# mlee03/FRE-NCtools

Hardware: AMD Instinct MI355X
Metric: exchange-cells/s (higher is better)
Workload: dtype f64; 1 GPU; C384 cubed sphere (6 tiles) -> 1440x720 lat-lon, conservative_order2: exchange-grid search + centroid pass + CSR build per step; nxgrid=4160000, parallelism=1 latitude band(s) of the target, one per GPU, world_size=1

## Files before the change

fre-nctools_amd/csrc/apply_kernels.hip:

```cpp
#include "xgrid_device.h"
#include <type_traits>

static inline int nblk(long n, int t) { return (int)((n + t - 1) / t); }

__global__ __launch_bounds__(256) void k_csr_count(long nx, const int *x_dst, int *row_cnt)
{
  long n = (long)blockIdx.x * blockDim.x + threadIdx.x;
  if (n < nx) atomicAdd(&row_cnt[x_dst[n]], 1);
}

__global__ __launch_bounds__(256) void k_csr_fill(long nx, const int *x_src, const int *x_dst, const int *row_ptr, int *row_fill, FgRowEnt *perm)
{
  const long n = (long)blockIdx.x * blockDim.x + threadIdx.x;
  const int lane = threadIdx.x & 63;
  const int d = (n < nx) ? x_dst[n] : -1;
  const int s = (n < nx) ? x_src[n] : 0;
  const int prev = __shfl_up(d, 1);
  const bool head = (lane == 0) || (d != prev);
  const unsigned long long heads = __ballot(head);
  const int start = 63 - __clzll((long long)(heads & ((2ull << lane) - 1ull)));
  const unsigned long long above = (start == 63) ? 0ull : (heads & ~((2ull << start) - 1ull));
  const int end = above ? (__ffsll((long long)above) - 1) : 64;
  int base = 0;
  if (lane == start && d >= 0) base = atomicAdd(&row_fill[d], end - start);
  base = __shfl(base, start);
  if (d >= 0) perm[row_ptr[d] + base + (lane - start)] = FgRowEnt{(int)n, s};
}

__global__ __launch_bounds__(256) void k_csr_fill_pos(long nx, const unsigned long long *nx_dev, const int *x_src, const int *x_dst,
                                                       const int *row_ptr, const int *x_rowpos, FgRowEnt *perm)
{
  if (nx_dev) { const unsigned long long nd = *nx_dev; if (nd < (unsigned long long)nx) nx = (long)nd; }
  const long n = (long)blockIdx.x * blockDim.x + threadIdx.x;
  if (n < nx) { const int s = x_src[n]; perm[row_ptr[x_dst[n]] + x_rowpos[n]] = FgRowEnt{(int)n, s}; }
}

template <int N>
__device__ __forceinline__ void d_rank_count(const int *keys, int n, const int (&v)[N], int (&rank)[N])
{
  int j = 0;
  for (; j + 4 <= n; j += 4) {
    const int x0 = keys[j], x1 = keys[j + 1], x2 = keys[j + 2], x3 = keys[j + 3];
#pragma unroll
    for (int k = 0; k < N; k++) rank[k] += ((x0 < v[k]) ? 1 : 0) + ((x1 < v[k]) ? 1 : 0) + ((x2 < v[k]) ? 1 : 0) + ((x3 < v[k]) ? 1 : 0);
  }
  for (; j < n; j++) {
    const int x = keys[j];
#pragma unroll
    for (int k = 0; k < N; k++) rank[k] += (x < v[k]) ? 1 : 0;
  }
}

template <typename E>
__device__ __forceinline__ void d_store_stream(E *dst, const E &e)
{
  typedef int v4i __attribute__((ext_vector_type(4)));
  static_assert(sizeof(E) % 16 == 0 && alignof(E) >= 8, "records are whole 16-byte words");
  v4i w[sizeof(E) / 16];
  __builtin_memcpy(w, &e, sizeof(E));
#pragma unroll
  for (unsigned k = 0; k < sizeof(E) / 16; k++) __builtin_nontemporal_store(w[k], (v4i *)dst + k);
}

template <int ORDER, bool DIST, int BT, int G, bool STAGED>
__device__ __forceinline__ void d_csr_records(const int *sh, const int *shs, const FgRowEnt *perm, int q0, int nq, const double *x_area,
                                              const double *x_c1, const double *x_c2, const int *src_idx_f, const FgSrcRec *cen,
                                              const FgCsr &csr)
{
  for (int i0 = threadIdx.x; i0 < nq; i0 += BT * G) {
    int n[G], s[G], idx[G];
    double ar[G], c1[G], c2[G], cl[G], ct[G];
#pragma unroll
    for (int g = 0; g < G; g++) {
      const int i = i0 + BT * g, ic = (i < nq) ? i : i0;
      if (STAGED) { n[g] = sh[ic]; s[g] = shs[ic]; }
      else { const FgRowEnt p = perm[q0 + ic]; n[g] = p.n; s[g] = p.s; }
    }
#pragma unroll
    for (int g = 0; g < G; g++) {
      ar[g] = x_area[n[g]];
      if (ORDER == 2) { c1[g] = x_c1[n[g]]; c2[g] = x_c2[n[g]]; }
      idx[g] = src_idx_f[s[g]];
      if (ORDER == 2 && DIST) { const FgSrcRec r = cen[s[g]]; cl[g] = r.cen_lon; ct[g] = r.cen_lat; }
    }
#pragma unroll
    for (int g = 0; g < G; g++) {
      const int i = i0 + BT * g;
      if (ORDER == 2) {
        FgCsrEntry2 E;
        E.idx_f = idx[g]; E.idx_g = s[g]; E.area = ar[g];
        if (DIST) {
          double di = c1[g] / E.area, dj = c2[g] / E.area;
          di -= cl[g]; dj -= ct[g];
          E.di = di; E.dj = dj;
        } else { E.di = c1[g]; E.dj = c2[g]; }
        if (i < nq) d_store_stream(&csr.e2[q0 + i], E);
      } else {
        FgCsrEntry1 E;
        E.idx_f = idx[g]; E.pad = 0; E.area = ar[g];
        if (i < nq) d_store_stream(&csr.e1[q0 + i], E);
      }
    }
  }
}

__device__ __forceinline__ void d_row_insertion(FgRowEnt *perm, int b, int e)
{
  for (int i = b + 1; i < e; i++) {
    const FgRowEnt v = perm[i];
    int j = i - 1;
    while (j >= b && perm[j].n > v.n) { perm[j + 1] = perm[j]; j--; }
    perm[j + 1] = v;
  }
}

#define SG_GROUP 2
template <int ORDER, int RPW, bool DIST, int BT, int G>
__global__ __launch_bounds__(BT) void k_csr_sortgather(int ndst, FgRowEnt *perm, const double *x_area, const double *x_c1, const double *x_c2,
                                                        const int *src_idx_f, const FgSrcRec *cen, FgCsr csr, int *tmp, long ntmp)
{
  constexpr int SHORT = 12, CAP = (RPW >= 64) ? 512 : 2048;
  __shared__ int sh[CAP], shs[CAP];
  __shared__ int long_b[RPW], long_n[RPW];
  __shared__ int nlong;
  if (threadIdx.x == 0) nlong = 0;
  __syncthreads();
  const int d0 = blockIdx.x * RPW, d1 = min(d0 + RPW, ndst);
  const int q0 = csr.row_ptr[d0], q1 = csr.row_ptr[d1], nq = q1 - q0;
  const bool staged = nq <= CAP;
  const int d = d0 + threadIdx.x;
  int b = 0, e = 0;
  if ((int)threadIdx.x < RPW && d < ndst) { b = csr.row_ptr[d]; e = csr.row_ptr[d + 1]; }
  if (staged) {
    for (int i = threadIdx.x; i < nq; i += BT) { const FgRowEnt p = perm[q0 + i]; sh[i] = p.n; shs[i] = p.s; }
    __syncthreads();
    if (e - b > SHORT) { const int q = atomicAdd(&nlong, 1); long_b[q] = b - q0; long_n[q] = e - b; }
    else
      for (int i = b - q0 + 1; i < e - q0; i++) {
        const int v = sh[i], w = shs[i];
        int j = i - 1;
        while (j >= b - q0 && sh[j] > v) { sh[j + 1] = sh[j]; shs[j + 1] = shs[j]; j--; }
        sh[j + 1] = v; shs[j + 1] = w;
      }
    __syncthreads();
    const int nl = nlong;
    for (int q = 0; q < nl; q++) {
      const int rb = long_b[q], n = long_n[q];
      constexpr int OWN = CAP / BT;
      if (n <= BT) {
        const bool own = (int)threadIdx.x < n;
        int v = 0, w = 0, rank = 0;
        if (own) {
          v = sh[rb + threadIdx.x]; w = shs[rb + threadIdx.x];
          for (int j = 0; j < n; j++) rank += (sh[rb + j] < v) ? 1 : 0;
        }
        __syncthreads();
        if (own) { sh[rb + rank] = v; shs[rb + rank] = w; }
      } else {
        int v[OWN], w[OWN], rank[OWN];
#pragma unroll
        for (int k = 0; k < OWN; k++) {
          const int i = threadIdx.x + BT * k;
          v[k] = (i < n) ? sh[rb + i] : 0x7fffffff; w[k] = (i < n) ? shs[rb + i] : 0; rank[k] = 0;
        }
        d_rank_count<OWN>(sh + rb, n, v, rank);
        __syncthreads();
#pragma unroll
        for (int k = 0; k < OWN; k++) if ((int)threadIdx.x + BT * k < n) { sh[rb + rank[k]] = v[k]; shs[rb + rank[k]] = w[k]; }
      }
      __syncthreads();
    }
  } else {
    if (e - b > SHORT) { const int q = atomicAdd(&nlong, 1); long_b[q] = b; long_n[q] = e - b; }
    else d_row_insertion(perm, b, e);
    __syncthreads();
    const int nl = nlong;
    for (int q = 0; q < nl; q++) {
      const int rb = long_b[q], n = long_n[q];
      if (n <= CAP) {
        for (int i = threadIdx.x; i < n; i += BT) { const FgRowEnt p = perm[rb + i]; sh[i] = p.n; shs[i] = p.s; }
        __syncthreads();
        for (int i = threadIdx.x; i < n; i += BT) {
          const int v = sh[i];
          int rank = 0;
          for (int j = 0; j < n; j++) rank += (sh[j] < v) ? 1 : 0;
          perm[rb + rank] = FgRowEnt{v, shs[i]};
        }
        __syncthreads();
      } else if (tmp) {
        FgRowEnt *srt = (FgRowEnt *)tmp + rb;
        int *rk = tmp + 2 * ntmp + rb;
        for (int t0 = 0; t0 < n; t0 += CAP) {
          const int m = min(CAP, n - t0);
          for (int j = threadIdx.x; j < m; j += BT) sh[j] = perm[rb + t0 + j].n;
          __syncthreads();
          for (int i0 = threadIdx.x; i0 < n; i0 += 8 * BT) {
            int v[8], r[8];
#pragma unroll
            for (int k = 0; k < 8; k++) { const int i = i0 + BT * k; v[k] = (i < n) ? perm[rb + i].n : 0x7fffffff; r[k] = (i < n && t0) ? rk[i] : 0; }
            d_rank_count<8>(sh, m, v, r);
#pragma unroll
            for (int k = 0; k < 8; k++) { const int i = i0 + BT * k; if (i < n) rk[i] = r[k]; }
          }
          __syncthreads();
        }
        for (int i = threadIdx.x; i < n; i += BT) srt[rk[i]] = perm[rb + i];
        __syncthreads();
        for (int i = threadIdx.x; i < n; i += BT) perm[rb + i] = srt[i];
        __syncthreads();
      } else if (threadIdx.x == 0) d_row_insertion(perm, rb, rb + n);
    }
    __syncthreads();
  }
  if (staged) d_csr_records<ORDER, DIST, BT, G, true>(sh, shs, perm, q0, nq, x_area, x_c1, x_c2, src_idx_f, cen, csr);
  else        d_csr_records<ORDER, DIST, BT, G, false>(sh, shs, perm, q0, nq, x_area, x_c1, x_c2, src_idx_f, cen, csr);
}

__global__ __launch_bounds__(256) void k_src_field_index(int order, const FgTile *tiles, int ntiles, int nsrc, int *src_idx_f)
{
  int s = blockIdx.x * blockDim.x + threadIdx.x;
  if (s >= nsrc) return;
  if (order != 2) { src_idx_f[s] = s; return; }
  int t = 0, foff = 0;
  while (t + 1 < ntiles && s >= tiles[t + 1].cell_off) { foff += (tiles[t].nx + 2) * (tiles[t].ny + 2); t++; }
  int loc = s - tiles[t].cell_off;
  int i = loc % tiles[t].nx, j = loc / tiles[t].nx;
  src_idx_f[s] = foff + (j + 1) * (tiles[t].nx + 2) + i + 1;
}

__device__ __forceinline__ int d_xcd_block(int b, int nb, int band)
{
  if (!band) return b;
  if (band == 1) {
    const int x = b & 7, k = b >> 3, q = nb >> 3, r = nb & 7;
    return x * q + min(x, r) + k;
  }
  const int C = band, per = 8 * C, full = nb / per * per;
  if (b >= full) return b;
  const int x = b & 7, k = b >> 3;
  return ((k / C) * 8 + x) * C + (k % C);
}

template <int ORDER> using CsrEntry = typename std::conditional<ORDER == 2, FgCsrEntry2, FgCsrEntry1>::type;
template <int ORDER> __device__ __forceinline__ const CsrEntry<ORDER> *csr_entries(const FgCsr &csr)
{
  if constexpr (ORDER == 2) return csr.e2; else return csr.e1;
}
typedef unsigned int u4v __attribute__((ext_vector_type(4)));

struct EpTile { int q0, q1, d, lev, b, e; bool lane; };
template <int ROWS, int LPR>
__device__ __forceinline__ EpTile ep_tile(const FgCsr &csr, int ndst, int tile)
{
  EpTile T;
  const int t = threadIdx.x;
  const int d0 = tile * ROWS, dl = min(d0 + ROWS, ndst);
  T.q0 = csr.row_ptr[d0]; T.q1 = csr.row_ptr[dl];
  T.lane = t < ROWS * LPR;
  T.d = d0 + t / LPR; T.lev = t % LPR;
  const int dc = min(T.d, ndst - 1);
  T.b = 0; T.e = 0;
  if (T.lane) { T.b = csr.row_ptr[dc]; T.e = csr.row_ptr[dc + 1]; }
  return T;
}

template <int TPB, int CAP, typename Entry>
__device__ __forceinline__ void ep_stage_unrolled(Entry *sh_e, const Entry *src, int n)
{
  constexpr int W = sizeof(Entry) / 16, WPL = CAP * W / TPB;
  const int t = threadIdx.x, nw = n * W;
  const u4v *g = reinterpret_cast<const u4v *>(src);
  u4v *l = reinterpret_cast<u4v *>(sh_e);
  u4v w[WPL];
#pragma unroll
  for (int j = 0; j < WPL; j++) w[j] = __builtin_nontemporal_load(g + min(t + TPB * j, nw - 1));
#pragma unroll
  for (int j = 0; j < WPL; j++) if (t + TPB * j < nw) l[t + TPB * j] = w[j];
}
template <int TPB, typename Entry>
__device__ __forceinline__ void ep_stage_loop(Entry *sh_e, const Entry *src, int n)
{
  constexpr int W = sizeof(Entry) / 16;
  const u4v *g = reinterpret_cast<const u4v *>(src);
  u4v *l = reinterpret_cast<u4v *>(sh_e);
  for (int i = threadIdx.x; i < n * W; i += TPB) l[i] = __builtin_nontemporal_load(g + i);
}

struct EpTerm { double p, a; unsigned ok; };
template <typename F>
__device__ __forceinline__ void ep_row_add(int b, int e, int c0, int n, double &acc, double &asum, unsigned &touched, F term)
{
  const int qa = max(b, c0) - c0, qb = min(e, c0 + n) - c0;
  int q = qa;
  for (; q + 8 <= qb; q += 8) {
    EpTerm c[8];
#pragma unroll
    for (int k = 0; k < 8; k++) c[k] = term(q + k);
#pragma unroll
    for (int k = 0; k < 8; k++) { acc += c[k].p; asum += c[k].a; touched |= c[k].ok; }
  }
  for (; q < qb; q++) { const EpTerm c = term(q); acc += c.p; asum += c.a; touched |= c.ok; }
}

__device__ __forceinline__ double apply_finish(double acc, double asum, bool touched, double missing, double &rs)
{
  rs = (asum > 0) ? acc : 0.0;
  if (asum > 0) return acc / asum;
  return touched ? 0.0 : missing;
}
__device__ __forceinline__ double apply_finish_ex(const FgApplyEx &o, int d, double acc, double asum, double asum_t, bool touched, double &rs)
{
  if (o.sum) {
    rs = (asum > 0) ? acc : 0.0;
    return (asum == 0) ? (touched ? 0.0 : o.missing) : acc;
  }
  double r = apply_finish(acc, asum, touched, o.missing, rs);
  if (o.cell_area_out && r != o.missing) r *= (asum_t / o.cell_area_out[d]);
  return r;
}

template <int ORDER, bool MISSING>
__global__ __launch_bounds__(256) void k_apply1(int ndst, FgCsr csr, const double *f, const double *px, const double *py,
                                                 const int *gmask, double missing, double *out, double *row_sum)
{
  int d = blockIdx.x * 256 + threadIdx.x;
  if (d >= ndst) return;
  int b = csr.row_ptr[d], e = csr.row_ptr[d + 1];
  double acc = 0.0, asum = 0.0;
  int touched = 0;
  for (int q = b; q < e; q++) {
    double a, v;
    if (ORDER == 2) {
      const FgCsrEntry2 E = csr.e2[q];
      a = E.area; v = f[E.idx_f];
      if (MISSING) { if (v == missing) continue; }
      bool flatgrad = false;
      if (MISSING) flatgrad = gmask[E.idx_g] != 0;
      if (!flatgrad) v = (v + px[E.idx_g] * E.di + py[E.idx_g] * E.dj);
    } else {
      const FgCsrEntry1 E = csr.e1[q];
      a = E.area; v = f[E.idx_f];
      if (MISSING) { if (v == missing) continue; }
    }
    acc += v * a;
    asum += a;
    touched = 1;
  }
  double rs;
  const double r = apply_finish(acc, asum, touched != 0, missing, rs);
  if (row_sum) row_sum[d] = rs;
  out[d] = r;
}

template <int ORDER, bool MISSING, int TPB, int CAP, int ROWS>
__global__ __launch_bounds__(TPB) void k_apply_ep1(int ndst, FgCsr csr, const double *f, const double *px, const double *py, const int *gmask,
                                                    double missing, double *out, double *row_sum, int xcd_band)
{
  typedef CsrEntry<ORDER> Entry;
  constexpr int PASS = CAP / TPB;
  static_assert(ROWS <= TPB && CAP % TPB == 0, "tile shape");
  __shared__ __attribute__((aligned(16))) Entry sh_e[CAP];
  double *sh_p = reinterpret_cast<double *>(sh_e), *sh_a = sh_p + CAP;
  __shared__ unsigned char sh_fl[CAP];
  const int t = threadIdx.x;
  const EpTile T = ep_tile<ROWS, 1>(csr, ndst, d_xcd_block(blockIdx.x, gridDim.x, xcd_band));
  double acc = 0.0, asum = 0.0;
  unsigned touched = 0;
  for (int c0 = T.q0; c0 < T.q1; c0 += CAP) {
// ... 469 lines not shown
  if (!T.lane || T.d >= ndst || (MASKED && lev >= nb_valid)) return;
  double rs;
  const double r = apply_finish(acc, asum, MASKED ? touched != 0 : T.e > T.b, missing, rs);
  if (row_sum) row_sum[MASKED ? (size_t)lev * out_ld + T.d : (size_t)T.d * NB + lev] = rs;
  if (MASKED || out_ld > 0) { if (lev < nb_valid) out[(size_t)lev * out_ld + T.d] = r; }
  else out[(size_t)T.d * NB + lev] = r;
}

__global__ __launch_bounds__(256) void k_gmask_bits(long n, const int *gmask, long ld, int nb, unsigned char *bits)
{
  const long c = (long)blockIdx.x * blockDim.x + threadIdx.x;
  if (c >= n) return;
  unsigned m = 0;
  for (int k = 0; k < nb; k++) m |= (gmask[(size_t)k * ld + c] != 0 ? 1u : 0u) << k;
  bits[c] = (unsigned char)m;
}

template <int NB>
__global__ __launch_bounds__(256) void k_interleave(long n, const double *in, long ld, int nb, double *out)
{
  long c = (long)blockIdx.x * blockDim.x + threadIdx.x;
  if (c >= n) return;
  double v[NB];
#pragma unroll
  for (int k = 0; k < NB; k++) v[k] = (k < nb) ? in[(size_t)k * ld + c] : 0.0;
#pragma unroll
  for (int k = 0; k < NB; k++) out[(size_t)c * NB + k] = v[k];
}
template <int NB>
__global__ __launch_bounds__(256) void k_deinterleave(long n, const double *in, long ld, int nb, double *out)
{
  long c = (long)blockIdx.x * blockDim.x + threadIdx.x;
  if (c >= n) return;
  double v[NB];
#pragma unroll
  for (int k = 0; k < NB; k++) v[k] = in[(size_t)c * NB + k];
#pragma unroll
  for (int k = 0; k < NB; k++) if (k < nb) out[(size_t)k * ld + c] = v[k];
}

struct FgIl3 { const double *in[3]; double *out[3]; long n[3]; long ld[3]; };
template <int NB>
__global__ __launch_bounds__(256) void k_interleave3(FgIl3 a, int nb)
{
  __shared__ double tile[256 * (NB + 1)];
  const int w = blockIdx.y;
  const long n = a.n[w];
  const long c0 = (long)blockIdx.x * 256;
  if (c0 >= n) return;
  const double *in = a.in[w];
  double *out = a.out[w];
  const long ld = a.ld[w];
  const long c = c0 + threadIdx.x;
#pragma unroll
  for (int k = 0; k < NB; k++) tile[threadIdx.x * (NB + 1) + k] = (k < nb && c < n) ? in[(size_t)k * ld + c] : 0.0;
  __syncthreads();
  const long cnt = ((n - c0) < 256 ? (n - c0) : 256) * NB;
#pragma unroll
  for (int i = 0; i < NB; i++) {
    const long e = (long)i * 256 + threadIdx.x;
    if (e < cnt) out[(size_t)c0 * NB + e] = tile[(e / NB) * (NB + 1) + (e % NB)];
  }
}

template <int NB, int CB>
__global__ __launch_bounds__(256) void k_merge3(long n, const int *src_idx_f, const double *f, long ld_f, const double *gx,
                                                const double *gy, long ld_g, int nb, double *out)
{
  constexpr int R = 3 * NB;
  __shared__ double tile[CB * (R + 1)];
  const long c0 = (long)blockIdx.x * CB;
  const int t = threadIdx.x % CB;
  const long c = c0 + t;
  const long cf = (c < n) ? (long)src_idx_f[c] : 0;
  for (int e = threadIdx.x; e < CB * R; e += 256) {
    const int wk = e / CB, w = wk / NB, k = wk % NB;
    double v = 0.0;
    if (k < nb && c < n) v = (w == 0) ? f[(size_t)k * ld_f + cf] : ((w == 1) ? gx[(size_t)k * ld_g + c] : gy[(size_t)k * ld_g + c]);
    tile[t * (R + 1) + wk] = v;
  }
  __syncthreads();
  const long cnt = ((n - c0) < CB ? (n - c0) : CB) * R;
  for (long e = threadIdx.x; e < cnt; e += 256) out[(size_t)c0 * R + e] = tile[(e / R) * (R + 1) + (e % R)];
}

__global__ __launch_bounds__(256) void k_xgrid_indices(long nx, const int *x_src, const int *x_dst, const FgTile *tiles, int ntiles,
                                                        int nx_out, int *t_in, int *i_in, int *j_in, int *i_out, int *j_out)
{
  const long k = (long)blockIdx.x * blockDim.x + threadIdx.x;
  if (k >= nx) return;
  const int s = x_src[k], d = x_dst[k];
  int m = 0;
  while (m + 1 < ntiles && s >= tiles[m + 1].cell_off) m++;
  const int loc = s - tiles[m].cell_off, nxt = tiles[m].nx;
  t_in[k] = m; i_in[k] = loc % nxt; j_in[k] = loc / nxt;
  i_out[k] = d % nx_out; j_out[k] = d / nx_out;
}
void fgd_xgrid_indices(long nx, const int *x_src, const int *x_dst, const FgTile *tiles_dev, int ntiles, int nx_out,
                       int *t_in, int *i_in, int *j_in, int *i_out, int *j_out, hipStream_t st)
{
  if (nx > 0) k_xgrid_indices<<<nblk(nx, 256), 256, 0, st>>>(nx, x_src, x_dst, tiles_dev, ntiles, nx_out, t_in, i_in, j_in, i_out, j_out);
}

__global__ __launch_bounds__(256) void k_apply_frac(int ndst, FgCsr csr, const double *data, double *out)
{
  int d = blockIdx.x * blockDim.x + threadIdx.x;
  if (d >= ndst) return;
  int b = csr.row_ptr[d], e = csr.row_ptr[d + 1];
  double asum = 0.0, acc = 0.0;
  for (int q = b; q < e; q++) asum += csr.e1[q].area;
  for (int q = b; q < e; q++) {
    double frac = csr.e1[q].area / asum;
    acc += data[csr.e1[q].idx_f] * frac;
  }
  out[d] = acc;
}

__global__ __launch_bounds__(256) void k_reduce_partial(const double *v, long n, double *partial)
{
  __shared__ double sh[256];
  double s = 0;
  for (long i = (long)blockIdx.x * blockDim.x + threadIdx.x; i < n; i += (long)gridDim.x * blockDim.x) s += v[i];
  sh[threadIdx.x] = s;
  __syncthreads();
  for (int w = 128; w > 0; w >>= 1) { if (threadIdx.x < w) sh[threadIdx.x] += sh[threadIdx.x + w]; __syncthreads(); }
  if (threadIdx.x == 0) partial[blockIdx.x] = sh[0];
}
__global__ __launch_bounds__(256) void k_reduce_final(const double *partial, int np, double *result)
{
  __shared__ double sh[256];
  double s = 0;
  for (int i = threadIdx.x; i < np; i += 256) s += partial[i];
  sh[threadIdx.x] = s;
  __syncthreads();
  for (int w = 128; w > 0; w >>= 1) { if (threadIdx.x < w) sh[threadIdx.x] += sh[threadIdx.x + w]; __syncthreads(); }
  if (threadIdx.x == 0) *result = sh[0];
}

#define REDUCE_BLOCKS 512

void fgd_csr_count(long nx, const int *x_dst, int *row_cnt, hipStream_t st)
{
  if (nx > 0) k_csr_count<<<nblk(nx, 256), 256, 0, st>>>(nx, x_dst, row_cnt);
}
void fgd_csr_fill(long nx, const int *x_src, const int *x_dst, const int *row_ptr, int *row_fill, FgRowEnt *perm, hipStream_t st)
{
  if (nx > 0) k_csr_fill<<<nblk(nx, 256), 256, 0, st>>>(nx, x_src, x_dst, row_ptr, row_fill, perm);
}
void fgd_csr_fill_pos(long nx_cap, const unsigned long long *nx_dev, const int *x_src, const int *x_dst, const int *row_ptr, const int *x_rowpos, FgRowEnt *perm,
                      hipStream_t st)
{
  if (nx_cap > 0) k_csr_fill_pos<<<nblk(nx_cap, 256), 256, 0, st>>>(nx_cap, nx_dev, x_src, x_dst, row_ptr, x_rowpos, perm);
}
void fgd_csr_sortgather(int order, int ndst, long nx, const FgRowEnt *perm, const double *x_area, const double *x_c1, const double *x_c2,
                        const int *src_idx_f, const FgSrcRec *cen, FgCsr csr, hipStream_t st, int *tmp, long ntmp,
                        int long_rows)
{
  if (ndst <= 0) return;
  FgRowEnt *pm = const_cast<FgRowEnt *>(perm);
  const int mode = nx > 256 * (long)ndst ? 2 : ((nx > 8 * (long)ndst || long_rows) ? 1 : 0);
#define SG(O_, R_, D_) k_csr_sortgather<O_, R_, D_, (R_ >= 64 ? 64 : 256), SG_GROUP><<<nblk(ndst, R_), (R_ >= 64 ? 64 : 256), 0, st>>>(ndst, pm, x_area, x_c1, x_c2, src_idx_f, cen, csr, tmp, ntmp)
#define SGM(O_, D_) do { if (mode == 2) SG(O_, 1, D_); else if (mode == 1) SG(O_, 16, D_); else SG(O_, 64, D_); } while (0)
  if (order == 2) { if (cen) SGM(2, true); else SGM(2, false); }
  else SGM(1, false);
#undef SGM
#undef SG
}
void fgd_src_field_index(int order, const FgTile *tiles_dev, int ntiles, int nsrc, int *src_idx_f, hipStream_t st)
{
  if (nsrc > 0) k_src_field_index<<<nblk(nsrc, 256), 256, 0, st>>>(order, tiles_dev, ntiles, nsrc, src_idx_f);
}
extern int g_apply_xcd, g_apply_ep;
template <int V> using Int = std::integral_constant<int, V>;
template <int R0, int R1, int R2, int R3, typename F>
static void by_row_length(long m, F launch)
{
  if (m <= 6) launch(Int<R0>()); else if (m <= 24) launch(Int<R1>()); else if (m <= 96) launch(Int<R2>()); else launch(Int<R3>());
}
static int xcd_chunk8() { return g_apply_xcd >= 2 ? 2 * g_apply_xcd : g_apply_xcd; }

void fgd_apply1(int order, int ndst, FgCsr csr, const double *f, const double *gx, const double *gy, const int *gmask,
                int has_missing, double missing, double *out, double *row_sum, hipStream_t st, long nx)
{
  if (ndst <= 0) return;
  if (g_apply_ep && nx >= 0) {
    auto ep1 = [&](auto O, auto M) {
      by_row_length<64, 16, 4, 1>(nx / ndst, [&](auto R) {
        k_apply_ep1<decltype(O)::value, decltype(M)::value, 256, 512, decltype(R)::value><<<nblk(ndst, decltype(R)::value), 256, 0, st>>>(
            ndst, csr, f, gx, gy, gmask, missing, out, row_sum, g_apply_xcd);
      });
    };
    if (order == 2) { if (has_missing) ep1(Int<2>(), std::true_type()); else ep1(Int<2>(), std::false_type()); }
    else            { if (has_missing) ep1(Int<1>(), std::true_type()); else ep1(Int<1>(), std::false_type()); }
    return;
  }
  int grid = nblk(ndst, 256);
  if (order == 2) {
    if (has_missing) k_apply1<2, true><<<grid, 256, 0, st>>>(ndst, csr, f, gx, gy, gmask, missing, out, row_sum);
    else             k_apply1<2, false><<<grid, 256, 0, st>>>(ndst, csr, f, gx, gy, gmask, missing, out, row_sum);
  } else {
    if (has_missing) k_apply1<1, true><<<grid, 256, 0, st>>>(ndst, csr, f, gx, gy, gmask, missing, out, row_sum);
    else             k_apply1<1, false><<<grid, 256, 0, st>>>(ndst, csr, f, gx, gy, gmask, missing, out, row_sum);
  }
}

template <int ORDER, bool MASKED, int CAP, int R0, int R1, int R2, int R3>
static void apply_ep8g(int ndst, long nx, FgCsr csr, const double *rec, const unsigned char *gbits, double missing, double *out,
                       double *row_sum, long out_ld, int nb_valid, int xb, hipStream_t st)
{
  by_row_length<R0, R1, R2, R3>(nx / ndst, [&](auto R) {
    k_apply_ep8g<ORDER, MASKED, 256, CAP, decltype(R)::value><<<nblk(ndst, decltype(R)::value), 256, 0, st>>>(
        ndst, csr, rec, gbits, missing, out, row_sum, out_ld, nb_valid, xb);
  });
}

template <int NB, int V>
static void apply_il_nb(int order, int ndst, FgCsr csr, const double *f, const double *gx, const double *gy, double missing,
                        double *out, double *row_sum, long out_ld, int nb_valid, hipStream_t st)
{
  int grid = nblk(ndst, 256 / (NB / V));
  if (order == 2) k_apply_il<2, NB, V><<<grid, 256, 0, st>>>(ndst, csr, f, gx, gy, missing, out, row_sum, out_ld, nb_valid, g_apply_xcd);
  else            k_apply_il<1, NB, V><<<grid, 256, 0, st>>>(ndst, csr, f, gx, gy, missing, out, row_sum, out_ld, nb_valid, g_apply_xcd);
}
int g_apply_xcd = 64;
int g_apply_ep = 1;
int g_apply_vec = 0;
void fgd_apply_il(int order, int nb, int ndst, FgCsr csr, const double *f, const double *gx, const double *gy, double missing,
                  double *out, double *row_sum, long out_ld, int nb_valid, hipStream_t st, long nx)
{
  if (ndst <= 0) return;
  if (order == 1 && nb == 8 && g_apply_ep && nx > 6L * ndst) {
    apply_ep8g<1, false, 256, 8, 8, 2, 1>(ndst, nx, csr, f, nullptr, missing, out, row_sum, out_ld, nb_valid, xcd_chunk8(), st);
    return;
  }
  const int v = g_apply_vec ? g_apply_vec : (nb >= 8 ? 4 : 2);
#define AP(NB_) do { if (v >= 4 && NB_ >= 4) apply_il_nb<NB_, (NB_ >= 4 ? 4 : 2)>(order, ndst, csr, f, gx, gy, missing, out, row_sum, out_ld, nb_valid, st); \
                     else if (v >= 2) apply_il_nb<NB_, 2>(order, ndst, csr, f, gx, gy, missing, out, row_sum, out_ld, nb_valid, st); \
                     else apply_il_nb<NB_, 1>(order, ndst, csr, f, gx, gy, missing, out, row_sum, out_ld, nb_valid, st); } while (0)
  if (nb == 16) AP(16);
  else if (nb == 8) AP(8);
  else if (nb == 4) AP(4);
  else AP(2);
#undef AP
}
void fgd_apply_il_merged(int nb, int ndst, long nx, FgCsr csr, const double *rec, double missing, double *out, double *row_sum, long out_ld,
                         int nb_valid, hipStream_t st)
{
  if (ndst <= 0) return;
#define APM(NB_, V_) k_apply_il<2, NB_, V_, true><<<nblk(ndst, 256 / (NB_ / V_)), 256, 0, st>>>(ndst, csr, rec, nullptr, nullptr, missing, out, row_sum, out_ld, nb_valid, g_apply_xcd)
  if (nb == 16) APM(16, 4);
  else if (nb == 8 && g_apply_ep && nx <= 6L * ndst)
    k_apply_ep8<256, 256><<<nblk(ndst, EP_ROWS), 256, 0, st>>>(ndst, csr, rec, missing, out, row_sum, out_ld, nb_valid, xcd_chunk8());
  else if (nb == 8 && g_apply_ep)
    apply_ep8g<2, false, 256, 8, 8, 2, 1>(ndst, nx, csr, rec, nullptr, missing, out, row_sum, out_ld, nb_valid, xcd_chunk8(), st);
  else if (nb == 8) { if (g_apply_vec == 2) APM(8, 2); else APM(8, 4); }
  else if (nb == 4) APM(4, 2);
  else APM(2, 2);
#undef APM
}
void fgd_apply_levels8(int order, int ndst, long nx, FgCsr csr, const double *rec, const unsigned char *gbits, double missing, double *out,
                       double *row_sum, long ld, int nb_valid, hipStream_t st)
{
  if (ndst <= 0) return;
  if (order == 2) apply_ep8g<2, true, FG_LEVELS_CAP, 32, 8, 2, 1>(ndst, nx, csr, rec, gbits, missing, out, row_sum, ld, nb_valid, 0, st);
  else            apply_ep8g<1, true, FG_LEVELS_CAP, 32, 8, 2, 1>(ndst, nx, csr, rec, gbits, missing, out, row_sum, ld, nb_valid, 0, st);
}
void fgd_gmask_bits(long n, const int *gmask, long ld, int nb, unsigned char *bits, hipStream_t st)
{
  if (n > 0) k_gmask_bits<<<nblk(n, 256), 256, 0, st>>>(n, gmask, ld, nb, bits);
}
void fgd_merge3(int nb_pad, long n, const int *src_idx_f, const double *f, long ld_f, const double *gx, const double *gy, long ld_g,
                int nb_valid, double *out, hipStream_t st)
{
  if (n <= 0) return;
  if (nb_pad == 16) k_merge3<16, 64><<<nblk(n, 64), 256, 0, st>>>(n, src_idx_f, f, ld_f, gx, gy, ld_g, nb_valid, out);
  else if (nb_pad == 8) k_merge3<8, 64><<<nblk(n, 64), 256, 0, st>>>(n, src_idx_f, f, ld_f, gx, gy, ld_g, nb_valid, out);
  else if (nb_pad == 4) k_merge3<4, 128><<<nblk(n, 128), 256, 0, st>>>(n, src_idx_f, f, ld_f, gx, gy, ld_g, nb_valid, out);
  else k_merge3<2, 128><<<nblk(n, 128), 256, 0, st>>>(n, src_idx_f, f, ld_f, gx, gy, ld_g, nb_valid, out);
}
void fgd_interleave(int nb_pad, long n, const double *in, long ld, int nb_valid, double *out, hipStream_t st)
{
  if (n <= 0) return;
  if (nb_pad == 16) k_interleave<16><<<nblk(n, 256), 256, 0, st>>>(n, in, ld, nb_valid, out);
  else if (nb_pad == 8) k_interleave<8><<<nblk(n, 256), 256, 0, st>>>(n, in, ld, nb_valid, out);
  else if (nb_pad == 4) k_interleave<4><<<nblk(n, 256), 256, 0, st>>>(n, in, ld, nb_valid, out);
  else k_interleave<2><<<nblk(n, 256), 256, 0, st>>>(n, in, ld, nb_valid, out);
}
void fgd_interleave3(int nb_pad, int narr, const double *const *in, const long *ld, const long *n, double *const *out, int nb_valid,
                     hipStream_t st)
{
  FgIl3 a;
  long nmax = 0;
  for (int w = 0; w < 3; w++) {
    a.in[w] = (w < narr) ? in[w] : nullptr; a.out[w] = (w < narr) ? out[w] : nullptr;
    a.n[w] = (w < narr) ? n[w] : 0; a.ld[w] = (w < narr) ? ld[w] : 0;
    if (a.n[w] > nmax) nmax = a.n[w];
  }
  if (nmax <= 0) return;
  dim3 grid(nblk(nmax, 256), narr);
  if (nb_pad == 16) k_interleave3<16><<<grid, 256, 0, st>>>(a, nb_valid);
  else if (nb_pad == 8) k_interleave3<8><<<grid, 256, 0, st>>>(a, nb_valid);
  else if (nb_pad == 4) k_interleave3<4><<<grid, 256, 0, st>>>(a, nb_valid);
  else k_interleave3<2><<<grid, 256, 0, st>>>(a, nb_valid);
}
void fgd_deinterleave(int nb_pad, long n, const double *in, long ld, int nb_valid, double *out, hipStream_t st)
{
  if (n <= 0) return;
  if (nb_pad == 16) k_deinterleave<16><<<nblk(n, 256), 256, 0, st>>>(n, in, ld, nb_valid, out);
  else if (nb_pad == 8) k_deinterleave<8><<<nblk(n, 256), 256, 0, st>>>(n, in, ld, nb_valid, out);
  else if (nb_pad == 4) k_deinterleave<4><<<nblk(n, 256), 256, 0, st>>>(n, in, ld, nb_valid, out);
  else k_deinterleave<2><<<nblk(n, 256), 256, 0, st>>>(n, in, ld, nb_valid, out);
}
void fgd_apply_ex(int order, int ndst, FgCsr csr, const double *f, const double *gx, const double *gy, FgApplyEx o,
                  double *out, double *row_sum, int *err, hipStream_t st, long nx)
// ... 46 lines not shown
```

fre-nctools_amd/csrc/plan.hip:

```cpp
#include <hip/hip_runtime.h>
#include <math.h>
#include <stdarg.h>
#include <stdio.h>
#include <stdlib.h>
#include <string.h>
#include <algorithm>
#include <map>
#include <mutex>
#include <string>
#include <type_traits>
#include <vector>
#include "fregrid_hip.h"
#include "xgrid_device.h"

static thread_local std::string g_err;
static int fail(int code, const char *fmt, ...)
{
  char buf[512];
  va_list ap; va_start(ap, fmt); vsnprintf(buf, sizeof buf, fmt, ap); va_end(ap);
  g_err = buf;
  return code;
}
#define HIPCHK(call) do { hipError_t e_ = (call); if (e_ != hipSuccess) \
  return fail(FG_ERR_HIP, "%s failed: %s (%s:%d)", #call, hipGetErrorString(e_), __FILE__, __LINE__); } while (0)
// ... 196 lines not shown
    for (const XferJob &j : batch) total += j.bytes;
    if (total == 0) return true;
    static const int nthreads = [] {
      const char *e = getenv("FREGRID_HIP_XFER_THREADS");
      int n = e ? atoi(e) : 0;
      if (n <= 0) { const unsigned hc = std::thread::hardware_concurrency(); n = hc >= 16 ? 8 : (hc >= 8 ? 4 : 2); }
      return std::min(n, 16);
    }();
    if (total < 2 * CHUNK) {
      if (hipSetDevice(dev) != hipSuccess) return false;
      for (const XferJob &j : batch)
        if (j.bytes && hipMemcpy(j.d2h ? j.host : j.dev, j.d2h ? j.dev : j.host, j.bytes, j.d2h ? hipMemcpyDeviceToHost : hipMemcpyHostToDevice) != hipSuccess) return false;
      return true;
    }
    std::lock_guard<std::mutex> bl(batch_mu);
    {
      std::lock_guard<std::mutex> lk(mu);
      if (threads.empty())
        for (int t = 0; t < nthreads; t++) { threads.emplace_back([this] { loop(); }); threads.back().detach(); }
      jobs = &batch; chunks.clear();
      for (size_t k = 0; k < batch.size(); k++)
        for (size_t off = 0; off < batch[k].bytes; off += CHUNK) chunks.push_back({(int)k, off});
      next.store(0); failed.store(0); device = dev; active = (int)threads.size(); gen++;
    }
    cv_work.notify_all();
    std::unique_lock<std::mutex> lk(mu);
    cv_done.wait(lk, [&] { return active == 0; });
    jobs = nullptr;
    return failed.load() == 0;
  }
};
XferPool &xfer_pool() { static XferPool *p = new XferPool(); return *p; }
}

static int g_profiling = 0;
extern "C" void fg_set_profiling(int on) { g_profiling = on ? 1 : 0; }
enum { PH_CELL_STRUCT = 0, PH_BINS, PH_CANDIDATES, PH_CLIP_QUAD, PH_CLIP_GENERAL, PH_COMPACT, PH_ROWS,
       PH_SEARCH_TOTAL, PH_FINALIZE, PH_APPLY, PH_COUNT };
struct HandleCache {
  std::mutex mu;
  std::map<int, std::vector<hipStream_t>> streams;
  std::map<int, std::vector<hipEvent_t>> events;
  static int current_device() { int d = 0; (void)hipGetDevice(&d); return d; }
  hipStream_t get_stream(int dev)
  {
    {
      std::lock_guard<std::mutex> lk(mu);
      auto &v = streams[dev];
      if (!v.empty()) { hipStream_t s = v.back(); v.pop_back(); return s; }
    }
    hipStream_t s = nullptr;
    if (hipStreamCreateWithFlags(&s, hipStreamNonBlocking) != hipSuccess) return nullptr;
    return s;
  }
  void put_stream(int dev, hipStream_t s)
  {
    if (!s) return;
    std::lock_guard<std::mutex> lk(mu);
    streams[dev].push_back(s);
  }
  hipEvent_t get_event()
  {
    {
      std::lock_guard<std::mutex> lk(mu);
      auto &v = events[current_device()];
      if (!v.empty()) { hipEvent_t e = v.back(); v.pop_back(); return e; }
    }
    hipEvent_t e = nullptr;
    (void)hipEventCreate(&e);
    return e;
  }
  void put_event(hipEvent_t e)
  {
    if (!e) return;
    std::lock_guard<std::mutex> lk(mu);
    events[current_device()].push_back(e);
  }
  std::map<int, std::vector<hipEvent_t>> sync_events;
  hipEvent_t get_sync_event()
  {
    {
      std::lock_guard<std::mutex> lk(mu);
      auto &v = sync_events[current_device()];
      if (!v.empty()) { hipEvent_t e = v.back(); v.pop_back(); return e; }
    }
    hipEvent_t e = nullptr;
    (void)hipEventCreateWithFlags(&e, hipEventDisableTiming);
    return e;
  }
  void put_sync_event(hipEvent_t e)
  {
    if (!e) return;
    std::lock_guard<std::mutex> lk(mu);
    sync_events[current_device()].push_back(e);
  }
};
static HandleCache g_handles;

struct PhaseTimer {
  bool on = false;
  hipStream_t st = nullptr;
  std::vector<std::pair<int, std::pair<hipEvent_t, hipEvent_t>>> spans;
  hipEvent_t open_ev = nullptr; int open_ph = -1;
  void start(bool enable, hipStream_t s) { on = enable; st = s; }
  void begin(int ph)
  {
    if (!on) return;
    open_ev = g_handles.get_event(); (void)hipEventRecord(open_ev, st); open_ph = ph;
  }
  void end()
  {
    if (!on || open_ph < 0) return;
    hipEvent_t e = g_handles.get_event(); (void)hipEventRecord(e, st);
    spans.push_back({open_ph, {open_ev, e}}); open_ph = -1;
  }
  void collect(float *ms)
  {
    for (auto &sp : spans) {
      float t = 0; (void)hipEventElapsedTime(&t, sp.second.first, sp.second.second);
      ms[sp.first] += t;
      g_handles.put_event(sp.second.first); g_handles.put_event(sp.second.second);
    }
    spans.clear();
  }
};

struct fg_plan {
  float phase_ms[PH_COUNT] = {0};
  PhaseTimer apply_pt;
  int apply_spans = 0;
  int order = 0, device = 0;
  bool great_circle = false;
  hipStream_t stream = nullptr;
  hipStream_t stream_b = nullptr;
  bool own_stream = true;
  int ntiles = 0;
  std::vector<int> nx_in, ny_in, cell_off;
  std::vector<FgTile> tiles_host;
  int nsrc = 0;
  int nx_out = 0, ny_out = 0, ndst = 0;
  long f_stride = 0;
  bool searched = false, finalized = false, have_geom = false;
  bool fused = false;

  std::vector<void *> owned;
  FgTile *tiles_dev = nullptr;
  double *mask_dev = nullptr;
  FgCells S{}, D{};
  bool rect = false;
  FgRect rect_tab{};
  FgPolyList polys{};
  long nx = 0;
  int *x_src = nullptr, *x_dst = nullptr;
  double *x_area = nullptr, *x_c1 = nullptr, *x_c2 = nullptr;
  int *xoff = nullptr;
  FgRowEnt *perm = nullptr;
  bool rows_built = false;
  bool dist_pending = false;
  double *sums = nullptr;
  FgSrcRec *cen = nullptr;
  FgCsr csr{};
  int *src_idx_f = nullptr;
  double *row_sum = nullptr, *red_partial = nullptr, *red_result = nullptr;
  long row_sum_cap = 0;
  double *il_f = nullptr, *il_out = nullptr, *il_rs = nullptr;
  double *il_m = nullptr;
  unsigned char *lv_bits = nullptr;
  long stats[FG_NSTATS] = {0};
  double *mono_x = nullptr, *mono_b = nullptr;
  int *xerr = nullptr;
  bool mono_open = false;
  unsigned *ll_err = nullptr;

  template <typename T> T *alloc(size_t count)
  {
    void *p = g_pool.get(device, count * sizeof(T));
    if (p) owned.push_back(p);
    return (T *)p;
  }
  void release(void *p)
  {
    if (!p) return;
    for (size_t k = 0; k < owned.size(); k++) if (owned[k] == p) { owned.erase(owned.begin() + k); break; }
    g_pool.put(p);
  }
  void drop_search(size_t keep)
  {
    while (owned.size() > keep) { g_pool.put(owned.back()); owned.pop_back(); }
    tiles_dev = nullptr; mask_dev = nullptr; S = FgCells{}; D = FgCells{};
    x_src = x_dst = nullptr; x_area = x_c1 = x_c2 = nullptr; xoff = nullptr;
    perm = nullptr; csr.row_ptr = nullptr; csr.e1 = nullptr; csr.e2 = nullptr; cen = nullptr; src_idx_f = nullptr; sums = nullptr;
    have_geom = false; rect = false; rect_tab = FgRect{};
  }
};

static bool alloc_cells(fg_plan *pl, FgCells *c, size_t n)
{
  c->lat_min = pl->alloc<double>(n); c->lat_max = pl->alloc<double>(n);
  c->lon_min = pl->alloc<double>(n); c->lon_max = pl->alloc<double>(n);
  c->lon_avg = pl->alloc<double>(n); c->area = pl->alloc<double>(n);
  c->nv = pl->alloc<int>(n);
  c->verts = pl->alloc<double>(n * 16);
  return c->lat_min && c->lat_max && c->lon_min && c->lon_max && c->lon_avg && c->area && c->nv && c->verts;
}

static int plan_base(int order, int ntiles_in, const int *nx_in, const int *ny_in, int nx_out, int ny_out,
                     int device, fg_plan **out)
{
  if (order != FG_CONSERVE_ORDER1 && order != FG_CONSERVE_ORDER2) return fail(FG_ERR_ARG, "order must be 1 or 2");
  if (ntiles_in < 1 || !nx_in || !ny_in || nx_out < 1 || ny_out < 1 || !out) return fail(FG_ERR_ARG, "bad grid sizes");
  int ndev = 0;
  HIPCHK(hipGetDeviceCount(&ndev));
  if (ndev < 1) return fail(FG_ERR_HIP, "no HIP device visible: libfregrid_hip needs an MI355X-class GPU");
  if (device < 0 || device >= ndev) return fail(FG_ERR_ARG, "device %d out of range (0..%d)", device, ndev - 1);
  HIPCHK(hipSetDevice(device));
  fg_plan *pl = new fg_plan();
  pl->order = order; pl->device = device; pl->ntiles = ntiles_in;
  long off = 0, foff = 0;
  for (int m = 0; m < ntiles_in; m++) {
    if (nx_in[m] < 1 || ny_in[m] < 1) { delete pl; return fail(FG_ERR_ARG, "bad source tile size"); }
    pl->nx_in.push_back(nx_in[m]); pl->ny_in.push_back(ny_in[m]); pl->cell_off.push_back((int)off);
    off += (long)nx_in[m] * ny_in[m];
    foff += (order == 2) ? (long)(nx_in[m] + 2) * (ny_in[m] + 2) : (long)nx_in[m] * ny_in[m];
  }
  if (off > 2000000000L || (long)nx_out * ny_out > 2000000000L) { delete pl; return fail(FG_ERR_ARG, "grid too large for 32-bit cell indices"); }
  pl->nsrc = (int)off; pl->f_stride = foff;
  pl->nx_out = nx_out; pl->ny_out = ny_out; pl->ndst = nx_out * ny_out;
  pl->stream = g_handles.get_stream(device);
  if (!pl->stream) { delete pl; return fail(FG_ERR_HIP, "hipStreamCreate failed"); }
  *out = pl;
  return 0;
}

extern "C" void fg_plan_destroy(fg_plan *pl)
{
  if (!pl) return;
  (void)hipSetDevice(pl->device);
  if (pl->stream || !pl->own_stream) (void)hipStreamSynchronize(pl->stream);
  if (pl->stream && pl->own_stream) g_handles.put_stream(pl->device, pl->stream);
  if (pl->stream_b) { (void)hipStreamSynchronize(pl->stream_b); g_handles.put_stream(pl->device, pl->stream_b); }
  { float junk[PH_COUNT] = {0}; pl->apply_pt.collect(junk); }
  for (void *p : pl->owned) g_pool.put(p);
  delete pl;
}

static void choose_bins(const fg_plan *pl, double mean_dlat, double mean_dlon, FgBins *b)
{
  const double PI = 3.14159265358979323846;
  double h = 1.25 * mean_dlat, w = 1.25 * mean_dlon;
  int nblat = (h > 0) ? (int)ceil(PI / h) : 1;
  int nblon = (w > 0) ? (int)ceil(2.0 * PI / w) : 1;
  if (nblat < 1) nblat = 1; if (nblat > 8192) nblat = 8192;
  if (nblon < 1) nblon = 1; if (nblon > 16384) nblon = 16384;
  (void)pl;
  b->nblat = nblat; b->nblon = nblon;
  b->inv_wlat = nblat / PI;
  b->inv_wlon = nblon / (2.0 * PI);
}

static FgCounters *pinned_counters()
{
  static thread_local FgCounters *h = nullptr;
  if (!h) { if (hipHostMalloc((void **)&h, sizeof(FgCounters), hipHostMallocDefault) != hipSuccess) h = nullptr; }
  return h;
}

struct GcXyz { const double *x, *y, *z; };
struct BoxMode { FgBox box; const double *mask_quad; int no_adjust; };
struct SearchIn {
  const double *const *lon_in = nullptr, *const *lat_in = nullptr, *const *mask_in = nullptr;
  const double *lon_out = nullptr, *lat_out = nullptr;
  const GcXyz *gc_in = nullptr, *gc_out = nullptr;
  const BoxMode *boxm = nullptr;
  double mean_dlat = 0, mean_dlon = 0;
  int rect_hint = 1;
};
struct SearchOpts { bool exact, cull, finalize, rect, dst_frame; int gc_split; bool profile; };
static const char *gc_clip_error(int code)
{
  switch (code) {
    case 3: return "firstIntersect is not in the grid1List";
    case 4: return " not found the next intersection ";
    case 5: return "not return back to the first intersection";
    case 6: return "After clipping, nintersect should be 0";
    case 7: return "inserAfter: point (x,y,z) is not found in the list";
    case 8: return "Error from create_xgrid.c: temp is not in list1";
    default: return "clip_2dx2d_great_circle: more intersections than two convex quadrilaterals can have (list capacity)";
  }
}

static int g_search_cull = 0;
static int g_search_finalize = 0;
static int g_gc_split = 1;
extern "C" void fg_set_gc_split(int on) { g_gc_split = on < 0 ? 0 : on; }
struct SearchCaps { unsigned long long entries; int regcap, nreg; bool rect; };
static int g_search_rect = 1;
extern "C" void fg_set_search_rect(int on) { g_search_rect = on ? 1 : 0; }
static int g_dst_frame = 0;
extern "C" void fg_set_search_frame(int coupler) { g_dst_frame = coupler ? 1 : 0; }
static bool host_says_not_rect(int nx, int ny, const double *lon, const double *lat)
{
  const long nxp = nx + 1;
  const int js[3] = {ny, ny / 2, 1}, is[3] = {nx, nx / 2, 1};
  for (int a = 0; a < 3; a++)
    for (int b = 0; b < 3; b++) {
      const long e = (long)js[a] * nxp + is[b];
      if (memcmp(&lon[e], &lon[is[b]], sizeof(double)) || memcmp(&lat[e], &lat[(long)js[a] * nxp], sizeof(double))) return true;
    }
  return false;
}
#define FG_RETRY (-1000L)
struct Carve {
  size_t n = 0;
  size_t operator()(size_t size) { const size_t at = n; n += size; return at; }
};
struct SearchBlocks {
  fg_plan *pl;
  bool ok = true;
  std::vector<void *> scratch;
  template <typename T> T *keep(size_t count) { T *p = pl->alloc<T>(count); ok = ok && p; return p; }
  template <typename T> T *get(size_t count) { T *p = keep<T>(count); if (p) scratch.push_back(p); return p; }
  void release() { for (void *p : scratch) pl->release(p); scratch.clear(); }
};
static long plan_search_core(fg_plan *pl, const SearchIn &in, const SearchOpts &opt, SearchCaps *caps)
{
  const bool gc = in.gc_in != nullptr;
  const BoxMode *const boxm = in.boxm;
  pl->great_circle = gc;
  hipStream_t st = pl->stream;
  const int nsrc = pl->nsrc, ndst = pl->ndst, order = pl->order;
  FgCounters *hc = pinned_counters();
  if (!hc) return fail(FG_ERR_HIP, "hipHostMalloc failed");

  std::vector<FgTile> &th = pl->tiles_host;
  th.resize(pl->ntiles + 1);
  for (int m = 0; m < pl->ntiles; m++) th[m] = FgTile{gc ? nullptr : in.lon_in[m], gc ? nullptr : in.lat_in[m], pl->nx_in[m], pl->ny_in[m], pl->cell_off[m]};
  th[pl->ntiles] = FgTile{in.lon_out, in.lat_out, pl->nx_out, pl->ny_out, 0};
  pl->tiles_dev = pl->alloc<FgTile>(pl->ntiles + 1);
  if (!pl->tiles_dev) return fail(FG_ERR_HIP, "out of device memory");
  FgTileSet ts; ts.n = 0;
  const bool by_value = !gc && pl->ntiles + 1 <= FG_TILESET_MAX;
  if (by_value) { ts.n = pl->ntiles + 1; for (int m = 0; m <= pl->ntiles; m++) ts.t[m] = th[m]; }
  else HIPCHK(hipMemcpyAsync(pl->tiles_dev, th.data(), sizeof(FgTile) * th.size(), hipMemcpyHostToDevice, st));
  FgTileXyz *gct_dev = nullptr;
  std::vector<FgTileXyz> gct;
  if (gc) {
    gct.resize(pl->ntiles + 1);
    for (int m = 0; m < pl->ntiles; m++) gct[m] = FgTileXyz{in.gc_in[m].x, in.gc_in[m].y, in.gc_in[m].z, pl->nx_in[m], pl->ny_in[m], pl->cell_off[m]};
    gct[pl->ntiles] = FgTileXyz{in.gc_out->x, in.gc_out->y, in.gc_out->z, pl->nx_out, pl->ny_out, 0};
    gct_dev = pl->alloc<FgTileXyz>(pl->ntiles + 1);
    if (!gct_dev) return fail(FG_ERR_HIP, "out of device memory");
    HIPCHK(hipMemcpyAsync(gct_dev, gct.data(), sizeof(FgTileXyz) * gct.size(), hipMemcpyHostToDevice, st));
  }

  bool any_mask = false;
  if (in.mask_in) for (int m = 0; m < pl->ntiles; m++) if (in.mask_in[m]) any_mask = true;
  if (any_mask) {
    pl->mask_dev = pl->alloc<double>(nsrc);
    if (!pl->mask_dev) return fail(FG_ERR_HIP, "out of device memory");
    std::vector<double> ones;
    for (int m = 0; m < pl->ntiles; m++) {
      size_t nc = (size_t)pl->nx_in[m] * pl->ny_in[m];
      if (in.mask_in[m]) HIPCHK(hipMemcpyAsync(pl->mask_dev + pl->cell_off[m], in.mask_in[m], nc * sizeof(double), hipMemcpyDeviceToDevice, st));
      else {
        ones.assign(nc, 1.0);
        HIPCHK(hipMemcpyAsync(pl->mask_dev + pl->cell_off[m], ones.data(), nc * sizeof(double), hipMemcpyHostToDevice, st));
        HIPCHK(hipStreamSynchronize(st));
      }
    }
  }

  const bool rect = caps->rect && !gc && !boxm;
  pl->rect = rect;
  const double dst_tlon = opt.dst_frame ? (double)NAN : 3.14159265358979323846;
  FgBins bins;
  choose_bins(pl, in.mean_dlat, in.mean_dlon, &bins);
  if (rect) { bins.nblat = 0; bins.nblon = 0; }
  const long nbins = (long)bins.nblat * bins.nblon;
  const long nslots = nbins + bins.nblat;
  const unsigned long long nentries = rect ? 0ull : caps->entries;
  const int ecap = (int)std::min<unsigned long long>(nentries, 2147483647ull);
  FgPairSpace ps{};
  ps.nreg = caps->nreg; ps.regcap = caps->regcap;
  const long npairs = fgd_pairs_total(ps);
  const long nx_alloc = npairs;

  if (!alloc_cells(pl, &pl->S, nsrc)) return fail(FG_ERR_HIP, "out of device memory");
  SearchBlocks blk{pl};
  struct { double *hdr, *lat_ax, *lon_ax, *col, *row, *col_min, *col_max, *col_avg; } rt{};
  if (rect) {
    pl->D = FgCells{};
    pl->D.area = blk.keep<double>(ndst);
    Carve at;
    const size_t o_hdr = at(8), o_lat = at((size_t)pl->ny_out + 1), o_lon = at((size_t)pl->nx_out + 1), o_col = at(8 * (size_t)pl->nx_out),
                 o_row = at(4 * ((size_t)pl->ny_out + 1)), o_cmin = at((size_t)pl->nx_out), o_cmax = at((size_t)pl->nx_out), o_cavg = at((size_t)pl->nx_out);
    double *rect_blk = blk.keep<double>(at.n);
    if (!blk.ok) return fail(FG_ERR_HIP, "out of device memory");
    rt = {rect_blk + o_hdr, rect_blk + o_lat, rect_blk + o_lon, rect_blk + o_col, rect_blk + o_row, rect_blk + o_cmin, rect_blk + o_cmax, rect_blk + o_cavg};
  } else if (!alloc_cells(pl, &pl->D, ndst)) return fail(FG_ERR_HIP, "out of device memory");
  const long t_bins = fgd_scan_tiles(nslots), t_rows = fgd_scan_tiles(ndst), t_comp = fgd_scan_tiles(nsrc);
  const size_t zreg = (size_t)FG_NREG * FG_FILL_STRIDE * sizeof(unsigned);
  Carve z;
  const size_t z_dc = z((sizeof(FgCounters) + 127) / 128 * 128), z_fill = z(zreg), z_tick = z(128);
  const size_t z_lb_bins = z(t_bins * sizeof(unsigned long long)), z_lb_rows = z(t_rows * sizeof(unsigned long long)),
               z_lb_comp = z(t_comp * sizeof(unsigned long long));
  const size_t z_bin_cnt = z((size_t)(nslots + 1) * sizeof(int)), z_bin_fill = z((size_t)(nslots + 1) * sizeof(int)),
               z_row_cnt = z((size_t)(ndst + 1) * sizeof(int)), z_nacc = z((size_t)(nsrc + 1) * sizeof(int));
  z((16 - (z.n - z_bin_cnt) % 16) % 16);
  const size_t z_gc_ntask = z(gc ? zreg : 0), z_gc_ocnt = z(gc ? zreg : 0);
  const size_t zbytes = z.n;
  char *zero_blk = blk.get<char>(zbytes);
  int *bin_start = blk.get<int>(nslots + 1);
  int *heavy_list = blk.get<int>(nsrc + 1);
  int *big_list = blk.get<int>(nsrc + 1);
  int *pair_beg = blk.get<int>(nsrc + 1), *pair_cnt = blk.get<int>(nsrc + 1);
  FgBinEntry *bin_entries = blk.get<FgBinEntry>(nentries ? nentries : 1);
  ps.src = blk.get<int>(npairs + 1); ps.dst = blk.get<int>(npairs + 1);
  double *tmp_area = blk.get<double>(npairs + 1);
  double *tmp_clon = (order == 2) ? blk.get<double>(npairs + 1) : nullptr;
  double *tmp_clat = (order == 2) ? blk.get<double>(npairs + 1) : nullptr;
  int *defer_list = blk.get<int>(npairs + 1);
  const bool early_rows = !gc && !boxm;
  int *tmp_rowpos = early_rows ? blk.get<int>(npairs + 1) : nullptr;
  const bool gc_split = gc && opt.gc_split && npairs < (1L << 28);
  const long tcap_want = (opt.gc_split == 2) ? npairs / 64 : 3 * npairs;
  const long tcap_reg = gc_split ? std::min<long>((tcap_want / FG_NREG + 255) / 256 * 256, 0x7ffffff0L / FG_NREG) : 0;
  const long tcap_all = tcap_reg * FG_NREG;
  unsigned *gc_meta = gc_split ? blk.get<unsigned>(npairs + 1) : nullptr;
  int *gc_tbase = gc_split ? blk.get<int>(npairs + 1) : nullptr;
  int *gc_order = gc_split ? blk.get<int>(npairs + 1) : nullptr;
  unsigned *gc_task = gc_split ? blk.get<unsigned>(tcap_all + 1) : nullptr;
  double *gc_res = gc_split ? blk.get<double>(2 * (size_t)tcap_all + 2) : nullptr;
  pl->xoff = blk.keep<int>(nsrc + 1);
  pl->x_src = blk.keep<int>(nx_alloc + 1); pl->x_dst = blk.keep<int>(nx_alloc + 1);
  pl->x_area = blk.keep<double>(nx_alloc + 1);
  if (order == 2) { pl->x_c1 = blk.keep<double>(nx_alloc + 1); pl->x_c2 = blk.keep<double>(nx_alloc + 1); pl->sums = blk.keep<double>(3 * (size_t)nsrc); }
  int *x_rowpos = blk.get<int>(nx_alloc + 1);
  pl->perm = blk.keep<FgRowEnt>(nx_alloc + 1);
  pl->csr.row_ptr = blk.keep<int>(ndst + 1);
  if (!pl->src_idx_f) pl->src_idx_f = blk.keep<int>(nsrc + 1);
  if (!blk.ok) return fail(FG_ERR_HIP, "out of device memory");
  FgCounters *dc = (FgCounters *)(zero_blk + z_dc);
  ps.fill = (unsigned *)(zero_blk + z_fill);
  unsigned *tickets = (unsigned *)(zero_blk + z_tick);
  unsigned long long *lb_bins = (unsigned long long *)(zero_blk + z_lb_bins), *lb_rows = (unsigned long long *)(zero_blk + z_lb_rows),
                     *lb_comp = (unsigned long long *)(zero_blk + z_lb_comp);
  int *bin_cnt = (int *)(zero_blk + z_bin_cnt), *bin_fill = (int *)(zero_blk + z_bin_fill), *row_cnt = (int *)(zero_blk + z_row_cnt);
  int *nacc = (int *)(zero_blk + z_nacc);
  HIPCHK(hipMemsetAsync(zero_blk, 0, zbytes, st));
  if (pl->ll_err) HIPCHK(hipMemcpyAsync(&dc->err[2], pl->ll_err, sizeof(unsigned), hipMemcpyDeviceToDevice, st));

  PhaseTimer pt, ptot;
  pt.start(opt.profile, st); ptot.start(opt.profile, st);
  for (int k = 0; k < PH_COUNT; k++) pl->phase_ms[k] = 0;
  ptot.begin(PH_SEARCH_TOTAL);
  pt.begin(PH_CELL_STRUCT);
  if (gc) {
    fgd_gc_cell_struct(gct_dev + pl->ntiles, 1, ndst, pl->D, st, opt.cull ? dc->band_keys : nullptr, 1);
    fgd_gc_cell_struct(gct_dev, pl->ntiles, nsrc, pl->S, st, opt.cull ? dc->band_keys : nullptr, 2);
    fgd_src_field_index(order, pl->tiles_dev, pl->ntiles, nsrc, pl->src_idx_f, st);
  } else if (rect) {
    FgRect &R = pl->rect_tab;
    R.hdr = rt.hdr; R.lat_ax = rt.lat_ax; R.lon_ax = rt.lon_ax; R.col = rt.col; R.row = rt.row;
    R.col_min = rt.col_min; R.col_max = rt.col_max; R.col_avg = rt.col_avg;
    R.bad = &dc->rect_bad; R.nx = pl->nx_out; R.ny = pl->ny_out;
    fgd_rect_tables(in.lon_out, in.lat_out, pl->nx_out, pl->ny_out, rt.hdr, rt.lat_ax, rt.lon_ax, rt.col, rt.col_min, rt.col_max, rt.col_avg, rt.row,
                    &dc->rect_bad, dc->err, st, dst_tlon);
    if (pl->polys.npoly) fgd_polylist_records(pl->polys, pl->S, pl->src_idx_f, pl->sums, &R, heavy_list, &dc->heavy_cnt, dc->err, st);
    fgd_cell_struct2r(ts, pl->tiles_dev, pl->tiles_dev, pl->ntiles, pl->polys.npoly ? 0 : nsrc, ndst, pl->S, pl->D.area, R, pl->mask_dev, order,
                      pl->src_idx_f, pl->sums, dc->err, st, dc->band_keys, (opt.cull && !pl->polys.npoly) ? 2 : 0, heavy_list, &dc->heavy_cnt,
                      ps, pair_beg, pair_cnt, big_list, &dc->big_cnt);
  } else if (opt.cull && !boxm && !pl->polys.npoly) {
    fgd_band_keys(in.lat_out, (long)(pl->nx_out + 1) * (pl->ny_out + 1), dc->band_keys, st);
    fgd_cell_struct2(ts, pl->tiles_dev, pl->tiles_dev, pl->ntiles, nsrc, ndst, pl->S, pl->D, bins, bin_cnt, order, pl->src_idx_f, pl->sums, dc->err, st, dc->band_keys, 2, dst_tlon);
  } else if (pl->polys.npoly) {
    fgd_polylist_records(pl->polys, pl->S, pl->src_idx_f, pl->sums, nullptr, nullptr, nullptr, dc->err, st);
    fgd_cell_struct2(ts, pl->tiles_dev, pl->tiles_dev, pl->ntiles, 0, ndst, pl->S, pl->D, bins, bin_cnt, order, pl->src_idx_f, pl->sums, dc->err, st, nullptr, 0, dst_tlon);
  } else
    fgd_cell_struct2(ts, pl->tiles_dev, pl->tiles_dev, pl->ntiles, nsrc, ndst, pl->S, pl->D, bins, bin_cnt, order, pl->src_idx_f, pl->sums, dc->err, st, nullptr, 0, dst_tlon);
  if (boxm) fgd_box_cell_boxes(boxm->box, pl->S, st);
  if (boxm && boxm->no_adjust) fgd_box_area_no_adjust(boxm->box, pl->S.area, st);
  pt.end();
  pl->have_geom = true;

  if (!rect) {
    pt.begin(PH_BINS);
    if (gc) fgd_bin_count(ndst, pl->D, bins, bin_cnt, st);
    fgd_exclusive_scan1(bin_cnt, nslots, bin_start, lb_bins, &tickets[0], &dc->total[0], dc->err, st);
    fgd_bin_fill(ndst, pl->D, bins, bin_fill, bin_start, bin_entries, ecap, nsrc, pl->S, pl->mask_dev, heavy_list, &dc->heavy_cnt, st);
    pt.end();
  }

  pt.begin(PH_CANDIDATES);
  if (rect)
    fgd_candidates_rect(nsrc, pl->S, pl->mask_dev, pl->rect_tab, ps, pair_beg, pair_cnt, heavy_list, &dc->heavy_cnt, big_list, &dc->big_cnt, st,
                        pl->polys.npoly ? 0 : 1);
  else
    fgd_candidates1(nsrc, pl->S, pl->mask_dev, bins, bin_start, bin_entries, ecap, ps, pair_beg, pair_cnt, heavy_list, &dc->heavy_cnt, big_list,
                    &dc->big_cnt, st);
  pt.end();
  hipEvent_t gc_e1 = nullptr, gc_e2 = nullptr;
  struct EvReturn {
    hipEvent_t &a, &b;
    ~EvReturn() { g_handles.put_sync_event(a); g_handles.put_sync_event(b); a = b = nullptr; }
  } ev_return{gc_e1, gc_e2};
  if (boxm) {
    pt.begin(PH_CLIP_GENERAL);
    fgd_clip_box(order, ps, boxm->box, th[pl->ntiles], pl->S, pl->D, pl->mask_dev, boxm->mask_quad, tmp_area, tmp_clon, tmp_clat, nacc, dc->stats, dc->err, st);
    pt.end();
  } else if (gc) {
    pt.begin(PH_CLIP_GENERAL);
    if (gc_split) {
      if (!pl->stream_b) pl->stream_b = g_handles.get_stream(pl->device);
      gc_e1 = g_handles.get_sync_event(); gc_e2 = g_handles.get_sync_event();
      GcSplit g{gc_meta, gc_tbase, gc_task, gc_res, (unsigned)tcap_reg, (unsigned *)(zero_blk + z_gc_ntask), defer_list, &dc->defer_cnt,
                &dc->gc_list2_cnt, npairs, gc_order, (unsigned *)(zero_blk + z_gc_ocnt)};
      fgd_gc_clip_split(ps, pl->S, pl->mask_dev, pl->D, tmp_area, nacc, g, dc->stats, dc->err, st, pl->stream_b, gc_e1, gc_e2);
    } else
      fgd_gc_clip(ps, pl->S, pl->mask_dev, pl->D, tmp_area, nacc, defer_list, &dc->defer_cnt, dc->stats, dc->err, st);
    pt.end();
  } else {
    pt.begin(PH_CLIP_QUAD);
    fgd_clip_quad(order, ps, pl->S, pl->mask_dev, pl->D, tmp_area, tmp_clon, tmp_clat, nacc, defer_list, &dc->defer_cnt, dc->stats, dc->err, st,
                  rect ? &pl->rect_tab : nullptr, row_cnt, tmp_rowpos);
    pt.end();
    pt.begin(PH_CLIP_GENERAL);
    fgd_clip_general(order, ps, pl->S, pl->mask_dev, pl->D, tmp_area, tmp_clon, tmp_clat, nacc, defer_list, &dc->defer_cnt, dc->stats, dc->err, st,
                     rect ? &pl->rect_tab : nullptr, row_cnt, tmp_rowpos);
    pt.end();
  }
  pt.begin(PH_COMPACT);
  FgCompactIo io{};
  io.pair_beg = pair_beg; io.pair_cnt = pair_cnt;
  io.tmp_area = tmp_area; io.tmp_clon = tmp_clon; io.tmp_clat = tmp_clat;
  io.xoff = pl->xoff; io.x_src = pl->x_src; io.x_dst = pl->x_dst; io.x_area = pl->x_area; io.x_c1 = pl->x_c1; io.x_c2 = pl->x_c2;
  io.row_cnt = row_cnt; io.x_rowpos = x_rowpos; io.sums = pl->sums; io.big_list = big_list; io.big_cnt = &dc->big_cnt;
  io.tmp_rowpos = tmp_rowpos; io.row_ptr = pl->csr.row_ptr; io.perm = pl->perm;
  io.dc = dc; io.xcap = nx_alloc;
  if (early_rows)
    fgd_exclusive_scan2(nacc, nsrc, pl->xoff, lb_comp, &tickets[2], &dc->xtot, row_cnt, ndst, pl->csr.row_ptr, lb_rows, &tickets[1], &dc->rows_total, dc->err, st);
  else
    fgd_exclusive_scan1(nacc, nsrc, pl->xoff, lb_comp, &tickets[2], &dc->xtot, dc->err, st);
  fgd_compact(order, nsrc, ps, io, st);
  pt.end();
  if (!early_rows) {
    pt.begin(PH_ROWS);
    fgd_exclusive_scan1(row_cnt, ndst, pl->csr.row_ptr, lb_rows, &tickets[1], &dc->rows_total, dc->err, st);
    fgd_csr_fill_pos(nx_alloc, &dc->xtot, pl->x_src, pl->x_dst, pl->csr.row_ptr, x_rowpos, pl->perm, st);
    pt.end();
  }
  ptot.end();
  const bool fuse = opt.finalize && early_rows && !pl->polys.npoly;
  int *fused_tmp = nullptr;
  if (fuse) {
    pt.begin(PH_FINALIZE);
    if (order == 2) {
      pl->cen = pl->alloc<FgSrcRec>((size_t)nsrc + 1);
      if (!pl->cen) return fail(FG_ERR_HIP, "out of device memory");
      fgd_centroids(nsrc, pl->S, pl->sums, pl->cen, st);
      pl->csr.e2 = pl->alloc<FgCsrEntry2>(nx_alloc + 1);
    } else pl->csr.e1 = pl->alloc<FgCsrEntry1>(nx_alloc + 1);
    if (!pl->csr.e1 && !pl->csr.e2) return fail(FG_ERR_HIP, "out of device memory");
    int *sg_tmp = pl->alloc<int>(3 * (size_t)(nx_alloc + 1));
    fgd_csr_sortgather(order, ndst, (long)nsrc + ndst, pl->perm, pl->x_area, pl->x_c1, pl->x_c2, pl->src_idx_f,
                       order == 2 ? pl->cen : nullptr, pl->csr, st, sg_tmp, nx_alloc + 1);
    fused_tmp = sg_tmp;
    pt.end();
  }
  HIPCHK(hipMemcpyAsync(hc, dc, sizeof(FgCounters), hipMemcpyDeviceToHost, st));
  HIPCHK(hipStreamSynchronize(st));
  pt.collect(pl->phase_ms); ptot.collect(pl->phase_ms);
  HIPCHK(hipGetLastError());
  if (rect && hc->rect_bad) { caps->rect = false; return FG_RETRY; }
  if (hc->total[0] > nentries) { caps->entries = hc->total[0]; return FG_RETRY; }
  if (hc->total[0] > 2000000000ull) return fail(FG_ERR_ARG, "bin table too large");
  if (hc->total[3] > (unsigned long long)ps.regcap) {
    if (hc->total[3] > 2000000000ull / (unsigned long long)ps.nreg) return fail(FG_ERR_CAPACITY, "candidate pair list exceeds 2^31 entries");
    caps->regcap = (int)((hc->total[3] + FG_REG_ALIGN - 1) / FG_REG_ALIGN * FG_REG_ALIGN);
    return FG_RETRY;
  }
  if (hc->err[2] & G_ERRBIT_LL2X) return fail(FG_ERR_ARG, "latlon2xyz: a grid corner is not finite, or its latitude (|lat| >= 2.4262) or longitude "
                                                          "(|lon| > 1024) lies outside the range of the device trig (radians expected)");
  if (hc->err[0] & 8u) return fail(FG_ERR_ARG, "a grid corner latitude lies outside [-pi/2, pi/2] (radians expected)");
  if (hc->err[0] & 1u) return fail(FG_ERR_MAXV, "create_xgrid.c: n2_in is greater than MAX_V");
  if (hc->err[0] & 2u) return fail(FG_ERR_PARALLEL, "the line between <x1_0,y1_0> and  <x1_1,y1_1> should not parallel to "
                                                    "the line between <x2_0,y2_0> and  <x2_1,y2_1>");
  if (hc->err[0] & 4u) return fail(FG_ERR_MAXV, "clipped polygon exceeds 16 vertices");
  if (hc->err[0] & G_ERRBIT_GC_CONVEX1) return fail(FG_ERR_GEOM, "create_xgrid.c(clip_2dx2d_great_circle): grid box 1 is not convex");
  if (hc->err[0] & G_ERRBIT_GC_CONVEX2) return fail(FG_ERR_GEOM, "create_xgrid.c(clip_2dx2d_great_circle): grid box 2 is not convex");
  if (hc->err[0] & G_ERRBIT_GC_CLIP) return fail(FG_ERR_GEOM, "%s", gc_clip_error((int)hc->err[1]));
  if (hc->err[0] & G_ERRBIT_LOOKBACK) return fail(FG_ERR_HIP, "single-pass scan: a tile waited too long for its predecessor");
  pl->nx = (long)hc->xtot;
  pl->stats[FG_STAT_PAIRS] = (long)hc->total[1];
  pl->stats[FG_STAT_NONEMPTY] = (long)(hc->xtot + hc->stats[FG_STAT_BELOW]);
  pl->stats[FG_STAT_NXGRID] = pl->nx;
  pl->stats[FG_STAT_BORDERLINE] = (long)hc->stats[FG_STAT_BORDERLINE];
  pl->stats[FG_STAT_BINS] = nbins;
  pl->stats[FG_STAT_BIN_ENTRIES] = (long)hc->total[0];
  pl->stats[FG_STAT_DEFERRED] = hc->defer_cnt + hc->gc_list2_cnt;
  pl->stats[FG_STAT_HEAVY] = hc->heavy_cnt;
  pl->stats[FG_STAT_BELOW] = (long)hc->stats[FG_STAT_BELOW];

  pl->rect_tab.bad = nullptr;
  blk.release();
  pl->rows_built = true;
  pl->searched = true;
  if (fuse) {
    pl->release(pl->perm); pl->perm = nullptr; pl->release(fused_tmp);
    if (!pl->red_partial) { pl->red_partial = pl->alloc<double>(1024); pl->red_result = pl->alloc<double>(260); }
    if (!pl->red_partial || !pl->red_result) return fail(FG_ERR_HIP, "out of device memory");
    pl->dist_pending = (order == 2);
    pl->finalized = true; pl->fused = true;
  }
  return pl->nx;
}

static int g_search_exact = 0;
extern "C" void fg_set_search_mode(int exact) { g_search_exact = exact; }
extern "C" void fg_set_search_cull(int on) { g_search_cull = on ? 1 : 0; }
extern "C" void fg_set_search_finalize(int on) { g_search_finalize = on ? 1 : 0; }
static long plan_search(fg_plan *pl, const SearchIn &in)
{
  static const bool env_exact = getenv("FREGRID_HIP_EXACT_SEARCH") && atoi(getenv("FREGRID_HIP_EXACT_SEARCH")) != 0;
  const SearchOpts opt{.exact = g_search_exact || env_exact, .cull = g_search_cull != 0, .finalize = g_search_finalize != 0,
                       .rect = g_search_rect != 0, .dst_frame = g_dst_frame != 0, .gc_split = g_gc_split, .profile = g_profiling != 0};
  const long big = std::max((long)pl->nsrc, (long)pl->ndst);
  if (big > (1L << 28)) return fail(FG_ERR_CAPACITY, "grid of %ld cells: more than 2^28 cells per search are not supported", big);
  SearchCaps caps;
  caps.entries = opt.exact ? 0ull : 3ull * (unsigned long long)pl->ndst + 4096ull;
  const unsigned long long cap_pairs = std::min<unsigned long long>(8ull * (unsigned long long)big + 65536ull, 2000000000ull);
  caps.nreg = (int)std::max(1L, std::min((long)FG_NREG, ((long)pl->nsrc + 1023) / 1024));
  caps.regcap = opt.exact ? 0 : (int)((cap_pairs / caps.nreg + FG_REG_ALIGN - 1) / FG_REG_ALIGN * FG_REG_ALIGN);
  caps.rect = opt.rect && in.rect_hint && !in.gc_in && !in.boxm && pl->nx_out <= 8192 && pl->nx_out >= 2;
  const size_t keep = pl->owned.size();
  long rc = FG_RETRY;
  int attempts = 0;
  for (; attempts < 4 && rc == FG_RETRY; attempts++) {
    if (attempts) {
      (void)hipStreamSynchronize(pl->stream);
      pl->drop_search(keep);
    }
    rc = plan_search_core(pl, in, opt, &caps);
  }
  if (rc == FG_RETRY) return fail(FG_ERR_CAPACITY, "exchange-grid search: capacities did not settle");
  if (rc >= 0) pl->stats[FG_STAT_EXACT] = (attempts > 1) ? 1 : 0;
  return rc;
}

struct CornerSample {
  int nsamp = 0;
  std::vector<double> q;
  const double *corners(int a, int k) const { return &q[((size_t)a * nsamp + k) * 4]; }
};
static long sample_step(int nx, int ny, int *nsamp)
{
  const long ncell = (long)nx * ny;
  long step = ncell / 4096; if (step < 1) step = 1;
  *nsamp = (int)((ncell + step - 1) / step);
  return step;
}
__host__ __device__ static inline void sample_nodes(int nx, long step, int k, long n[4])
{
  const long c = (long)k * step;
  const int i = (int)(c % nx), j = (int)(c / nx);
  n[0] = (long)j * (nx + 1) + i; n[1] = n[0] + 1; n[3] = n[0] + nx + 1; n[2] = n[3] + 1;
}
static CornerSample sample_corners_host(int nx, int ny, int narr, const double *const *arr)
{
  CornerSample s;
  const long step = sample_step(nx, ny, &s.nsamp);
  s.q.resize((size_t)s.nsamp * narr * 4);
  for (int k = 0; k < s.nsamp; k++) {
    long n[4];
    sample_nodes(nx, step, k, n);
    for (int a = 0; a < narr; a++)
      for (int v = 0; v < 4; v++) s.q[((size_t)a * s.nsamp + k) * 4 + v] = arr[a][n[v]];
  }
  return s;
}
__global__ void k_sample_corners(int nx, long step, int nsamp, int narr, const double *a0, const double *a1, const double *a2, double *out)
{
  const int k = blockIdx.x * blockDim.x + threadIdx.x;
  if (k >= nsamp) return;
  long n[4];
  sample_nodes(nx, step, k, n);
  const double *arr[3] = {a0, a1, a2};
  for (int a = 0; a < narr; a++) {
    double *o = out + ((size_t)a * nsamp + k) * 4;
    o[0] = arr[a][n[0]]; o[1] = arr[a][n[1]]; o[2] = arr[a][n[2]]; o[3] = arr[a][n[3]];
  }
}
static int sample_corners_dev(fg_plan *pl, int nx, int ny, int narr, const double *d_a0, const double *d_a1, const double *d_a2, CornerSample *s)
{
  const long step = sample_step(nx, ny, &s->nsamp);
  s->q.resize((size_t)s->nsamp * narr * 4);
  double *d_q = (double *)g_pool.get(pl->device, s->q.size() * sizeof(double));
  if (!d_q) return fail(FG_ERR_HIP, "out of device memory");
  k_sample_corners<<<(s->nsamp + 255) / 256, 256, 0, pl->stream>>>(nx, step, s->nsamp, narr, d_a0, d_a1, d_a2, d_q);
  hipError_t e = hipMemcpyAsync(s->q.data(), d_q, s->q.size() * sizeof(double), hipMemcpyDeviceToHost, pl->stream);
  if (e == hipSuccess) e = hipStreamSynchronize(pl->stream);
  g_pool.put(d_q);
  if (e != hipSuccess) return fail(FG_ERR_HIP, "sampling the destination corners failed: %s", hipGetErrorString(e));
  return 0;
}
static void mean_extents(double sl, double sw, long cnt, double *mdlat, double *mdlon)
{
  const double PI = 3.14159265358979323846;
  if (cnt == 0) { *mdlat = PI / 180; *mdlon = PI / 180; return; }
  *mdlat = sl / cnt; *mdlon = sw / cnt;
  if (*mdlat < 1e-7) *mdlat = 1e-7;
  if (*mdlon < 1e-7) *mdlon = 1e-7;
}
static void extents_lonlat(const CornerSample &s, double *mdlat, double *mdlon, int *curvilinear)
{
  const double PI = 3.14159265358979323846;
  *curvilinear = 0;
  double sl = 0, sw = 0; long cnt = 0;
// ... 205 lines not shown


extern "C" int fg_dev_latlon2xyz(long n, const double *d_lon, const double *d_lat, double *d_x, double *d_y, double *d_z, int device, void *stream)
{
  if (n < 0 || (n > 0 && (!d_lon || !d_lat || !d_x || !d_y || !d_z))) return fail(FG_ERR_ARG, "fg_dev_latlon2xyz: bad size or null pointer");
  if (n == 0) return 0;
  HIPCHK(hipSetDevice(device));
  const FgLl2xGrid g{d_lon, d_lat, d_x, d_y, d_z, n};
  fgd_latlon2xyz(&g, 1, nullptr, (hipStream_t)stream);
  HIPCHK(hipGetLastError());
  return 0;
}

static long gc_lonlat_search(fg_plan *pl, const double *const *d_lon_in, const double *const *d_lat_in, const double *const *d_mask_in,
                             const double *d_lon_out, const double *d_lat_out, DstExtents x)
{
  const int nt = pl->ntiles;
  std::vector<FgLl2xGrid> jobs(nt + 1);
  std::vector<GcXyz> gxyz(nt + 1);
  std::vector<void *> blocks;
  for (int m = 0; m <= nt; m++) {
    const size_t np = m < nt ? (size_t)(pl->nx_in[m] + 1) * (pl->ny_in[m] + 1) : (size_t)(pl->nx_out + 1) * (pl->ny_out + 1);
    double *d = pl->alloc<double>(3 * np);
    if (!d) return fail(FG_ERR_HIP, "out of device memory");
    blocks.push_back(d);
    jobs[m] = FgLl2xGrid{m < nt ? d_lon_in[m] : d_lon_out, m < nt ? d_lat_in[m] : d_lat_out, d, d + np, d + 2 * np, (long)np};
    gxyz[m] = GcXyz{d, d + np, d + 2 * np};
  }
  pl->ll_err = pl->alloc<unsigned>(1);
  if (!pl->ll_err) return fail(FG_ERR_HIP, "out of device memory");
  blocks.push_back(pl->ll_err);
  hipError_t e = hipSetDevice(pl->device);
  if (e == hipSuccess) e = hipMemsetAsync(pl->ll_err, 0, sizeof(unsigned), pl->stream);
  if (e == hipSuccess) { fgd_latlon2xyz(jobs.data(), nt + 1, pl->ll_err, pl->stream); e = hipGetLastError(); }
  if (e != hipSuccess) return fail(FG_ERR_HIP, "latlon2xyz: %s", hipGetErrorString(e));
  const long nx = gc_search(pl, gxyz.data(), d_mask_in, x);
  if (nx < 0) return nx;
  for (void *p : blocks) pl->release(p);
  pl->ll_err = nullptr;
  return nx;
}

extern "C" long fg_plan_create_great_circle_lonlat_dev(int ntiles_in, const int *nx_in, const int *ny_in,
                                                       const double *const *d_lon_in, const double *const *d_lat_in,
                                                       const double *const *d_mask_in, int nx_out, int ny_out,
                                                       const double *d_lon_out, const double *d_lat_out,
                                                       double mean_dlat, double mean_dlon, int device, void *stream, int use_caller_stream,
                                                       fg_plan **plan_out)
{
  PlanGuard g;
  if (int rc = plan_base(FG_CONSERVE_ORDER1, ntiles_in, nx_in, ny_in, nx_out, ny_out, device, &g.pl)) return rc;
  if (int rc = check_grid_ptrs(ntiles_in, {d_lon_in, d_lat_in}, {d_lon_out, d_lat_out})) return rc;
  if (use_caller_stream) adopt_stream(g.pl, stream);
  const long nx = gc_lonlat_search(g.pl, d_lon_in, d_lat_in, d_mask_in, d_lon_out, d_lat_out, DstExtents{mean_dlat, mean_dlon});
  return g.hand_over(nx, plan_out);
}

extern "C" long fg_plan_create_great_circle_lonlat(int ntiles_in, const int *nx_in, const int *ny_in,
                                                   const double *const *lon_in, const double *const *lat_in, const double *const *mask_in,
                                                   int nx_out, int ny_out, const double *lon_out, const double *lat_out,
                                                   int device, fg_plan **plan_out)
{
  PlanGuard g;
  if (int rc = plan_base(FG_CONSERVE_ORDER1, ntiles_in, nx_in, ny_in, nx_out, ny_out, device, &g.pl)) return rc;
  StagedGrids s(g.pl);
  if (int rc = stage_host_grids(g.pl, lon_in, lat_in, mask_in, lon_out, lat_out, &s)) return rc;
  const long nx = gc_lonlat_search(g.pl, s.lon.data(), s.lat.data(), s.masks(), s.lon_out, s.lat_out,
                                   dst_extents_host(nx_out, ny_out, lon_out, lat_out));
  if (nx >= 0) s.up.done();
  return g.hand_over(nx, plan_out);
}

extern "C" long fg_plan_create_polylist(int order, int npoly, const int *n, const double *lon, const double *lat, const double *lon_avg,
                                        const double *area_ref, int nx_out, int ny_out, const double *lon_out, const double *lat_out,
                                        int device, fg_plan **plan_out)
{
  if (npoly < 1 || !n || !lon || !lat || !lon_avg || !area_ref || !lon_out || !lat_out) return fail(FG_ERR_ARG, "null argument");
  PlanGuard g;
  const int one = 1;
  if (int rc = plan_base(order, 1, &npoly, &one, nx_out, ny_out, device, &g.pl)) return rc;
  fg_plan *pl = g.pl;
  if (order == 2) pl->f_stride = npoly;
  const size_t npo = (size_t)(nx_out + 1) * (ny_out + 1);
  HostUpload up{pl};
  pl->polys = FgPolyList{up.put(n, npoly), up.put(lon, (size_t)npoly * 8), up.put(lat, (size_t)npoly * 8), up.put(lon_avg, npoly),
                         up.put(area_ref, npoly), npoly};
  double *d_lo = up.put(lon_out, npo), *d_la = up.put(lat_out, npo);
  if (!up.run()) return fail(FG_ERR_HIP, "polygon upload failed (out of device memory?)");
  const DstExtents x = dst_extents_host(nx_out, ny_out, lon_out, lat_out);
  const double *none[1] = {nullptr};
  const long nx = plan_search(pl, SearchIn{.lon_in = none, .lat_in = none, .lon_out = d_lo, .lat_out = d_la, .mean_dlat = x.dlat,
                                           .mean_dlon = x.dlon, .rect_hint = x.rect_hint});
  if (nx >= 0) { pl->release(d_lo); pl->release(d_la); }
  return g.hand_over(nx, plan_out);
}

extern "C" int fg_plan_set_stream(fg_plan *pl, void *stream)
{
  if (!pl) return fail(FG_ERR_ARG, "null plan");
  HIPCHK(hipSetDevice(pl->device));
  HIPCHK(hipStreamSynchronize(pl->stream));
  adopt_stream(pl, stream);
  return 0;
}

int fg_plan_borrow_stream(fg_plan *pl, void *stream, void **saved, int *saved_own)
{
  if (!pl) return fail(FG_ERR_ARG, "null plan");
  HIPCHK(hipSetDevice(pl->device));
  HIPCHK(hipStreamSynchronize(pl->stream));
  *saved = (void *)pl->stream; *saved_own = pl->own_stream ? 1 : 0;
  pl->stream = (hipStream_t)stream; pl->own_stream = false;
  return 0;
}
void fg_plan_return_stream(fg_plan *pl, void *saved, int saved_own)
{
  if (!pl) return;
  pl->stream = (hipStream_t)saved; pl->own_stream = saved_own != 0;
}

extern "C" int fg_plan_create_empty(int order, int ntiles_in, const int *nx_in, const int *ny_in,
                                    int nx_out, int ny_out, int device, fg_plan **plan_out)
{
  PlanGuard g;
  if (int rc = plan_base(order, ntiles_in, nx_in, ny_in, nx_out, ny_out, device, &g.pl)) return rc;
  fg_plan *pl = g.pl;
  std::vector<FgTile> th(pl->ntiles);
  for (int m = 0; m < pl->ntiles; m++) th[m] = FgTile{nullptr, nullptr, pl->nx_in[m], pl->ny_in[m], pl->cell_off[m]};
  pl->tiles_dev = pl->alloc<FgTile>(pl->ntiles + 1);
  if (!pl->tiles_dev || hipMemcpy(pl->tiles_dev, th.data(), sizeof(FgTile) * th.size(), hipMemcpyHostToDevice) != hipSuccess)
    return fail(FG_ERR_HIP, "out of device memory");
  return (int)g.hand_over(0, plan_out);
}

extern "C" int fg_plan_trim(fg_plan *pl)
{
  if (!pl) return fail(FG_ERR_ARG, "null plan");
  if (!pl->searched) return fail(FG_ERR_STATE, "fg_plan_trim: plan holds no exchange cells");
  HIPCHK(hipSetDevice(pl->device));
  HIPCHK(hipStreamSynchronize(pl->stream));
  const size_t n = (size_t)pl->nx + 1;
  auto shrink = [&](auto *&ptr) -> int {
    if (!ptr) return 0;
    typedef typename std::remove_reference<decltype(*ptr)>::type T;
    T *q = pl->alloc<T>(n);
    if (!q) return fail(FG_ERR_HIP, "out of device memory");
    if (hipMemcpyAsync(q, ptr, n * sizeof(T), hipMemcpyDeviceToDevice, pl->stream) != hipSuccess) return fail(FG_ERR_HIP, "device copy failed");
    void *old = ptr; ptr = q;
    HIPCHK(hipStreamSynchronize(pl->stream));
    pl->release(old);
    return 0;
  };
  int rc = 0;
  if ((rc = shrink(pl->x_src)) || (rc = shrink(pl->x_dst)) || (rc = shrink(pl->x_area)) || (rc = shrink(pl->x_c1)) || (rc = shrink(pl->x_c2))) return rc;
  if (pl->perm && (rc = shrink(pl->perm))) return rc;
  return 0;
}

extern "C" long fg_plan_nxgrid(const fg_plan *pl) { return pl ? pl->nx : FG_ERR_ARG; }
extern "C" long fg_plan_ncells_in(const fg_plan *pl) { return pl ? pl->nsrc : FG_ERR_ARG; }
extern "C" long fg_plan_ncells_out(const fg_plan *pl) { return pl ? pl->ndst : FG_ERR_ARG; }
extern "C" int fg_plan_order(const fg_plan *pl) { return pl ? pl->order : FG_ERR_ARG; }
extern "C" int fg_plan_device(const fg_plan *pl) { return pl ? pl->device : FG_ERR_ARG; }
extern "C" double *fg_plan_cell_sums_dev(fg_plan *pl) { return (pl && pl->order == 2) ? pl->sums : nullptr; }
extern "C" int fg_plan_copy_cell_sums(fg_plan *pl, double *dst_dev)
{
  if (!pl || !dst_dev) return fail(FG_ERR_ARG, "null argument");
  if (pl->order != 2 || !pl->sums) return fail(FG_ERR_STATE, "plan holds no order-2 cell sums");
  HIPCHK(hipSetDevice(pl->device));
  HIPCHK(hipMemcpyAsync(dst_dev, pl->sums, 3 * (size_t)pl->nsrc * sizeof(double), hipMemcpyDeviceToDevice, pl->stream));
  HIPCHK(hipStreamSynchronize(pl->stream));
  return 0;
}
static int accumulate_cell_sums(fg_plan *pl, double *total_dev, const int *cells_dev, int ncells, bool sync)
{
  if (!pl || !total_dev) return fail(FG_ERR_ARG, "null argument");
  if (pl->order != 2 || !pl->searched || pl->finalized || !pl->xoff)
    return fail(FG_ERR_STATE, "fg_plan_accumulate_cell_sums: needs a searched, not yet finalized order-2 plan");
  HIPCHK(hipSetDevice(pl->device));
  if (pl->nx > 0)
    fgd_accumulate_cell_sums(cells_dev ? ncells : pl->nsrc, cells_dev, pl->nsrc, pl->xoff, pl->x_area, pl->x_c1, pl->x_c2, total_dev, pl->stream);
  if (sync) HIPCHK(hipStreamSynchronize(pl->stream));
  HIPCHK(hipGetLastError());
  return 0;
}
extern "C" int fg_plan_accumulate_cell_sums(fg_plan *pl, double *total_dev, const int *cells_dev, int ncells)
{
  return accumulate_cell_sums(pl, total_dev, cells_dev, ncells, true);
}
extern "C" int fg_plan_accumulate_cell_sums_async(fg_plan *pl, double *total_dev, const int *cells_dev, int ncells)
{
  return accumulate_cell_sums(pl, total_dev, cells_dev, ncells, false);
}
extern "C" void *fg_plan_stream(fg_plan *pl) { return pl ? (void *)pl->stream : nullptr; }
extern "C" int fg_plan_sync(fg_plan *pl)
{
  if (!pl) return fail(FG_ERR_ARG, "null plan");
  HIPCHK(hipStreamSynchronize(pl->stream));
  return 0;
}
extern "C" int fg_plan_stats(const fg_plan *pl, long *stats, int n)
{
  if (!pl || !stats) return fail(FG_ERR_ARG, "null argument");
  for (int k = 0; k < n && k < FG_NSTATS; k++) stats[k] = pl->stats[k];
  return 0;
}

static int build_csr(fg_plan *pl, const FgSrcRec *cen)
{
  hipStream_t st = pl->stream;
  const int ndst = pl->ndst;
  const long nx = pl->nx;
  HIPCHK(hipSetDevice(pl->device));
  if (!pl->src_idx_f) {
    pl->src_idx_f = pl->alloc<int>(pl->nsrc + 1);
    if (!pl->src_idx_f) return fail(FG_ERR_HIP, "out of device memory");
    fgd_src_field_index(pl->order, pl->tiles_dev, pl->ntiles, pl->nsrc, pl->src_idx_f, st);
  }
  void *scratch = nullptr;
  if (!pl->rows_built) {
    const long t_rows = fgd_scan_tiles(ndst);
    const size_t zb = 256 + (size_t)t_rows * sizeof(unsigned long long) + 2 * ((size_t)ndst + 1) * sizeof(int);
    char *z = pl->alloc<char>(zb);
    pl->perm = pl->alloc<FgRowEnt>(nx + 1);
    pl->csr.row_ptr = pl->alloc<int>(ndst + 1);
    if (!z || !pl->perm || !pl->csr.row_ptr) return fail(FG_ERR_HIP, "out of device memory");
    HIPCHK(hipMemsetAsync(z, 0, zb, st));
    unsigned long long *lb = (unsigned long long *)(z + 256);
    int *row_cnt = (int *)(z + 256 + (size_t)t_rows * sizeof(unsigned long long));
    fgd_csr_count(nx, pl->x_dst, row_cnt, st);
    fgd_exclusive_scan1(row_cnt, ndst, pl->csr.row_ptr, lb, (unsigned *)z, (unsigned long long *)(z + 8), (unsigned *)(z + 16), st);
    fgd_csr_fill(nx, pl->x_src, pl->x_dst, pl->csr.row_ptr, row_cnt + ndst + 1, pl->perm, st);
    scratch = z;
  }
  if (pl->order == 2) pl->csr.e2 = pl->alloc<FgCsrEntry2>(nx + 1);
  else pl->csr.e1 = pl->alloc<FgCsrEntry1>(nx + 1);
  if (!pl->csr.e1 && !pl->csr.e2) return fail(FG_ERR_HIP, "out of device memory");
  int *sg_tmp = pl->alloc<int>(3 * (size_t)(nx + 1));
  const int long_rows = !pl->rect && !pl->great_circle && pl->stats[FG_STAT_DEFERRED] > 0 && nx > 4 * (long)ndst;
  fgd_csr_sortgather(pl->order, ndst, nx, pl->perm, pl->x_area, pl->x_c1, pl->x_c2, pl->src_idx_f, cen, pl->csr, st, sg_tmp, nx + 1,
                     long_rows);
  HIPCHK(hipStreamSynchronize(st));
  HIPCHK(hipGetLastError());
  pl->release(scratch); pl->release(pl->perm); pl->perm = nullptr; pl->release(sg_tmp);
  if (!pl->red_partial) { pl->red_partial = pl->alloc<double>(1024); pl->red_result = pl->alloc<double>(260); }
  if (!pl->red_partial || !pl->red_result) return fail(FG_ERR_HIP, "out of device memory");
  return 0;
}

extern "C" int fg_plan_finalize(fg_plan *pl, const double *total_cell_sums_dev)
{
  if (!pl) return fail(FG_ERR_ARG, "null plan");
  if (!pl->searched) return fail(FG_ERR_STATE, "fg_plan_finalize: plan holds no search result");
  if (pl->finalized && pl->fused && !total_cell_sums_dev) return 0;
  if (pl->finalized) return fail(FG_ERR_STATE, pl->fused ? "fg_plan_finalize: the plan was finalized by its search (fg_set_search_finalize) from its own "
                                                          "per-cell sums; totals over several plans need the two-step sequence"
                                                         : "fg_plan_finalize: already finalized");
  HIPCHK(hipSetDevice(pl->device));
  PhaseTimer pt; pt.start(g_profiling != 0, pl->stream);
  pt.begin(PH_FINALIZE);
  if (pl->order == 2) {
    pl->cen = pl->alloc<FgSrcRec>((size_t)pl->nsrc + 1);
    if (!pl->cen) return fail(FG_ERR_HIP, "out of device memory");
    const double *tot = total_cell_sums_dev ? total_cell_sums_dev : pl->sums;
    fgd_centroids(pl->nsrc, pl->S, tot, pl->cen, pl->stream);
    pl->dist_pending = true;
  }
  int rc = build_csr(pl, pl->order == 2 ? pl->cen : nullptr);
  if (rc) return rc;
  pt.end();
  HIPCHK(hipStreamSynchronize(pl->stream));
  pl->phase_ms[PH_FINALIZE] = 0; pt.collect(pl->phase_ms);
  pl->finalized = true;
  return 0;
}

extern "C" int fg_plan_phase_ms(fg_plan *pl, float *ms, int n)
{
  if (!pl || !ms) return fail(FG_ERR_ARG, "null argument");
  if (pl->apply_spans > 0) {
    HIPCHK(hipSetDevice(pl->device));
    HIPCHK(hipStreamSynchronize(pl->stream));
    float acc[PH_COUNT] = {0};
    pl->apply_pt.collect(acc);
    pl->phase_ms[PH_APPLY] = acc[PH_APPLY] / pl->apply_spans;
    pl->apply_spans = 0;
  }
  for (int k = 0; k < n && k < PH_COUNT; k++) ms[k] = pl->phase_ms[k];
  return 0;
}

extern "C" int fg_plan_get_xgrid(const fg_plan *pl, int *t_in, int *i_in, int *j_in, int *i_out, int *j_out,
                                 double *area, double *c1, double *c2)
{
  if (!pl) return fail(FG_ERR_ARG, "null plan");
  if (!pl->searched) return fail(FG_ERR_STATE, "plan holds no exchange cells");
  HIPCHK(hipSetDevice(pl->device));
  HIPCHK(hipStreamSynchronize(pl->stream));
  const long nx = pl->nx;
  if (nx == 0) return 0;
  if (pl->dist_pending) {
    fg_plan *m = const_cast<fg_plan *>(pl);
    fgd_distances(nx, pl->x_src, pl->x_area, pl->cen, m->x_c1, m->x_c2, pl->stream);
    HIPCHK(hipStreamSynchronize(pl->stream));
    m->dist_pending = false;
  }
  std::vector<XferJob> jobs;
  int *idx = nullptr;
  struct PutBack { int *&p; ~PutBack() { g_pool.put(p); } } put_back{idx};
  if (t_in || i_in || j_in || i_out || j_out) {
    idx = (int *)g_pool.get(pl->device, 5 * (size_t)nx * sizeof(int));
    if (!idx) return fail(FG_ERR_HIP, "out of device memory");
    fgd_xgrid_indices(nx, pl->x_src, pl->x_dst, pl->tiles_dev, pl->ntiles, pl->nx_out, idx, idx + nx, idx + 2 * nx, idx + 3 * nx,
                      idx + 4 * nx, pl->stream);
    HIPCHK(hipStreamSynchronize(pl->stream));
    int *dst[5] = {t_in, i_in, j_in, i_out, j_out};
    for (int q = 0; q < 5; q++) if (dst[q]) jobs.push_back(XferJob{dst[q], idx + (size_t)q * nx, (size_t)nx * sizeof(int), true});
  }
  if (area) jobs.push_back(XferJob{area, pl->x_area, (size_t)nx * sizeof(double), true});
  if (pl->order == 2) {
    if (c1) jobs.push_back(XferJob{c1, pl->x_c1, (size_t)nx * sizeof(double), true});
    if (c2) jobs.push_back(XferJob{c2, pl->x_c2, (size_t)nx * sizeof(double), true});
  }
  if (!xfer_pool().run(pl->device, jobs)) return fail(FG_ERR_HIP, "fg_plan_get_xgrid: device -> host copy failed");
  return 0;
}

extern "C" int fg_plan_get_polygons(const fg_plan *pl, int maxv, int *n_out, double *v0, double *v1, double *v2)
{
  if (!pl || !n_out || !v0 || !v1) return fail(FG_ERR_ARG, "null argument");
  if (!pl->searched || !pl->have_geom || !pl->x_src) return fail(FG_ERR_STATE, "fg_plan_get_polygons: needs a plan from a search (cell records)");
  if (pl->great_circle && !v2) return fail(FG_ERR_ARG, "fg_plan_get_polygons: a great-circle plan returns x, y, z");
  if (maxv < 3 || maxv > 64) return fail(FG_ERR_ARG, "fg_plan_get_polygons: maxv must be 3..64");
  HIPCHK(hipSetDevice(pl->device));
  HIPCHK(hipStreamSynchronize(pl->stream));
  const long nx = pl->nx, CH = 1L << 20;
  const int dev = pl->device;
  for (long k0 = 0; k0 < nx; k0 += CH) {
    const long n = std::min(CH, nx - k0);
    const size_t nv = (size_t)n * maxv;
    int *d_n = (int *)g_pool.get(dev, n * sizeof(int));
    double *d_v = (double *)g_pool.get(dev, 3 * nv * sizeof(double));
    struct Put { void *a, *b; ~Put() { g_pool.put(a); g_pool.put(b); } } put{d_n, d_v};
    if (!d_n || !d_v) return fail(FG_ERR_HIP, "out of device memory");
    std::vector<XferJob> jobs;
    if (pl->great_circle) {
      double *a = (double *)g_pool.get(dev, (size_t)n * 12 * 8), *b = (double *)g_pool.get(dev, (size_t)n * 12 * 8);
      double *o = (double *)g_pool.get(dev, (size_t)n * FG_GC_POLY_CAP * 3 * 8), *ar = (double *)g_pool.get(dev, (size_t)n * 8);
      struct Put4 { void *p[4]; ~Put4() { for (void *q : p) g_pool.put(q); } } put4{{a, b, o, ar}};
      if (!a || !b || !o || !ar) return fail(FG_ERR_HIP, "out of device memory");
      fgd_xgrid_gather_gc(n, pl->x_src + k0, pl->x_dst + k0, pl->S, pl->D, a, b, pl->stream);
      fgd_gc_clip_batch((int)n, a, b, o, d_n, ar, pl->stream);
      fgd_split_xyz(n, maxv, o, d_v, d_v + nv, d_v + 2 * nv, pl->stream);
      HIPCHK(hipStreamSynchronize(pl->stream));
      jobs.push_back(XferJob{v2 + (size_t)k0 * maxv, d_v + 2 * nv, nv * sizeof(double), true});
    } else {
      fgd_xgrid_polygons(n, pl->x_src + k0, pl->x_dst + k0, pl->S, pl->D, pl->rect ? &pl->rect_tab : nullptr, maxv, d_n, d_v, d_v + nv, pl->stream);
      HIPCHK(hipStreamSynchronize(pl->stream));
    }
    HIPCHK(hipGetLastError());
    jobs.push_back(XferJob{n_out + k0, d_n, (size_t)n * sizeof(int), true});
    jobs.push_back(XferJob{v0 + (size_t)k0 * maxv, d_v, nv * sizeof(double), true});
    jobs.push_back(XferJob{v1 + (size_t)k0 * maxv, d_v + nv, nv * sizeof(double), true});
    if (!xfer_pool().run(dev, jobs)) return fail(FG_ERR_HIP, "fg_plan_get_polygons: device -> host copy failed");
  }
  return 0;
}

extern "C" int fg_plan_get_cell_area(const fg_plan *pl, double *area_in, double *area_out)
{
  if (!pl) return fail(FG_ERR_ARG, "null plan");
  if (!pl->have_geom) return fail(FG_ERR_STATE, "plan holds no cell records");
  HIPCHK(hipSetDevice(pl->device));
  HIPCHK(hipStreamSynchronize(pl->stream));
  if (area_in) HIPCHK(hipMemcpy(area_in, pl->S.area, (size_t)pl->nsrc * sizeof(double), hipMemcpyDeviceToHost));
  if (area_out) HIPCHK(hipMemcpy(area_out, pl->D.area, (size_t)pl->ndst * sizeof(double), hipMemcpyDeviceToHost));
  return 0;
}

extern "C" int fg_plan_get_cell_struct(const fg_plan *pl, int which, double *lat_min, double *lat_max, double *lon_min,
                                       double *lon_max, double *lon_avg, int *nvert, double *vlon, double *vlat)
{
  if (!pl) return fail(FG_ERR_ARG, "null plan");
  if (!pl->have_geom) return fail(FG_ERR_STATE, "plan holds no cell records");
  HIPCHK(hipSetDevice(pl->device));
  HIPCHK(hipStreamSynchronize(pl->stream));
  FgCells tmp{};
  std::vector<void *> tmp_blocks;
  struct Free { std::vector<void *> &v; ~Free() { for (void *p : v) g_pool.put(p); } } free_tmp{tmp_blocks};
  if (which && pl->rect) {
    const size_t nd = (size_t)pl->ndst;
    auto get = [&](size_t bytes) { void *p = g_pool.get(pl->device, bytes); if (p) tmp_blocks.push_back(p); return p; };
    tmp.lat_min = (double *)get(nd * 8); tmp.lat_max = (double *)get(nd * 8); tmp.lon_min = (double *)get(nd * 8);
    tmp.lon_max = (double *)get(nd * 8); tmp.lon_avg = (double *)get(nd * 8); tmp.nv = (int *)get(nd * 4); tmp.verts = (double *)get(nd * 128);
    tmp.area = pl->D.area;
    if (tmp_blocks.size() != 7) return fail(FG_ERR_HIP, "out of device memory");
    FgRect R = pl->rect_tab;
    fgd_rect_materialize(pl->ndst, R, tmp, pl->stream);
    HIPCHK(hipStreamSynchronize(pl->stream));
  }
  const FgCells &c = which ? (pl->rect ? tmp : pl->D) : pl->S;
  size_t n = which ? pl->ndst : pl->nsrc;
  if (lat_min) HIPCHK(hipMemcpy(lat_min, c.lat_min, n * sizeof(double), hipMemcpyDeviceToHost));
  if (lat_max) HIPCHK(hipMemcpy(lat_max, c.lat_max, n * sizeof(double), hipMemcpyDeviceToHost));
  if (lon_min) HIPCHK(hipMemcpy(lon_min, c.lon_min, n * sizeof(double), hipMemcpyDeviceToHost));
  if (lon_max) HIPCHK(hipMemcpy(lon_max, c.lon_max, n * sizeof(double), hipMemcpyDeviceToHost));
  if (lon_avg) HIPCHK(hipMemcpy(lon_avg, c.lon_avg, n * sizeof(double), hipMemcpyDeviceToHost));
  if (nvert) HIPCHK(hipMemcpy(nvert, c.nv, n * sizeof(int), hipMemcpyDeviceToHost));
  if (vlon || vlat) {
    std::vector<double> v(n * 16);
    HIPCHK(hipMemcpy(v.data(), c.verts, n * 16 * sizeof(double), hipMemcpyDeviceToHost));
    for (size_t k = 0; k < n; k++)
      for (int l = 0; l < 8; l++) {
        if (vlon) vlon[k * 8 + l] = v[k * 16 + l];
        if (vlat) vlat[k * 8 + l] = v[k * 16 + 8 + l];
      }
  }
  return 0;
}

extern "C" int fg_plan_set_xgrid(fg_plan *pl, long nxgrid, const int *t_in, const int *i_in, const int *j_in,
                                 const int *i_out, const int *j_out, const double *area,
                                 const double *di_in, const double *dj_in)
{
  if (!pl) return fail(FG_ERR_ARG, "null plan");
  if (nxgrid < 0 || (nxgrid > 0 && (!t_in || !i_in || !j_in || !i_out || !j_out || !area))) return fail(FG_ERR_ARG, "null exchange-cell array");
  if (pl->order == 2 && nxgrid > 0 && (!di_in || !dj_in)) return fail(FG_ERR_ARG, "order 2 needs di_in/dj_in");
  if (pl->finalized || pl->searched) return fail(FG_ERR_STATE, "fg_plan_set_xgrid needs a plan from fg_plan_create_empty");
  HIPCHK(hipSetDevice(pl->device));
  std::vector<int> s(nxgrid), d(nxgrid);
  for (long k = 0; k < nxgrid; k++) {
    int m = t_in[k];
    if (m < 0 || m >= pl->ntiles || i_in[k] < 0 || i_in[k] >= pl->nx_in[m] || j_in[k] < 0 || j_in[k] >= pl->ny_in[m] ||
        i_out[k] < 0 || i_out[k] >= pl->nx_out || j_out[k] < 0 || j_out[k] >= pl->ny_out)
      return fail(FG_ERR_ARG, "exchange cell %ld has an index outside its grid", k);
    s[k] = pl->cell_off[m] + j_in[k] * pl->nx_in[m] + i_in[k];
    d[k] = j_out[k] * pl->nx_out + i_out[k];
  }
  pl->nx = nxgrid;
  pl->x_src = pl->alloc<int>(nxgrid + 1); pl->x_dst = pl->alloc<int>(nxgrid + 1);
  pl->x_area = pl->alloc<double>(nxgrid + 1);
  if (pl->order == 2) { pl->x_c1 = pl->alloc<double>(nxgrid + 1); pl->x_c2 = pl->alloc<double>(nxgrid + 1); }
  if (!pl->x_src || !pl->x_dst || !pl->x_area || (pl->order == 2 && (!pl->x_c1 || !pl->x_c2))) return fail(FG_ERR_HIP, "out of device memory");
  if (nxgrid > 0) {
    HIPCHK(hipMemcpy(pl->x_src, s.data(), nxgrid * sizeof(int), hipMemcpyHostToDevice));
    HIPCHK(hipMemcpy(pl->x_dst, d.data(), nxgrid * sizeof(int), hipMemcpyHostToDevice));
    HIPCHK(hipMemcpy(pl->x_area, area, nxgrid * sizeof(double), hipMemcpyHostToDevice));
    if (pl->order == 2) {
      HIPCHK(hipMemcpy(pl->x_c1, di_in, nxgrid * sizeof(double), hipMemcpyHostToDevice));
      HIPCHK(hipMemcpy(pl->x_c2, dj_in, nxgrid * sizeof(double), hipMemcpyHostToDevice));
    }
  }
  pl->searched = true;
  int rc = build_csr(pl, nullptr);
  if (rc) return rc;
  pl->finalized = true;
  return 0;
}

extern int g_apply_vec, g_apply_ep;
extern "C" void fg_set_apply_ep(int on) { g_apply_ep = on ? 1 : 0; }

extern int g_apply_xcd;
extern "C" void fg_set_apply_xcd(int on) { g_apply_xcd = on < 0 ? 0 : on; }
extern "C" void fg_set_apply_vec(int v) { g_apply_vec = (v >= 4) ? 4 : (v >= 2 ? 2 : (v == 1 ? 1 : 0)); }

static void apply_span_begin(fg_plan *pl, hipStream_t st)
{
  pl->apply_pt.start(g_profiling != 0 && pl->apply_spans < 256, st);
  pl->apply_pt.begin(PH_APPLY);
}
static void apply_span_end(fg_plan *pl)
{
  pl->apply_pt.end();
  if (pl->apply_pt.on) pl->apply_spans++;
}

static int levels_pad(int nz) { return nz > 4 ? 8 : (nz > 2 ? 4 : 2); }

static int ensure_il_rs(fg_plan *pl)
{
  if (!pl->il_rs) {
    pl->il_rs = pl->alloc<double>((size_t)pl->ndst * 16);
    if (!pl->il_rs) return fail(FG_ERR_HIP, "out of device memory");
  }
  return 0;
}

static int ensure_il_scratch(fg_plan *pl, bool want_rs)
{
  if (!pl->il_out) {
    pl->il_out = pl->alloc<double>((size_t)pl->ndst * 8);
    if (pl->order == 2) pl->il_m = pl->alloc<double>((size_t)pl->nsrc * 24);
    else pl->il_f = pl->alloc<double>((size_t)pl->f_stride * 8);
    if (!pl->il_out || (pl->order == 2 ? !pl->il_m : !pl->il_f)) return fail(FG_ERR_HIP, "out of device memory");
  }
  return want_rs ? ensure_il_rs(pl) : 0;
}

static void interleave_field(fg_plan *pl, const double *f, int nbp, int nbv, hipStream_t st)
{
  const double *ins[3] = {f, nullptr, nullptr};
  double *outs[3] = {pl->il_f, nullptr, nullptr};
  const long lds[3] = {pl->f_stride, 0, 0}, ns[3] = {pl->f_stride, 0, 0};
  fgd_interleave3(nbp, 1, ins, lds, ns, outs, nbv, st);
}

extern "C" int fg_plan_apply(fg_plan *pl, const double *data, const double *grad_x, const double *grad_y,
                             const int *grad_mask, int has_missing, double missing, int nz,
                             double *out, double *gsum_out)
{
  if (!pl || !data || !out) return fail(FG_ERR_ARG, "null argument");
  if (!pl->finalized) return fail(FG_ERR_STATE, "fg_plan_apply: call fg_plan_finalize first");
  if (nz < 1) return fail(FG_ERR_ARG, "nz must be >= 1");
  if (nz > 1 && has_missing) return fail(FG_ERR_ARG, "conserve_interp: has_missing should be false when nz > 1");
  if (pl->order == 2 && (!grad_x || !grad_y)) return fail(FG_ERR_ARG, "order 2 needs grad_x and grad_y");
  if (pl->order == 2 && has_missing && !grad_mask) return fail(FG_ERR_ARG, "order 2 with missing values needs grad_mask");
  HIPCHK(hipSetDevice(pl->device));
  hipStream_t st = pl->stream;
  const double miss = has_missing ? missing : -1.e20;
  const int ndst = pl->ndst;
  const int nchunk = (nz + 7) / 8;
  if (nchunk > 256) return fail(FG_ERR_ARG, "nz too large for one call (max 2048 levels)");
  if (gsum_out && pl->row_sum_cap < ndst) {
    pl->release(pl->row_sum);
    pl->row_sum = pl->alloc<double>(ndst);
    if (!pl->row_sum) { pl->row_sum_cap = 0; return fail(FG_ERR_HIP, "out of device memory"); }
    pl->row_sum_cap = ndst;
  }
  if (nz > 1) { int rc = ensure_il_scratch(pl, gsum_out != nullptr); if (rc) return rc; }
  apply_span_begin(pl, st);
  int nred = 0;
  for (int k0 = 0; k0 < nz; k0 += 8) {
    const int nbv = (nz - k0 < 8) ? nz - k0 : 8;
    const double *f = data + (size_t)k0 * pl->f_stride;
    const double *gx = grad_x ? grad_x + (size_t)k0 * pl->nsrc : nullptr;
    const double *gy = grad_y ? grad_y + (size_t)k0 * pl->nsrc : nullptr;
    double *o = out + (size_t)k0 * ndst;
    if (nbv == 1) {
      fgd_apply1(pl->order, ndst, pl->csr, f, gx, gy, grad_mask, has_missing, miss, o, gsum_out ? pl->row_sum : nullptr, st, pl->nx);
      if (gsum_out) fgd_reduce_sum(pl->row_sum, ndst, pl->red_partial, pl->red_result + nred++, st);
    } else {
      const int nbp = levels_pad(nbv);
      double *rs = gsum_out ? pl->il_rs : nullptr;
      if (pl->order == 2) {
        fgd_merge3(nbp, pl->nsrc, pl->src_idx_f, f, pl->f_stride, gx, gy, pl->nsrc, nbv, pl->il_m, st);
        fgd_apply_il_merged(nbp, ndst, pl->nx, pl->csr, pl->il_m, miss, o, rs, (long)ndst, nbv, st);
      } else {
        interleave_field(pl, f, nbp, nbv, st);
        fgd_apply_il(1, nbp, ndst, pl->csr, pl->il_f, nullptr, nullptr, miss, o, rs, (long)ndst, nbv, st, pl->nx);
      }
      if (gsum_out) fgd_reduce_sum(pl->il_rs, (long)ndst * nbp, pl->red_partial, pl->red_result + nred++, st);
    }
  }
  apply_span_end(pl);
  if (gsum_out) {
    double parts[256];
    HIPCHK(hipMemcpyAsync(parts, pl->red_result, nred * sizeof(double), hipMemcpyDeviceToHost, st));
    HIPCHK(hipStreamSynchronize(st));
    double g = 0;
    for (int k = 0; k < nred; k++) g += parts[k];
    *gsum_out = g;
  }
  HIPCHK(hipGetLastError());
  return 0;
}

extern "C" int fg_plan_apply_records(fg_plan *pl, int nz, const double *rec, double *out, double *gsum_out)
{
  if (!pl || !rec || !out) return fail(FG_ERR_ARG, "null argument");
  if (!pl->finalized) return fail(FG_ERR_STATE, "fg_plan_apply_records: call fg_plan_finalize first");
  if (pl->order != 2) return fail(FG_ERR_ARG, "fg_plan_apply_records: records carry gradients, the plan is first order");
  if (nz < 1 || nz > 8) return fail(FG_ERR_ARG, "fg_plan_apply_records: 1 to 8 levels per call");
  HIPCHK(hipSetDevice(pl->device));
  hipStream_t st = pl->stream;
  const int ndst = pl->ndst, nbp = levels_pad(nz);
  if (gsum_out) { int rc = ensure_il_rs(pl); if (rc) return rc; }
  apply_span_begin(pl, st);
  fgd_apply_il_merged(nbp, ndst, pl->nx, pl->csr, rec, -1.e20, out, gsum_out ? pl->il_rs : nullptr, (long)ndst, nz, st);
  if (gsum_out) fgd_reduce_sum(pl->il_rs, (long)ndst * nbp, pl->red_partial, pl->red_result, st);
  apply_span_end(pl);
  if (gsum_out) {
    HIPCHK(hipMemcpyAsync(gsum_out, pl->red_result, sizeof(double), hipMemcpyDeviceToHost, st));
    HIPCHK(hipStreamSynchronize(st));
  }
  HIPCHK(hipGetLastError());
  return 0;
}

extern "C" int fg_plan_levels_capacity(void) { return FG_LEVELS_CAP; }
int fg_plan_is_finalized(const fg_plan *pl) { return pl && pl->finalized; }

static int levels_scratch(fg_plan *pl, bool want_rs, bool want_il)
{
  if (want_il) { int rc = ensure_il_scratch(pl, false); if (rc) return rc; }
  if (want_il && pl->order == 2 && !pl->lv_bits) {
    pl->lv_bits = pl->alloc<unsigned char>(pl->nsrc > 0 ? pl->nsrc : 1);
    if (!pl->lv_bits) return fail(FG_ERR_HIP, "out of device memory");
  }
  return want_rs ? ensure_il_rs(pl) : 0;
}

static int levels_gsum(fg_plan *pl, int nbv, int *nred, double **gsum_out, bool last)
{
// ... 930 lines not shown
```

fre-nctools_amd/csrc/xgrid_device.h:

```cpp
#pragma once
#include <hip/hip_runtime.h>

struct FgTile {
  const double *lon;
  const double *lat;
  int nx, ny;
  int cell_off;
};

struct FgTileXyz {
  const double *x, *y, *z;
  int nx, ny;
  int cell_off;
};
#define G_ERRBIT_GC_CONVEX1 16u
#define G_ERRBIT_GC_CONVEX2 32u
#define G_ERRBIT_GC_CLIP    64u

struct FgCells {
  double *lat_min, *lat_max, *lon_min, *lon_max, *lon_avg, *area;
  int *nv;
  double *verts;
};

struct FgBins {
  int nblat, nblon;
  double inv_wlat, inv_wlon;
};

struct FgBinEntry {
  double lat_min, lat_max, lon_min, lon_max, lon_avg;
  int d;
  int row0;
};

enum {
  FG_STAT_PAIRS = 0,
  FG_STAT_NONEMPTY = 1,
  FG_STAT_NXGRID = 2,
  FG_STAT_BORDERLINE = 3,
  FG_STAT_BINS = 4,
  FG_STAT_BIN_ENTRIES = 5,
  FG_STAT_DEFERRED = 6,
  FG_STAT_HEAVY = 7,
  FG_STAT_BELOW = 8,
  FG_STAT_EXACT = 9,
  FG_NSTATS = 10
};

#define FG_REG_ALIGN 512
#define FG_NREG 64
#define FG_FILL_STRIDE 32
struct FgPairSpace {
  int *src, *dst;
  unsigned *fill;
  int regcap, nreg;
};
#ifdef __HIPCC__
__device__ __forceinline__ bool d_pair_live(const FgPairSpace &ps, int p)
{
  const unsigned first = blockIdx.x * blockDim.x;
  const unsigned r = first / (unsigned)ps.regcap;
  const unsigned f = ps.fill[r * FG_FILL_STRIDE];
  return (unsigned)p - r * (unsigned)ps.regcap < (f < (unsigned)ps.regcap ? f : (unsigned)ps.regcap);
}
#endif
static inline long fgd_pairs_total(const FgPairSpace &ps) { return (long)ps.regcap * ps.nreg; }
#ifdef __HIPCC__
__device__ __forceinline__ unsigned long long d_ord_key(double v)
{
  const unsigned long long b = (unsigned long long)__double_as_longlong(v);
  return (b >> 63) ? ~b : (b | 0x8000000000000000ull);
}
__device__ __forceinline__ double d_ord_val(unsigned long long k)
{
  const unsigned long long b = (k >> 63) ? (k & 0x7fffffffffffffffull) : ~k;
  return __longlong_as_double((long long)b);
}
#endif

#define FG_TILESET_MAX 8
struct FgTileSet { FgTile t[FG_TILESET_MAX]; int n; };

struct FgLl2xGrid { const double *lon, *lat; double *x, *y, *z; long n; };
struct FgLl2xSet { FgLl2xGrid g[FG_TILESET_MAX]; int n; };
#define G_ERRBIT_LL2X 256u
void fgd_latlon2xyz(const FgLl2xGrid *grids, int ngrids, unsigned *err, hipStream_t st);

struct FgCounters {
  unsigned long long total[4];
  unsigned long long rows_total;
  unsigned long long band_keys[2];
  unsigned long long xtot;
  unsigned err[4];
  int heavy_cnt;
  unsigned rect_bad;
  int defer_cnt, big_cnt;
  int gc_list2_cnt;
  unsigned long long stats[FG_NSTATS];
};
#define G_ERRBIT_LOOKBACK 128u

long fgd_scan_tiles(long n);
void fgd_exclusive_scan1(const int *in, long n, int *out, unsigned long long *status, unsigned *ticket,
                         unsigned long long *total_dev, unsigned *err, hipStream_t st);

void fgd_exclusive_scan2(const int *in_a, long n_a, int *out_a, unsigned long long *status_a, unsigned *ticket_a, unsigned long long *total_a,
                         const int *in_b, long n_b, int *out_b, unsigned long long *status_b, unsigned *ticket_b, unsigned long long *total_b,
                         unsigned *err, hipStream_t st);

void fgd_cell_struct2(const FgTileSet &ts, const FgTile *tiles_in, FgTile *tiles_out, int ntiles, int nsrc, int ndst, FgCells S, FgCells D,
                      FgBins b, int *slot_cnt, int order, int *src_idx_f, double *sums, unsigned *err, hipStream_t st,
                      unsigned long long *band_keys = nullptr, int cull = 0, double dst_tlon = 3.14159265358979323846);
void fgd_cell_struct(const FgTile *tiles_dev, int ntiles, int ncells, FgCells c, unsigned *err, hipStream_t st);
void fgd_band_keys(const double *lat, long n, unsigned long long *band_keys, hipStream_t st);
void fgd_bin_count(int ncells, FgCells c, FgBins b, int *slot_cnt, hipStream_t st);
void fgd_bin_fill(int ndst, FgCells D, FgBins b, int *slot_fill, const int *slot_start, FgBinEntry *entries, int cap,
                  int nsrc, FgCells S, const double *mask, int *heavy_list, int *heavy_cnt, hipStream_t st);
void fgd_candidates1(int nsrc, FgCells S, const double *mask, FgBins b, const int *slot_start, const FgBinEntry *entries, int ecap,
                     FgPairSpace ps, int *pair_beg, int *pair_cnt, const int *heavy_list, const int *heavy_cnt, int *big_list, int *big_cnt,
                     hipStream_t st);
#define RECT_COLW 8
struct FgRect {
  const double *lon_ax;
  const double *lat_ax;
  const double *col;
  const double *col_min, *col_max, *col_avg;
  const double *hdr;
  const double *row;
  const unsigned *bad;
  int nx, ny;
};
void fgd_rect_tables(const double *lon, const double *lat, int nx, int ny, double *hdr, double *lat_ax, double *lon_ax, double *col,
                     double *col_min, double *col_max, double *col_avg, double *row, unsigned *bad, unsigned *err, hipStream_t st,
                     double dst_tlon = 3.14159265358979323846);
void fgd_cell_struct2r(const FgTileSet &ts, const FgTile *tiles_in, FgTile *tiles_out, int ntiles, int nsrc, int ndst, FgCells S, double *area_out,
                       FgRect R, const double *mask, int order, int *src_idx_f, double *sums, unsigned *err, hipStream_t st,
                       unsigned long long *band_keys, int cull, int *heavy_list, int *heavy_cnt, FgPairSpace ps, int *pair_beg, int *pair_cnt,
                       int *big_list, int *big_cnt);
void fgd_rect_materialize(int ndst, FgRect R, FgCells D, hipStream_t st);
struct FgPolyList { const int *n; const double *lon, *lat; const double *lon_avg, *area; int npoly; };
void fgd_polylist_records(FgPolyList P, FgCells S, int *src_idx_f, double *sums, const FgRect *rect, int *heavy_list, int *heavy_cnt,
                          unsigned *err, hipStream_t st);
void fgd_candidates_rect(int nsrc, FgCells S, const double *mask, FgRect R, FgPairSpace ps, int *pair_beg, int *pair_cnt,
                         const int *heavy_list, const int *heavy_cnt, int *big_list, int *big_cnt, hipStream_t st, int listed_only);
void fgd_clip_general(int order, FgPairSpace ps, FgCells S, const double *mask, FgCells D,
              double *tmp_area, double *tmp_clon, double *tmp_clat, int *nacc, int *defer_list, int *defer_cnt,
              unsigned long long *stats, unsigned *err, hipStream_t st, const FgRect *rect = nullptr, int *row_cnt = nullptr,
              int *tmp_rowpos = nullptr);
void fgd_clip_quad(int order, FgPairSpace ps, FgCells S, const double *mask, FgCells D,
              double *tmp_area, double *tmp_clon, double *tmp_clat, int *nacc, int *defer_list, int *defer_cnt,
              unsigned long long *stats, unsigned *err, hipStream_t st, const FgRect *rect = nullptr, int *row_cnt = nullptr,
              int *tmp_rowpos = nullptr);
struct alignas(8) FgRowEnt { int n, s; };
struct alignas(16) FgSrcRec { double cen_lon, cen_lat; };
struct FgCompactIo {
  const int *pair_beg, *pair_cnt;
  const double *tmp_area, *tmp_clon, *tmp_clat;
  const int *xoff;
  int *x_src, *x_dst;
  double *x_area, *x_c1, *x_c2;
  int *row_cnt, *x_rowpos;
  const int *tmp_rowpos;
  const int *row_ptr; FgRowEnt *perm;
  double *sums;
  const int *big_list;
  const int *big_cnt;
  FgCounters *dc;
  long xcap;
};
void fgd_compact(int order, int nsrc, FgPairSpace ps, const FgCompactIo &io, hipStream_t st);
void fgd_centroids(int nsrc, FgCells S, const double *sums, FgSrcRec *cen, hipStream_t st);
void fgd_distances(long nx, const int *x_src, const double *x_area, const FgSrcRec *cen, double *x_c1, double *x_c2, hipStream_t st);

struct FgCsrEntry1 { int idx_f; int pad; double area; };
struct FgCsrEntry2 { int idx_f; int idx_g; double area, di, dj; };
struct FgCsr {
  int *row_ptr;
  FgCsrEntry1 *e1;
  FgCsrEntry2 *e2;
};
void fgd_csr_count(long nx, const int *x_dst, int *row_cnt, hipStream_t st);
void fgd_csr_fill(long nx, const int *x_src, const int *x_dst, const int *row_ptr, int *row_fill, FgRowEnt *perm, hipStream_t st);
void fgd_csr_fill_pos(long nx_cap, const unsigned long long *nx_dev, const int *x_src, const int *x_dst, const int *row_ptr, const int *x_rowpos,
                      FgRowEnt *perm, hipStream_t st);
void fgd_csr_sortgather(int order, int ndst, long nx, const FgRowEnt *perm, const double *x_area, const double *x_c1, const double *x_c2,
                        const int *src_idx_f, const FgSrcRec *cen, FgCsr csr, hipStream_t st, int *tmp = nullptr, long ntmp = 0,
                        int long_rows = 0);
void fgd_src_field_index(int order, const FgTile *tiles_dev, int ntiles, int nsrc, int *src_idx_f, hipStream_t st);
void fgd_apply1(int order, int ndst, FgCsr csr, const double *f, const double *gx, const double *gy, const int *gmask,
                int has_missing, double missing, double *out, double *row_sum, hipStream_t st, long nx = -1);
void fgd_apply_il(int order, int nb, int ndst, FgCsr csr, const double *f, const double *gx, const double *gy, double missing,
                  double *out, double *row_sum, long out_ld, int nb_valid, hipStream_t st, long nx = -1);
void fgd_interleave(int nb_pad, long n, const double *in, long ld, int nb_valid, double *out, hipStream_t st);
void fgd_apply_il_merged(int nb, int ndst, long nx, FgCsr csr, const double *rec, double missing, double *out, double *row_sum, long out_ld,
                         int nb_valid, hipStream_t st);
void fgd_merge3(int nb_pad, long n, const int *src_idx_f, const double *f, long ld_f, const double *gx, const double *gy, long ld_g,
                int nb_valid, double *out, hipStream_t st);
void fgd_interleave3(int nb_pad, int narr, const double *const *in, const long *ld, const long *n, double *const *out, int nb_valid,
                     hipStream_t st);
void fgd_deinterleave(int nb_pad, long n, const double *in, long ld, int nb_valid, double *out, hipStream_t st);
#define FG_LEVELS_CAP 256
void fgd_apply_levels8(int order, int ndst, long nx, FgCsr csr, const double *rec, const unsigned char *gbits, double missing, double *out,
                       double *row_sum, long ld, int nb_valid, hipStream_t st);
void fgd_gmask_bits(long n, const int *gmask, long ld, int nb, unsigned char *bits, hipStream_t st);
void fgd_apply_frac(int ndst, FgCsr csr, const double *data, double *out, hipStream_t st);
void fgd_reduce_sum(const double *v, long n, double *partial, double *result, hipStream_t st);
void fgd_xgrid_indices(long nx, const int *x_src, const int *x_dst, const FgTile *tiles_dev, int ntiles, int nx_out,
                       int *t_in, int *i_in, int *j_in, int *i_out, int *j_out, hipStream_t st);

struct FgApplyEx {
  const double *weight;
  const double *cell_area;
  const double *field_area;
  const double *cell_area_out;
  const int *gmask;
  const double *xdata;
  double area_missing, missing;
  int has_missing, sum;
};
#define FG_XERR_AREA_MISSING 1
#define FG_XERR_ABOVE 2
#define FG_XERR_BELOW 4
void fgd_apply_ex(int order, int ndst, FgCsr csr, const double *f, const double *gx, const double *gy, FgApplyEx o,
                  double *out, double *row_sum, int *err, hipStream_t st, long nx = -1);
void fgd_mono_bounds(const FgTile *tiles_dev, int ntiles, int nsrc, const int *src_idx_f, const double *f, double missing,
                     double *fbmax, double *fbmin, double *fmax, double *fmin, hipStream_t st);
void fgd_mono_xdata(long nx, FgCsr csr, const double *f, const double *gx, const double *gy, const int *gmask, double missing,
                    double *xdata, double *fmax, double *fmin, hipStream_t st);
void fgd_mono_limit(long nx, FgCsr csr, const double *f, double missing, const double *fbmax, const double *fbmin,
                    const double *fmax, const double *fmin, double *xdata, int *err, hipStream_t st);

struct FgBox { const double *lon, *lat; int nx, ny; };
void fgd_clip_box(int order, FgPairSpace ps, FgBox box, FgTile quad, FgCells S, FgCells D,
                  const double *mask_box, const double *mask_quad, double *tmp_area, double *tmp_clon, double *tmp_clat, int *nacc,
                  unsigned long long *stats, unsigned *err, hipStream_t st);
void fgd_box_area_no_adjust(FgBox box, double *area, hipStream_t st);
void fgd_box_cell_boxes(FgBox box, FgCells c, hipStream_t st);
void fgd_clip_single(const double *lon_in, const double *lat_in, int n_in, double ll_lon, double ll_lat, double ur_lon, double ur_lat,
                     double *lon_out, double *lat_out, int *n_out, hipStream_t st);
void fgd_box_ctr(double ll_lon, double ll_lat, double ur_lon, double ur_lat, double clon, double *out, hipStream_t st);
void fgd_grid_area_no_adjust(int nx, int ny, const double *lon, const double *lat, double *area, hipStream_t st);

void fgd_accumulate_cell_sums(int n, const int *cells, int nsrc, const int *xoff, const double *xa, const double *c1, const double *c2,
                              double *total, hipStream_t st);

void fgd_gc_cell_struct(const FgTileXyz *tiles_dev, int ntiles, int ncells, FgCells c, hipStream_t st,
                        unsigned long long *band_keys = nullptr, int band_mode = 0);
void fgd_gc_clip(FgPairSpace ps, FgCells S, const double *mask, FgCells D,
                 double *tmp_area, int *nacc, int *defer_list, int *defer_cnt, unsigned long long *stats, unsigned *err, hipStream_t st);
struct GcSplit {
  unsigned *meta;
  int *tbase;
  unsigned *task;
  double *res;
  unsigned tcap;
  unsigned *ntask;
  int *list, *list_cnt;
  int *list2_cnt;
  long list_cap;
  int *order;
  unsigned *ocnt;
};
void fgd_gc_clip_split(FgPairSpace ps, FgCells S, const double *mask, FgCells D, double *tmp_area, int *nacc, GcSplit g,
                       unsigned long long *stats, unsigned *err, hipStream_t st, hipStream_t st2, hipEvent_t e1, hipEvent_t e2);
#define FG_GC_POLY_CAP 16
void fgd_gc_clip_batch(int n, const double *a, const double *b, double *out, int *n_out, double *area, hipStream_t st);
void fgd_gc_area_batch(int npoly, int stride_pts, const double *xyz, const int *n, double *area, hipStream_t st);

#define FG_POLY_STRIDE 24
void fgd_poly_clip(int npoly, const double *lon1, const double *lat1, const int *n1, const double *lon2, const double *lat2,
                   const int *n2, double *lon_out, double *lat_out, int *n_out, hipStream_t st);
void fgd_poly_op(int op, int npoly, double *lon, double *lat, int *n, const double *clon, double *result, hipStream_t st);
void fgd_xgrid_polygons(long n, const int *x_src, const int *x_dst, FgCells S, FgCells D, const FgRect *rect, int maxv,
                        int *n_out, double *lon_out, double *lat_out, hipStream_t st);
void fgd_xgrid_gather_gc(long n, const int *x_src, const int *x_dst, FgCells S, FgCells D, double *a, double *b, hipStream_t st);
void fgd_split_xyz(long n, int maxv, const double *xyz, double *x, double *y, double *z, hipStream_t st);
void fgd_sincos_probe(long n, const double *x, double *s, double *c, hipStream_t st);

void fgd_pack_interior(const void *tiles, int ntiles, long ncells, long F, int nz, const double *src, double *dst, hipStream_t st);
void fgd_halo_gather(long F, int nz, const int *map, double *data, hipStream_t st);
void fgd_grad_c2l(const void *tiles, int ntiles, long ncells, long F, int nz, const double *data, const double *const *geom,
                  double *grad_x, double *grad_y, hipStream_t st);
void fgd_grad_c2l_rec(const void *tiles, int ntiles, long ncells, long F, int nz, int nb_pad, const double *data,
                      const double *const *geom, double *rec, hipStream_t st);
void fgd_c2l_records(const void *tiles, int ntiles, long ncells, int nz, int nb_pad, const double *src, const int *cell_of,
                     const double *const *geom, double *rec, hipStream_t st);
void fgd_c2l_records_levels(const void *tiles, int ntiles, long ncells, int nz, const double *src, const int *cell_of,
                            const double *const *geom, double missing, double *rec, unsigned char *gbits, hipStream_t st);
void fgd_grad_mask(const void *tiles, int ntiles, long ncells, long F, int nz, const double *data, double missing, int *mask, hipStream_t st);
size_t fgd_c2l_tile_size(void);
void fgd_c2l_tile_fill(void *dst, int idx, int nx, int ny, long cell_off, long f_off, long dx_off, long dy_off, long ew_off, long es_off);
```

fre-nctools_amd/csrc/xgrid_kernels.hip:

```cpp
#include <algorithm>
#include "xgrid_device.h"
#ifndef FG_EXP
#define FG_EXP 0
#endif
static __shared__ double fgs_lds_tab[112 * 4];
#define FGS_TAB(k, j) fgs_lds_tab[(k) * 4 + (j)]
#include "geom.hip.h"
__device__ __forceinline__ void d_load_trig_table()
{
  for (int i = threadIdx.x; i < 112 * 4; i += blockDim.x) fgs_lds_tab[i] = FG_SINCOS_TAB[i >> 2][i & 3];
  __syncthreads();
}

#define SCAN_THREADS 256
#define SCAN_ITEMS   8
#define SCAN_CHUNK   (SCAN_THREADS * SCAN_ITEMS)
#define LB_AGG   (1ull << 62)
#define LB_INC   (2ull << 62)
#define LB_MASK  ((1ull << 62) - 1ull)
#define LB_SPIN_LIMIT (1u << 22)

__device__ __forceinline__ unsigned wave_incl_scan(unsigned v, int lane)
{
#pragma unroll
// ... 1402 lines not shown
    }
    double shift = 0.0;
    {
      double dx = lon_out_avg - lon_in_avg;
      if (dx < -G_PI) shift = G_TPI; else if (dx > G_PI) shift = -G_TPI;
    }
    bool wrap = false;
    for (int k = 0; k < n1; k++) { double xv = sv[k]; if (xv > G_TPI || xv < 0.0) wrap = true; }
    for (int k = 0; k < n1; k++) {
      double xv = sv[k]; if (wrap) xv = d_pimod1(xv);
      sh_a[k][tid] = make_double2(xv, sv[8 + k]);
    }
#pragma unroll
    for (int k = 0; k < G_MAXV; k++)
      if (k < n2) {
        double xv = dvx[k]; if (shift != 0.0) xv += shift; if (wrap) xv = d_pimod1(xv);
        sh_cut[k][tid] = make_double2(xv, dvy[k]);
      }
    double2 (*cur)[GEN_THREADS] = sh_a;
    double2 (*nxt)[GEN_THREADS] = sh_b;
    int n_cur = n1;
    bool overflow = false, parallel = false;
    double2 e0 = sh_cut[n2 - 1][tid];
    for (int e = 0; e < n2 && n_cur > 0 && !overflow; e++) {
      double2 e1 = sh_cut[e][tid];
      const double x2_0 = e0.x, y2_0 = e0.y, x2_1 = e1.x, y2_1 = e1.y;
      double2 lastv = cur[n_cur - 1][tid];
      double x1_0 = lastv.x, y1_0 = lastv.y;
      int inside_last = d_inside_edge(x2_0, y2_0, x2_1, y2_1, x1_0, y1_0);
      int n_new = 0;
      for (int k = 0; k < n_cur; k++) {
        double2 cv = cur[k][tid];
        double x1_1 = cv.x, y1_1 = cv.y;
        int inside = d_inside_edge(x2_0, y2_0, x2_1, y2_1, x1_1, y1_1);
        if (inside != inside_last) {
          double dy1 = y1_1 - y1_0;
          double dy2 = y2_1 - y2_0;
          double dx1 = x1_1 - x1_0;
          double dx2 = x2_1 - x2_0;
          double ds1 = y1_0 * x1_1 - y1_1 * x1_0;
          double ds2 = y2_0 * x2_1 - y2_1 * x2_0;
          double determ = dy2 * dx1 - dy1 * dx2;
          if (fabs(determ) < 1.0e-30) parallel = true;
          if (n_new < GEN_CAP) nxt[n_new][tid] = make_double2((dx2 * ds1 - dx1 * ds2) / determ,
                                                              (dy2 * ds1 - dy1 * ds2) / determ);
          else overflow = true;
          n_new++;
        }
        if (inside) {
          if (n_new < GEN_CAP) nxt[n_new][tid] = make_double2(x1_1, y1_1);
          else overflow = true;
          n_new++;
        }
        x1_0 = x1_1; y1_0 = y1_1; inside_last = inside;
      }
      n_cur = n_new;
      double2 (*t)[GEN_THREADS] = cur; cur = nxt; nxt = t;
      e0 = e1;
    }
    if (overflow) { atomicOr(err, G_ERRBIT_OVERFLOW); pair_dst[p] = -1; continue; }
    if (parallel) atomicOr(err, G_ERRBIT_PARALLEL);
    ClipOut o; o.area = -1.0; o.clon = 0; o.clat = 0;
    if (n_cur > 0) {
      const double *px = (const double *)&cur[0][tid];
      d_finish_pair<ORDER, 2 * GEN_THREADS>(px, px + 1, n_cur, mask ? mask[s] : 1.0, S.area[s], D.area[d],
                                            lon_in_avg, &o, stats);
    }
    if (o.area >= 0) {
      tmp_area[p] = o.area;
      if (ORDER == 2) { tmp_clon[p] = o.clon; tmp_clat[p] = o.clat; }
      atomicAdd(&nacc[s], 1);
      if (row_cnt) tmp_rowpos[p] = atomicAdd(&row_cnt[d], 1);
    } else {
      pair_dst[p] = -1;
      if (o.area == -2.0) atomicAdd(&stats[FG_STAT_BELOW], 1ull);
    }
  }
}

#define CP_SPAN (256 + CP_SMALL)
static_assert(CP_SMALL % 64 == 0 && CP_SMALL <= 256, "the halo lanes of k_compact are whole waves of its 256-lane block");

struct CpPair { int s, d, beg, cnt, row; long x0; int na; double a, l, t; bool mine; };

__device__ __forceinline__ int d_row_slot(int *row_cnt, bool take, int d, int lane)
{
  const int key = take ? d : -1 - lane;
  const int prev = __shfl_up(key, 1, 64);
  const bool head = (lane == 0) || (key != prev);
  const unsigned long long hm = __ballot(head), am = __ballot(take);
  int slot = 0;
  if (!am) return 0;
  if (4 * __popcll(hm & am) > 3 * __popcll(am)) {
    if (take) slot = atomicAdd(&row_cnt[d], 1);
    return slot;
  }
  unsigned long long rem = am;
  for (int it = 0; rem && it < 8; it++) {
    const int lead = __ffsll((long long)rem) - 1;
    const int d0 = __shfl(d, lead);
    const unsigned long long grp = __ballot(take && d == d0) & rem;
    int base = 0;
    if (lane == lead) base = atomicAdd(&row_cnt[d0], __popcll(grp));
    base = __shfl(base, lead);
    if ((grp >> lane) & 1ull) slot = base + __popcll(grp & ((1ull << lane) - 1ull));
    rem &= ~grp;
  }
  if ((rem >> lane) & 1ull) slot = atomicAdd(&row_cnt[d], 1);
  return slot;
}

template <int ORDER, bool HALO>
__device__ __forceinline__ void d_cp_load(const FgPairSpace &ps, const FgCompactIo &io, int p0, int tid, unsigned live_end, CpPair &c, CpPair &h)
{
  constexpr int N = HALO ? 2 : 1;
  const int *const rowpos = io.tmp_rowpos ? io.tmp_rowpos : ps.dst;
  int p[N], pc[N], s[N], d[N], rp[N], beg[N], cnt[N], rb[N], x0[N], x1[N];
  bool ok[N];
  double a[N], l[N], t[N];
#pragma unroll
  for (int k = 0; k < N; k++) { p[k] = p0 + 256 * k + tid; ok[k] = (unsigned)p[k] < live_end; pc[k] = ok[k] ? p[k] : p0; }
#pragma unroll
  for (int k = 0; k < N; k++) {
    s[k] = ps.src[pc[k]]; d[k] = ps.dst[pc[k]]; rp[k] = rowpos[pc[k]];
    if (k == 0) { a[k] = io.tmp_area[pc[k]]; if (ORDER == 2) { l[k] = io.tmp_clon[pc[k]]; t[k] = io.tmp_clat[pc[k]]; } }
  }
#pragma unroll
  for (int k = 0; k < N; k++) {
    beg[k] = io.pair_beg[s[k]]; cnt[k] = io.pair_cnt[s[k]]; rb[k] = io.row_ptr[max(d[k], 0)];
    x0[k] = io.xoff[s[k]]; x1[k] = io.xoff[s[k] + 1];
  }
#pragma unroll
  for (int k = 0; k < N; k++) {
    const bool mine = ok[k] && cnt[k] <= CP_SMALL && beg[k] >= p0 && beg[k] < p0 + 256;
    if (k == 1) {
      a[k] = 0; l[k] = 0; t[k] = 0;
      if (mine && d[k] >= 0) { a[k] = io.tmp_area[p[k]]; if (ORDER == 2) { l[k] = io.tmp_clon[p[k]]; t[k] = io.tmp_clat[p[k]]; } }
    }
    CpPair &o = k ? h : c;
    o.s = ok[k] ? s[k] : 0; o.d = ok[k] ? d[k] : -1; o.beg = ok[k] ? beg[k] : 0; o.cnt = ok[k] ? cnt[k] : 0;
    o.mine = mine; o.x0 = mine ? x0[k] : 0; o.na = mine ? x1[k] - x0[k] : 0; o.row = (int)((unsigned)rb[k] + (unsigned)rp[k]);
    o.a = a[k]; o.l = (ORDER == 2) ? l[k] : 0.0; o.t = (ORDER == 2) ? t[k] : 0.0;
  }
}

template <int ORDER>
__device__ __forceinline__ long d_cp_place(const FgCompactIo &io, const CpPair &c, int p0, const int *sh_d, double (*sh_v)[CP_SPAN])
{
  if (!c.mine || c.d < 0 || c.x0 + c.na > io.xcap) return -1;
  int rank = 0;
  const int lb = c.beg - p0;
  for (int j = 0; j < c.cnt; j++) rank += ((unsigned)sh_d[lb + j] < (unsigned)c.d) ? 1 : 0;
  const long pos = c.x0 + rank;
  io.x_src[pos] = c.s; io.x_dst[pos] = c.d; io.x_area[pos] = c.a;
  if (ORDER == 2) { io.x_c1[pos] = c.l; io.x_c2[pos] = c.t; sh_v[0][lb + rank] = c.a; sh_v[1][lb + rank] = c.l; sh_v[2][lb + rank] = c.t; }
  if (io.tmp_rowpos) io.perm[c.row] = FgRowEnt{(int)pos, c.s};
  else return pos;
  return -1;
}

#define RANK_WORDS 1024
#define BIG_STAGE 512
#define BIG_BLOCKS 512
#define CP_LDS_DOUBLES (RANK_WORDS + RANK_WORDS / 2 + 3 * BIG_STAGE)

template <int ORDER>
__device__ __forceinline__ void d_compact_big(int nsrc, const FgPairSpace &ps, const FgCompactIo &io, double *lds)
{
  unsigned long long *bits = (unsigned long long *)lds;
  int *pref = (int *)(lds + RANK_WORDS);
  double (*sval)[BIG_STAGE] = (double (*)[BIG_STAGE])(lds + RANK_WORDS + RANK_WORDS / 2);
  __shared__ int smin, smax;
  if (blockIdx.x == 0 && threadIdx.x < 64) {
    unsigned long long f = 0; unsigned mx = 0;
    for (int r = threadIdx.x; r < ps.nreg; r += 64) { const unsigned v = ps.fill[r * FG_FILL_STRIDE]; f += v; mx = max(mx, v); }
#pragma unroll
    for (int o = 32; o; o >>= 1) { f += __shfl_xor(f, o); mx = max(mx, (unsigned)__shfl_xor((int)mx, o)); }
    if (threadIdx.x == 0) { io.dc->total[1] = f; io.dc->total[3] = mx; }
  }
  const int nb = *io.big_cnt;
  for (int h = blockIdx.x; h < nb; h += BIG_BLOCKS) {
    const int s = io.big_list[h];
    const int o = io.pair_beg[s], c = io.pair_cnt[s];
    const long x0 = io.xoff[s];
    const int na = io.xoff[s + 1] - (int)x0;
    if (threadIdx.x == 0) { smin = 0x7fffffff; smax = -1; }
    __syncthreads();
    int lmin = 0x7fffffff, lmax = -1;
    for (int k = threadIdx.x; k < c; k += 256) { const int d = ps.dst[o + k]; if (d >= 0) { lmin = min(lmin, d); lmax = max(lmax, d); } }
    if (lmax >= 0) { atomicMin(&smin, lmin); atomicMax(&smax, lmax); }
    __syncthreads();
    const int dmin = smin, dmax = smax;
    const long span = (long)dmax - dmin + 1;
    const bool bitmap = dmax >= 0 && span <= (long)RANK_WORDS * 64;
    if (bitmap) {
      const int nw = (int)((span + 63) >> 6);
      for (int w = threadIdx.x; w < nw; w += 256) bits[w] = 0ull;
      __syncthreads();
      for (int k = threadIdx.x; k < c; k += 256) {
        const int d = ps.dst[o + k];
        if (d >= 0) atomicOr(&bits[(d - dmin) >> 6], 1ull << ((d - dmin) & 63));
      }
      __syncthreads();
      const int per = (nw + 255) / 256, w0 = threadIdx.x * per, w1 = min(nw, w0 + per);
      int mine = 0;
      for (int w = w0; w < w1; w++) mine += __popcll(bits[w]);
      unsigned tot;
      const int before = (int)block_incl_scan((unsigned)mine, &tot) - mine;
      int run = before;
      for (int w = w0; w < w1; w++) { pref[w] = run; run += __popcll(bits[w]); }
      __syncthreads();
    }
    const bool ahead = na <= BIG_STAGE;
    const int *const rowpos = io.tmp_rowpos ? io.tmp_rowpos : ps.dst;
    double acc = 0;
    for (int c0 = 0; c0 < max(na, 1); c0 += BIG_STAGE) {
      for (int k = threadIdx.x; k < c; k += 256) {
        const int p = o + k;
        const int d = ps.dst[p];
        double a = 0, l = 0, t = 0;
        int row = 0;
        if (ahead) {
          a = io.tmp_area[p]; if (ORDER == 2) { l = io.tmp_clon[p]; t = io.tmp_clat[p]; }
          row = (int)((unsigned)rowpos[p] + (unsigned)io.row_ptr[max(d, 0)]);
        }
        if (d < 0) continue;
        int rank;
        if (bitmap) { const int w = (d - dmin) >> 6, b = (d - dmin) & 63; rank = pref[w] + __popcll(bits[w] & ((1ull << b) - 1ull)); }
        else { rank = 0; for (int j = 0; j < c; j++) rank += ((unsigned)ps.dst[o + j] < (unsigned)d) ? 1 : 0; }
        if (rank < c0 || rank >= c0 + BIG_STAGE) continue;
        const long pos = x0 + rank;
        if (pos >= io.xcap) continue;
        if (!ahead) {
          a = io.tmp_area[p]; if (ORDER == 2) { l = io.tmp_clon[p]; t = io.tmp_clat[p]; }
          if (io.tmp_rowpos) row = io.row_ptr[d] + io.tmp_rowpos[p];
        }
        io.x_src[pos] = s; io.x_dst[pos] = d; io.x_area[pos] = a;
        if (ORDER == 2) {
          io.x_c1[pos] = l; io.x_c2[pos] = t;
          sval[0][rank - c0] = a; sval[1][rank - c0] = l; sval[2][rank - c0] = t;
        }
        if (io.tmp_rowpos) io.perm[row] = FgRowEnt{(int)pos, s};
        else io.x_rowpos[pos] = atomicAdd(&io.row_cnt[d], 1);
      }
      __syncthreads();
      if (ORDER == 2 && threadIdx.x < 3 && x0 + na <= io.xcap) {
        const double *v = sval[threadIdx.x];
        const int n = min(BIG_STAGE, na - c0);
        int k = 0;
        for (; k + 8 <= n; k += 8) {
          double t[8];
#pragma unroll
          for (int u = 0; u < 8; u++) t[u] = v[k + u];
#pragma unroll
          for (int u = 0; u < 8; u++) acc += t[u];
        }
        for (; k < n; k++) acc += v[k];
      }
      __syncthreads();
    }
    if (ORDER == 2 && io.sums && threadIdx.x < 3) io.sums[(size_t)threadIdx.x * nsrc + s] = acc;
  }
}

template <int ORDER>
__global__ __launch_bounds__(256) void k_compact(int nsrc, FgPairSpace ps, FgCompactIo io)
{
  __shared__ double lds[CP_LDS_DOUBLES];
  if ((int)blockIdx.x < BIG_BLOCKS) { d_compact_big<ORDER>(nsrc, ps, io, lds); return; }
  int *sh_d = (int *)lds;
  double (*sh_v)[CP_SPAN] = (double (*)[CP_SPAN])(lds + CP_SPAN / 2 + 8);
  const int tid = threadIdx.x;
  const int p0 = ((int)blockIdx.x - BIG_BLOCKS) * 256;
  const unsigned r = (unsigned)p0 / (unsigned)ps.regcap;
  const unsigned rfill = ps.fill[r * FG_FILL_STRIDE];
  const unsigned live_end = r * (unsigned)ps.regcap + (rfill < (unsigned)ps.regcap ? rfill : (unsigned)ps.regcap);
  if ((unsigned)p0 >= live_end) return;
  CpPair c, h; h.mine = false; h.d = -1;
  if (tid < CP_SMALL) { d_cp_load<ORDER, true>(ps, io, p0, tid, live_end, c, h); sh_d[256 + tid] = h.d; }
  else d_cp_load<ORDER, false>(ps, io, p0, tid, live_end, c, h);
  sh_d[tid] = c.d;
  __syncthreads();
  const bool first = (unsigned)(p0 + tid) < live_end && p0 + tid == c.beg;
  {
    const long pos = d_cp_place<ORDER>(io, c, p0, sh_d, sh_v);
    if (!io.tmp_rowpos) { const int slot = d_row_slot(io.row_cnt, pos >= 0, c.d, tid & 63); if (pos >= 0) io.x_rowpos[pos] = slot; }
  }
  if (tid < CP_SMALL) {
    const long pos = d_cp_place<ORDER>(io, h, p0, sh_d, sh_v);
    if (!io.tmp_rowpos) { const int slot = d_row_slot(io.row_cnt, pos >= 0, h.d, tid & 63); if (pos >= 0) io.x_rowpos[pos] = slot; }
  }
  if (ORDER != 2 || !io.sums) return;
  __syncthreads();
  if (!first || !c.mine || c.x0 + c.na > io.xcap) return;
  double sa = 0, sl = 0, st = 0;
  const int lb = c.beg - p0;
  for (int k = 0; k < c.na; k++) { sa += sh_v[0][lb + k]; sl += sh_v[1][lb + k]; st += sh_v[2][lb + k]; }
  io.sums[c.s] = sa; io.sums[nsrc + c.s] = sl; io.sums[2 * (size_t)nsrc + c.s] = st;
}

__global__ __launch_bounds__(256) void k_centroids(int nsrc, FgCells S, const double *sums, FgSrcRec *cen)
{
  const int s = blockIdx.x * blockDim.x + threadIdx.x;
  double a = 0, ca = 1, cl = 0, ct = 0;
  int nv = 0;
  bool whole = false;
  if (s < nsrc && (a = sums[s]) > 0) {
    const double sl = sums[nsrc + s], st = sums[2 * (size_t)nsrc + s], sa = S.area[s];
    nv = S.nv[s];
    if (nv > 0) {
      ca = sa;
      if (fabs(a - ca) / ca < 1.e-3) {
        cl = sl / a;
        ct = st / a;
      } else whole = true;
    }
  }
  if (__syncthreads_or(whole)) {
    d_load_trig_table();
    if (whole) {
      double x[G_MAXV], y[G_MAXV];
      int n = nv;
      const double *vp = S.verts + (size_t)s * 16;
      for (int k = 0; k < G_MAXV; k++) { x[k] = vp[k]; y[k] = vp[8 + k]; }
      cl = d_poly_ctrlon<1>(x, y, n, S.lon_avg[s]) / ca;
      ct = d_poly_ctrlat<1>(x, y, n) / ca;
    }
  }
  if (s < nsrc) cen[s] = FgSrcRec{cl, ct};
}

__global__ __launch_bounds__(256) void k_distances(long nx, const int *x_src, const double *x_area, const FgSrcRec *cen, double *x_c1,
                                                    double *x_c2)
{
  long n = (long)blockIdx.x * blockDim.x + threadIdx.x;
  if (n >= nx) return;
  int s = x_src[n];
  double a = x_area[n];
  double di = x_c1[n] / a, dj = x_c2[n] / a;
  di -= cen[s].cen_lon; dj -= cen[s].cen_lat;
  x_c1[n] = di; x_c2[n] = dj;
}

static inline int nblk(long n, int t) { return (int)((n + t - 1) / t); }

void fgd_cell_struct(const FgTile *tiles_dev, int ntiles, int ncells, FgCells c, unsigned *err, hipStream_t st)
{
  if (ncells > 0) k_cell_struct<<<nblk(ncells, 256), 256, 0, st>>>(tiles_dev, ntiles, ncells, c, err);
}

void fgd_cell_struct2(const FgTileSet &ts, const FgTile *tiles_in, FgTile *tiles_out, int ntiles, int nsrc, int ndst, FgCells S, FgCells D,
                      FgBins b, int *slot_cnt, int order, int *src_idx_f, double *sums, unsigned *err, hipStream_t st,
                      unsigned long long *band_keys, int cull, double dst_tlon)
{
  const int nbS = nblk(nsrc, 256), nbD = nblk(ndst, 256);
  if (nbS + nbD > 0)
    k_cell_struct2<<<nbS + nbD, 256, 0, st>>>(ts, tiles_in, tiles_out, ntiles, nsrc, ndst, nbS, S, D, b, slot_cnt, order, src_idx_f, sums, err,
                                              band_keys, cull, dst_tlon);
}

void fgd_bin_count(int ncells, FgCells c, FgBins b, int *slot_cnt, hipStream_t st)
{
  if (ncells > 0) k_bin_count<<<nblk(ncells, 256), 256, 0, st>>>(ncells, c, b, slot_cnt);
}

void fgd_bin_fill(int ndst, FgCells D, FgBins b, int *slot_fill, const int *slot_start, FgBinEntry *entries, int cap,
                  int nsrc, FgCells S, const double *mask, int *heavy_list, int *heavy_cnt, hipStream_t st)
{
  const int nbD = nblk(ndst, 256), nbS = nblk(nsrc, 256);
  if (nbD + nbS > 0)
    k_bin_fill<<<nbD + nbS, 256, 0, st>>>(ndst, nbD, D, b, slot_fill, slot_start, entries, cap, nsrc, S, mask, heavy_list, heavy_cnt);
}

void fgd_candidates1(int nsrc, FgCells S, const double *mask, FgBins b, const int *slot_start, const FgBinEntry *entries, int ecap,
                     FgPairSpace ps, int *pair_beg, int *pair_cnt, const int *heavy_list, const int *heavy_cnt, int *big_list, int *big_cnt,
                     hipStream_t st)
{
  if (nsrc <= 0) return;
  const int nbR = nblk((long)nsrc * CAND_G, 64);
  const int H = min(8 * HEAVY_BLOCKS, max(64, nblk(nsrc, 8)));
  k_candidates1<<<nbR + H, 64, 0, st>>>(nsrc, H, S, mask, b, slot_start, entries, ecap, ps, pair_beg, pair_cnt, heavy_list, heavy_cnt, big_list, big_cnt);
}

void fgd_clip_quad(int order, FgPairSpace ps, FgCells S, const double *mask, FgCells D,
                   double *tmp_area, double *tmp_clon, double *tmp_clat, int *nacc, int *defer_list, int *defer_cnt,
                   unsigned long long *stats, unsigned *err, hipStream_t st, const FgRect *rect, int *row_cnt, int *tmp_rowpos)
{
  const long np = fgd_pairs_total(ps);
  if (np <= 0) return;
  const FgRect R = rect ? *rect : FgRect{};
  const int g = nblk(np, CLIP_THREADS);
#define FG_LAUNCH_QUAD(O, RC) k_clip_quad<O, RC><<<g, CLIP_THREADS, 0, st>>>(ps, S, mask, D, R, tmp_area, tmp_clon, tmp_clat, nacc, defer_list, defer_cnt, stats, err, row_cnt, tmp_rowpos)
  if (order == 2) { if (rect) FG_LAUNCH_QUAD(2, true); else FG_LAUNCH_QUAD(2, false); }
  else            { if (rect) FG_LAUNCH_QUAD(1, true); else FG_LAUNCH_QUAD(1, false); }
#undef FG_LAUNCH_QUAD
}

void fgd_clip_general(int order, FgPairSpace ps, FgCells S, const double *mask, FgCells D,
                      double *tmp_area, double *tmp_clon, double *tmp_clat, int *nacc, int *defer_list, int *defer_cnt,
                      unsigned long long *stats, unsigned *err, hipStream_t st, const FgRect *rect, int *row_cnt, int *tmp_rowpos)
{
  const long np = fgd_pairs_total(ps);
  if (np <= 0) return;
  int grid = nblk(np, GEN_THREADS); if (grid > 1024) grid = 1024;
  const FgRect R = rect ? *rect : FgRect{};
#define FG_LAUNCH_GEN(O, RC) k_clip_general<O, RC><<<grid, GEN_THREADS, 0, st>>>(defer_list, defer_cnt, ps.src, ps.dst, S, mask, D, R, tmp_area, tmp_clon, tmp_clat, nacc, stats, err, row_cnt, tmp_rowpos)
  if (order == 2) { if (rect) FG_LAUNCH_GEN(2, true); else FG_LAUNCH_GEN(2, false); }
  else            { if (rect) FG_LAUNCH_GEN(1, true); else FG_LAUNCH_GEN(1, false); }
#undef FG_LAUNCH_GEN
}

void fgd_rect_tables(const double *lon, const double *lat, int nx, int ny, double *hdr, double *lat_ax, double *lon_ax, double *col,
                     double *col_min, double *col_max, double *col_avg, double *row, unsigned *bad, unsigned *err, hipStream_t st, double dst_tlon)
{
  const long np = (long)(nx + 1) * (ny + 1);
  const int g = (int)std::min<long>(1024, std::max<long>((np + 255) / 256, (std::max(nx, ny) + 1 + 255) / 256));
  k_rect_tables<<<std::max(g, 1), 256, 0, st>>>(lon, lat, nx, ny, hdr, lat_ax, lon_ax, col, col_min, col_max, col_avg, row, bad, err, dst_tlon);
}
void fgd_cell_struct2r(const FgTileSet &ts, const FgTile *tiles_in, FgTile *tiles_out, int ntiles, int nsrc, int ndst, FgCells S, double *area_out,
                       FgRect R, const double *mask, int order, int *src_idx_f, double *sums, unsigned *err, hipStream_t st,
                       unsigned long long *band_keys, int cull, int *heavy_list, int *heavy_cnt, FgPairSpace ps, int *pair_beg, int *pair_cnt,
                       int *big_list, int *big_cnt)
{
  const int nbS = nblk(nsrc, 256), nbD = nblk(ndst, 256);
  if (nbS + nbD > 0)
    k_cell_struct2r<<<nbS + nbD, 256, 0, st>>>(ts, tiles_in, tiles_out, ntiles, nsrc, ndst, nbS, S, area_out, R, mask, order, src_idx_f, sums, err,
                                               band_keys, cull, heavy_list, heavy_cnt, ps, pair_beg, pair_cnt, big_list, big_cnt);
}
void fgd_polylist_records(FgPolyList P, FgCells S, int *src_idx_f, double *sums, const FgRect *rect, int *heavy_list, int *heavy_cnt,
                          unsigned *err, hipStream_t st)
{
  if (P.npoly > 0)
    k_polylist_records<<<nblk(P.npoly, 256), 256, 0, st>>>(P, S, src_idx_f, sums, rect ? *rect : FgRect{}, rect ? 1 : 0, heavy_list, heavy_cnt, err);
}
void fgd_rect_materialize(int ndst, FgRect R, FgCells D, hipStream_t st)
{
  if (ndst > 0) k_rect_materialize<<<nblk(ndst, 256), 256, 0, st>>>(ndst, R, D);
}
void fgd_candidates_rect(int nsrc, FgCells S, const double *mask, FgRect R, FgPairSpace ps, int *pair_beg, int *pair_cnt,
                         const int *heavy_list, const int *heavy_cnt, int *big_list, int *big_cnt, hipStream_t st, int listed_only)
{
  if (nsrc <= 0) return;
  const int nbR = listed_only ? 0 : nblk(nsrc, 64);
  const int H = min(HEAVY_BLOCKS, max(64, nblk(nsrc, 8)));
  k_candidates_rect<<<nbR + H, 64, 0, st>>>(nsrc, H, S, mask, R, ps, pair_beg, pair_cnt, heavy_list, heavy_cnt, big_list, big_cnt);
}

void fgd_compact(int order, int nsrc, FgPairSpace ps, const FgCompactIo &io, hipStream_t st)
{
  if (nsrc <= 0) return;
  const long np = fgd_pairs_total(ps);
  if (order == 2) k_compact<2><<<BIG_BLOCKS + nblk(np, 256), 256, 0, st>>>(nsrc, ps, io);
  else            k_compact<1><<<BIG_BLOCKS + nblk(np, 256), 256, 0, st>>>(nsrc, ps, io);
}

void fgd_centroids(int nsrc, FgCells S, const double *sums, FgSrcRec *cen, hipStream_t st)
{
  if (nsrc > 0) k_centroids<<<nblk(nsrc, 256), 256, 0, st>>>(nsrc, S, sums, cen);
}

void fgd_distances(long nx, const int *x_src, const double *x_area, const FgSrcRec *cen, double *x_c1, double *x_c2, hipStream_t st)
{
  if (nx > 0) k_distances<<<nblk(nx, 256), 256, 0, st>>>(nx, x_src, x_area, cen, x_c1, x_c2);
}

__global__ __launch_bounds__(256) void k_accumulate_cell_sums(int n, const int *cells, int nsrc, const int *xoff, const double *xa,
                                                               const double *c1, const double *c2, double *total)
{
  const int i = blockIdx.x * blockDim.x + threadIdx.x;
  if (i >= n) return;
  const int s = cells ? cells[i] : i;
  if (s < 0 || s >= nsrc) return;
  const int b = xoff[s], e = xoff[s + 1];
  if (b >= e) return;
  double a0 = total[s], a1 = total[(size_t)nsrc + s], a2 = total[2 * (size_t)nsrc + s];
  for (int q = b; q < e; q++) { a0 += xa[q]; a1 += c1[q]; a2 += c2[q]; }
  total[s] = a0; total[(size_t)nsrc + s] = a1; total[2 * (size_t)nsrc + s] = a2;
}
void fgd_accumulate_cell_sums(int n, const int *cells, int nsrc, const int *xoff, const double *xa, const double *c1, const double *c2,
                              double *total, hipStream_t st)
{
  if (n > 0) k_accumulate_cell_sums<<<(n + 255) / 256, 256, 0, st>>>(n, cells, nsrc, xoff, xa, c1, c2, total);
}
```

Baseline: 5.316 billion exchange-cells/s.

## Pack per-exchange-cell area and centroid moments into an AoS record for order-2

For order-2 plans, the three separate double arrays (area, c1, c2) become one array of 24-byte FgXVal records. The compact, distance, CSR sort-gather and cell-sum kernels all switch to it, so each random gather by exchange index touches one record instead of three separate cache lines. Host transfer paths gain split and join kernels to convert between the packed layout and the separate host arrays. This adds a staging buffer and extra kernels on the get/set paths, and coalescing drops for purely streaming kernels.

```diff
diff --git a/fre-nctools_amd/csrc/apply_kernels.hip b/fre-nctools_amd/csrc/apply_kernels.hip
--- a/fre-nctools_amd/csrc/apply_kernels.hip
+++ b/fre-nctools_amd/csrc/apply_kernels.hip
@@ -64,7 +64,7 @@
 
 template <int ORDER, bool DIST, int BT, int G, bool STAGED>
 __device__ __forceinline__ void d_csr_records(const int *sh, const int *shs, const FgRowEnt *perm, int q0, int nq, const double *x_area,
-                                              const double *x_c1, const double *x_c2, const int *src_idx_f, const FgSrcRec *cen,
+                                              const FgXVal *x_val, const int *src_idx_f, const FgSrcRec *cen,
                                               const FgCsr &csr)
 {
   for (int i0 = threadIdx.x; i0 < nq; i0 += BT * G) {
@@ -78,8 +78,8 @@
     }
 #pragma unroll
     for (int g = 0; g < G; g++) {
-      ar[g] = x_area[n[g]];
-      if (ORDER == 2) { c1[g] = x_c1[n[g]]; c2[g] = x_c2[n[g]]; }
+      if (ORDER == 2) { const FgXVal v = x_val[n[g]]; ar[g] = v.area; c1[g] = v.c1; c2[g] = v.c2; }
+      else ar[g] = x_area[n[g]];
       idx[g] = src_idx_f[s[g]];
       if (ORDER == 2 && DIST) { const FgSrcRec r = cen[s[g]]; cl[g] = r.cen_lon; ct[g] = r.cen_lat; }
     }
@@ -116,7 +116,7 @@
 
 #define SG_GROUP 2
 template <int ORDER, int RPW, bool DIST, int BT, int G>
-__global__ __launch_bounds__(BT) void k_csr_sortgather(int ndst, FgRowEnt *perm, const double *x_area, const double *x_c1, const double *x_c2,
+__global__ __launch_bounds__(BT) void k_csr_sortgather(int ndst, FgRowEnt *perm, const double *x_area, const FgXVal *x_val,
                                                         const int *src_idx_f, const FgSrcRec *cen, FgCsr csr, int *tmp, long ntmp)
 {
   constexpr int SHORT = 12, CAP = (RPW >= 64) ? 512 : 2048;
@@ -212,8 +212,8 @@
     }
     __syncthreads();
   }
-  if (staged) d_csr_records<ORDER, DIST, BT, G, true>(sh, shs, perm, q0, nq, x_area, x_c1, x_c2, src_idx_f, cen, csr);
-  else        d_csr_records<ORDER, DIST, BT, G, false>(sh, shs, perm, q0, nq, x_area, x_c1, x_c2, src_idx_f, cen, csr);
+  if (staged) d_csr_records<ORDER, DIST, BT, G, true>(sh, shs, perm, q0, nq, x_area, x_val, src_idx_f, cen, csr);
+  else        d_csr_records<ORDER, DIST, BT, G, false>(sh, shs, perm, q0, nq, x_area, x_val, src_idx_f, cen, csr);
 }
 
 __global__ __launch_bounds__(256) void k_src_field_index(int order, const FgTile *tiles, int ntiles, int nsrc, int *src_idx_f)
@@ -989,14 +989,14 @@
 {
   if (nx_cap > 0) k_csr_fill_pos<<<nblk(nx_cap, 256), 256, 0, st>>>(nx_cap, nx_dev, x_src, x_dst, row_ptr, x_rowpos, perm);
 }
-void fgd_csr_sortgather(int order, int ndst, long nx, const FgRowEnt *perm, const double *x_area, const double *x_c1, const double *x_c2,
+void fgd_csr_sortgather(int order, int ndst, long nx, const FgRowEnt *perm, const double *x_area, const FgXVal *x_val,
                         const int *src_idx_f, const FgSrcRec *cen, FgCsr csr, hipStream_t st, int *tmp, long ntmp,
                         int long_rows)
 {
   if (ndst <= 0) return;
   FgRowEnt *pm = const_cast<FgRowEnt *>(perm);
   const int mode = nx > 256 * (long)ndst ? 2 : ((nx > 8 * (long)ndst || long_rows) ? 1 : 0);
-#define SG(O_, R_, D_) k_csr_sortgather<O_, R_, D_, (R_ >= 64 ? 64 : 256), SG_GROUP><<<nblk(ndst, R_), (R_ >= 64 ? 64 : 256), 0, st>>>(ndst, pm, x_area, x_c1, x_c2, src_idx_f, cen, csr, tmp, ntmp)
+#define SG(O_, R_, D_) k_csr_sortgather<O_, R_, D_, (R_ >= 64 ? 64 : 256), SG_GROUP><<<nblk(ndst, R_), (R_ >= 64 ? 64 : 256), 0, st>>>(ndst, pm, x_area, x_val, src_idx_f, cen, csr, tmp, ntmp)
 #define SGM(O_, D_) do { if (mode == 2) SG(O_, 1, D_); else if (mode == 1) SG(O_, 16, D_); else SG(O_, 64, D_); } while (0)
   if (order == 2) { if (cen) SGM(2, true); else SGM(2, false); }
   else SGM(1, false);
diff --git a/fre-nctools_amd/csrc/plan.hip b/fre-nctools_amd/csrc/plan.hip
--- a/fre-nctools_amd/csrc/plan.hip
+++ b/fre-nctools_amd/csrc/plan.hip
@@ -372,7 +372,8 @@
   FgPolyList polys{};
   long nx = 0;
   int *x_src = nullptr, *x_dst = nullptr;
-  double *x_area = nullptr, *x_c1 = nullptr, *x_c2 = nullptr;
+  double *x_area = nullptr;
+  FgXVal *x_val = nullptr;
   int *xoff = nullptr;
   FgRowEnt *perm = nullptr;
   bool rows_built = false;
@@ -408,7 +409,7 @@
   {
     while (owned.size() > keep) { g_pool.put(owned.back()); owned.pop_back(); }
     tiles_dev = nullptr; mask_dev = nullptr; S = FgCells{}; D = FgCells{};
-    x_src = x_dst = nullptr; x_area = x_c1 = x_c2 = nullptr; xoff = nullptr;
+    x_src = x_dst = nullptr; x_area = nullptr; x_val = nullptr; xoff = nullptr;
     perm = nullptr; csr.row_ptr = nullptr; csr.e1 = nullptr; csr.e2 = nullptr; cen = nullptr; src_idx_f = nullptr; sums = nullptr;
     have_geom = false; rect = false; rect_tab = FgRect{};
   }
@@ -653,8 +654,8 @@
   double *gc_res = gc_split ? blk.get<double>(2 * (size_t)tcap_all + 2) : nullptr;
   pl->xoff = blk.keep<int>(nsrc + 1);
   pl->x_src = blk.keep<int>(nx_alloc + 1); pl->x_dst = blk.keep<int>(nx_alloc + 1);
-  pl->x_area = blk.keep<double>(nx_alloc + 1);
-  if (order == 2) { pl->x_c1 = blk.keep<double>(nx_alloc + 1); pl->x_c2 = blk.keep<double>(nx_alloc + 1); pl->sums = blk.keep<double>(3 * (size_t)nsrc); }
+  if (order == 2) { pl->x_val = blk.keep<FgXVal>(nx_alloc + 1); pl->sums = blk.keep<double>(3 * (size_t)nsrc); }
+  else pl->x_area = blk.keep<double>(nx_alloc + 1);
   int *x_rowpos = blk.get<int>(nx_alloc + 1);
   pl->perm = blk.keep<FgRowEnt>(nx_alloc + 1);
   pl->csr.row_ptr = blk.keep<int>(ndst + 1);
@@ -753,7 +754,7 @@
   FgCompactIo io{};
   io.pair_beg = pair_beg; io.pair_cnt = pair_cnt;
   io.tmp_area = tmp_area; io.tmp_clon = tmp_clon; io.tmp_clat = tmp_clat;
-  io.xoff = pl->xoff; io.x_src = pl->x_src; io.x_dst = pl->x_dst; io.x_area = pl->x_area; io.x_c1 = pl->x_c1; io.x_c2 = pl->x_c2;
+  io.xoff = pl->xoff; io.x_src = pl->x_src; io.x_dst = pl->x_dst; io.x_area = pl->x_area; io.x_val = pl->x_val;
   io.row_cnt = row_cnt; io.x_rowpos = x_rowpos; io.sums = pl->sums; io.big_list = big_list; io.big_cnt = &dc->big_cnt;
   io.tmp_rowpos = tmp_rowpos; io.row_ptr = pl->csr.row_ptr; io.perm = pl->perm;
   io.dc = dc; io.xcap = nx_alloc;
@@ -782,7 +783,7 @@
     } else pl->csr.e1 = pl->alloc<FgCsrEntry1>(nx_alloc + 1);
     if (!pl->csr.e1 && !pl->csr.e2) return fail(FG_ERR_HIP, "out of device memory");
     int *sg_tmp = pl->alloc<int>(3 * (size_t)(nx_alloc + 1));
-    fgd_csr_sortgather(order, ndst, (long)nsrc + ndst, pl->perm, pl->x_area, pl->x_c1, pl->x_c2, pl->src_idx_f,
+    fgd_csr_sortgather(order, ndst, (long)nsrc + ndst, pl->perm, pl->x_area, pl->x_val, pl->src_idx_f,
                        order == 2 ? pl->cen : nullptr, pl->csr, st, sg_tmp, nx_alloc + 1);
     fused_tmp = sg_tmp;
     pt.end();
@@ -1294,7 +1295,7 @@
     return 0;
   };
   int rc = 0;
-  if ((rc = shrink(pl->x_src)) || (rc = shrink(pl->x_dst)) || (rc = shrink(pl->x_area)) || (rc = shrink(pl->x_c1)) || (rc = shrink(pl->x_c2))) return rc;
+  if ((rc = shrink(pl->x_src)) || (rc = shrink(pl->x_dst)) || (rc = shrink(pl->x_area)) || (rc = shrink(pl->x_val))) return rc;
   if (pl->perm && (rc = shrink(pl->perm))) return rc;
   return 0;
 }
@@ -1321,7 +1322,7 @@
     return fail(FG_ERR_STATE, "fg_plan_accumulate_cell_sums: needs a searched, not yet finalized order-2 plan");
   HIPCHK(hipSetDevice(pl->device));
   if (pl->nx > 0)
-    fgd_accumulate_cell_sums(cells_dev ? ncells : pl->nsrc, cells_dev, pl->nsrc, pl->xoff, pl->x_area, pl->x_c1, pl->x_c2, total_dev, pl->stream);
+    fgd_accumulate_cell_sums(cells_dev ? ncells : pl->nsrc, cells_dev, pl->nsrc, pl->xoff, pl->x_val, total_dev, pl->stream);
   if (sync) HIPCHK(hipStreamSynchronize(pl->stream));
   HIPCHK(hipGetLastError());
   return 0;
@@ -1380,7 +1381,7 @@
   if (!pl->csr.e1 && !pl->csr.e2) return fail(FG_ERR_HIP, "out of device memory");
   int *sg_tmp = pl->alloc<int>(3 * (size_t)(nx + 1));
   const int long_rows = !pl->rect && !pl->great_circle && pl->stats[FG_STAT_DEFERRED] > 0 && nx > 4 * (long)ndst;
-  fgd_csr_sortgather(pl->order, ndst, nx, pl->perm, pl->x_area, pl->x_c1, pl->x_c2, pl->src_idx_f, cen, pl->csr, st, sg_tmp, nx + 1,
+  fgd_csr_sortgather(pl->order, ndst, nx, pl->perm, pl->x_area, pl->x_val, pl->src_idx_f, cen, pl->csr, st, sg_tmp, nx + 1,
                      long_rows);
   HIPCHK(hipStreamSynchronize(st));
   HIPCHK(hipGetLastError());
@@ -1443,7 +1444,7 @@
   if (nx == 0) return 0;
   if (pl->dist_pending) {
     fg_plan *m = const_cast<fg_plan *>(pl);
-    fgd_distances(nx, pl->x_src, pl->x_area, pl->cen, m->x_c1, m->x_c2, pl->stream);
+    fgd_distances(nx, pl->x_src, pl->cen, m->x_val, pl->stream);
     HIPCHK(hipStreamSynchronize(pl->stream));
     m->dist_pending = false;
   }
@@ -1459,11 +1460,21 @@
     int *dst[5] = {t_in, i_in, j_in, i_out, j_out};
     for (int q = 0; q < 5; q++) if (dst[q]) jobs.push_back(XferJob{dst[q], idx + (size_t)q * nx, (size_t)nx * sizeof(int), true});
   }
-  if (area) jobs.push_back(XferJob{area, pl->x_area, (size_t)nx * sizeof(double), true});
+  double *val = nullptr;
+  struct PutBackVal { double *&p; ~PutBackVal() { g_pool.put(p); } } put_back_val{val};
   if (pl->order == 2) {
-    if (c1) jobs.push_back(XferJob{c1, pl->x_c1, (size_t)nx * sizeof(double), true});
-    if (c2) jobs.push_back(XferJob{c2, pl->x_c2, (size_t)nx * sizeof(double), true});
-  }
+    double *want[3] = {area, c1, c2}, *dev[3] = {nullptr, nullptr, nullptr};
+    int nwant = 0;
+    for (int q = 0; q < 3; q++) if (want[q]) nwant++;
+    if (nwant) {
+      val = (double *)g_pool.get(pl->device, (size_t)nwant * nx * sizeof(double));
+      if (!val) return fail(FG_ERR_HIP, "out of device memory");
+      for (int q = 0, k = 0; q < 3; q++) if (want[q]) dev[q] = val + (size_t)(k++) * nx;
+      fgd_xval_split(nx, pl->x_val, dev[0], dev[1], dev[2], pl->stream);
+      HIPCHK(hipStreamSynchronize(pl->stream));
+      for (int q = 0; q < 3; q++) if (want[q]) jobs.push_back(XferJob{want[q], dev[q], (size_t)nx * sizeof(double), true});
+    }
+  } else if (area) jobs.push_back(XferJob{area, pl->x_area, (size_t)nx * sizeof(double), true});
   if (!xfer_pool().run(pl->device, jobs)) return fail(FG_ERR_HIP, "fg_plan_get_xgrid: device -> host copy failed");
   return 0;
 }
@@ -1581,17 +1592,22 @@
   }
   pl->nx = nxgrid;
   pl->x_src = pl->alloc<int>(nxgrid + 1); pl->x_dst = pl->alloc<int>(nxgrid + 1);
-  pl->x_area = pl->alloc<double>(nxgrid + 1);
-  if (pl->order == 2) { pl->x_c1 = pl->alloc<double>(nxgrid + 1); pl->x_c2 = pl->alloc<double>(nxgrid + 1); }
-  if (!pl->x_src || !pl->x_dst || !pl->x_area || (pl->order == 2 && (!pl->x_c1 || !pl->x_c2))) return fail(FG_ERR_HIP, "out of device memory");
+  if (pl->order == 2) pl->x_val = pl->alloc<FgXVal>(nxgrid + 1);
+  else pl->x_area = pl->alloc<double>(nxgrid + 1);
+  if (!pl->x_src || !pl->x_dst || (!pl->x_area && !pl->x_val)) return fail(FG_ERR_HIP, "out of device memory");
   if (nxgrid > 0) {
     HIPCHK(hipMemcpy(pl->x_src, s.data(), nxgrid * sizeof(int), hipMemcpyHostToDevice));
     HIPCHK(hipMemcpy(pl->x_dst, d.data(), nxgrid * sizeof(int), hipMemcpyHostToDevice));
-    HIPCHK(hipMemcpy(pl->x_area, area, nxgrid * sizeof(double), hipMemcpyHostToDevice));
     if (pl->order == 2) {
-      HIPCHK(hipMemcpy(pl->x_c1, di_in, nxgrid * sizeof(double), hipMemcpyHostToDevice));
-      HIPCHK(hipMemcpy(pl->x_c2, dj_in, nxgrid * sizeof(double), hipMemcpyHostToDevice));
-    }
+      double *stage = pl->alloc<double>(3 * (size_t)nxgrid);
+      if (!stage) return fail(FG_ERR_HIP, "out of device memory");
+      HIPCHK(hipMemcpy(stage, area, nxgrid * sizeof(double), hipMemcpyHostToDevice));
+      HIPCHK(hipMemcpy(stage + nxgrid, di_in, nxgrid * sizeof(double), hipMemcpyHostToDevice));
+      HIPCHK(hipMemcpy(stage + 2 * nxgrid, dj_in, nxgrid * sizeof(double), hipMemcpyHostToDevice));
+      fgd_xval_join(nxgrid, stage, stage + nxgrid, stage + 2 * nxgrid, pl->x_val, pl->stream);
+      HIPCHK(hipStreamSynchronize(pl->stream));
+      pl->release(stage);
+    } else HIPCHK(hipMemcpy(pl->x_area, area, nxgrid * sizeof(double), hipMemcpyHostToDevice));
   }
   pl->searched = true;
   int rc = build_csr(pl, nullptr);
diff --git a/fre-nctools_amd/csrc/xgrid_device.h b/fre-nctools_amd/csrc/xgrid_device.h
--- a/fre-nctools_amd/csrc/xgrid_device.h
+++ b/fre-nctools_amd/csrc/xgrid_device.h
@@ -154,12 +154,14 @@
               int *tmp_rowpos = nullptr);
 struct alignas(8) FgRowEnt { int n, s; };
 struct alignas(16) FgSrcRec { double cen_lon, cen_lat; };
+struct alignas(8) FgXVal { double area, c1, c2; };
 struct FgCompactIo {
   const int *pair_beg, *pair_cnt;
   const double *tmp_area, *tmp_clon, *tmp_clat;
   const int *xoff;
   int *x_src, *x_dst;
-  double *x_area, *x_c1, *x_c2;
+  double *x_area;
+  FgXVal *x_val;
   int *row_cnt, *x_rowpos;
   const int *tmp_rowpos;
   const int *row_ptr; FgRowEnt *perm;
@@ -171,7 +173,9 @@
 };
 void fgd_compact(int order, int nsrc, FgPairSpace ps, const FgCompactIo &io, hipStream_t st);
 void fgd_centroids(int nsrc, FgCells S, const double *sums, FgSrcRec *cen, hipStream_t st);
-void fgd_distances(long nx, const int *x_src, const double *x_area, const FgSrcRec *cen, double *x_c1, double *x_c2, hipStream_t st);
+void fgd_distances(long nx, const int *x_src, const FgSrcRec *cen, FgXVal *x_val, hipStream_t st);
+void fgd_xval_split(long nx, const FgXVal *x_val, double *area, double *c1, double *c2, hipStream_t st);
+void fgd_xval_join(long nx, const double *area, const double *c1, const double *c2, FgXVal *x_val, hipStream_t st);
 
 struct FgCsrEntry1 { int idx_f; int pad; double area; };
 struct FgCsrEntry2 { int idx_f; int idx_g; double area, di, dj; };
@@ -184,7 +188,7 @@
 void fgd_csr_fill(long nx, const int *x_src, const int *x_dst, const int *row_ptr, int *row_fill, FgRowEnt *perm, hipStream_t st);
 void fgd_csr_fill_pos(long nx_cap, const unsigned long long *nx_dev, const int *x_src, const int *x_dst, const int *row_ptr, const int *x_rowpos,
                       FgRowEnt *perm, hipStream_t st);
-void fgd_csr_sortgather(int order, int ndst, long nx, const FgRowEnt *perm, const double *x_area, const double *x_c1, const double *x_c2,
+void fgd_csr_sortgather(int order, int ndst, long nx, const FgRowEnt *perm, const double *x_area, const FgXVal *x_val,
                         const int *src_idx_f, const FgSrcRec *cen, FgCsr csr, hipStream_t st, int *tmp = nullptr, long ntmp = 0,
                         int long_rows = 0);
 void fgd_src_field_index(int order, const FgTile *tiles_dev, int ntiles, int nsrc, int *src_idx_f, hipStream_t st);
@@ -242,8 +246,7 @@
 void fgd_box_ctr(double ll_lon, double ll_lat, double ur_lon, double ur_lat, double clon, double *out, hipStream_t st);
 void fgd_grid_area_no_adjust(int nx, int ny, const double *lon, const double *lat, double *area, hipStream_t st);
 
-void fgd_accumulate_cell_sums(int n, const int *cells, int nsrc, const int *xoff, const double *xa, const double *c1, const double *c2,
-                              double *total, hipStream_t st);
+void fgd_accumulate_cell_sums(int n, const int *cells, int nsrc, const int *xoff, const FgXVal *x_val, double *total, hipStream_t st);
 
 void fgd_gc_cell_struct(const FgTileXyz *tiles_dev, int ntiles, int ncells, FgCells c, hipStream_t st,
                         unsigned long long *band_keys = nullptr, int band_mode = 0);
diff --git a/fre-nctools_amd/csrc/xgrid_kernels.hip b/fre-nctools_amd/csrc/xgrid_kernels.hip
--- a/fre-nctools_amd/csrc/xgrid_kernels.hip
+++ b/fre-nctools_amd/csrc/xgrid_kernels.hip
@@ -1578,8 +1578,9 @@
   const int lb = c.beg - p0;
   for (int j = 0; j < c.cnt; j++) rank += ((unsigned)sh_d[lb + j] < (unsigned)c.d) ? 1 : 0;
   const long pos = c.x0 + rank;
-  io.x_src[pos] = c.s; io.x_dst[pos] = c.d; io.x_area[pos] = c.a;
-  if (ORDER == 2) { io.x_c1[pos] = c.l; io.x_c2[pos] = c.t; sh_v[0][lb + rank] = c.a; sh_v[1][lb + rank] = c.l; sh_v[2][lb + rank] = c.t; }
+  io.x_src[pos] = c.s; io.x_dst[pos] = c.d;
+  if (ORDER == 2) { io.x_val[pos] = FgXVal{c.a, c.l, c.t}; sh_v[0][lb + rank] = c.a; sh_v[1][lb + rank] = c.l; sh_v[2][lb + rank] = c.t; }
+  else io.x_area[pos] = c.a;
   if (io.tmp_rowpos) io.perm[c.row] = FgRowEnt{(int)pos, c.s};
   else return pos;
   return -1;
@@ -1661,11 +1662,11 @@
           a = io.tmp_area[p]; if (ORDER == 2) { l = io.tmp_clon[p]; t = io.tmp_clat[p]; }
           if (io.tmp_rowpos) row = io.row_ptr[d] + io.tmp_rowpos[p];
         }
-        io.x_src[pos] = s; io.x_dst[pos] = d; io.x_area[pos] = a;
+        io.x_src[pos] = s; io.x_dst[pos] = d;
         if (ORDER == 2) {
-          io.x_c1[pos] = l; io.x_c2[pos] = t;
+          io.x_val[pos] = FgXVal{a, l, t};
           sval[0][rank - c0] = a; sval[1][rank - c0] = l; sval[2][rank - c0] = t;
-        }
+        } else io.x_area[pos] = a;
         if (io.tmp_rowpos) io.perm[row] = FgRowEnt{(int)pos, s};
         else io.x_rowpos[pos] = atomicAdd(&io.row_cnt[d], 1);
       }
@@ -1756,16 +1757,30 @@
   if (s < nsrc) cen[s] = FgSrcRec{cl, ct};
 }
 
-__global__ __launch_bounds__(256) void k_distances(long nx, const int *x_src, const double *x_area, const FgSrcRec *cen, double *x_c1,
-                                                    double *x_c2)
+__global__ __launch_bounds__(256) void k_distances(long nx, const int *x_src, const FgSrcRec *cen, FgXVal *x_val)
 {
   long n = (long)blockIdx.x * blockDim.x + threadIdx.x;
   if (n >= nx) return;
-  int s = x_src[n];
-  double a = x_area[n];
-  double di = x_c1[n] / a, dj = x_c2[n] / a;
-  di -= cen[s].cen_lon; dj -= cen[s].cen_lat;
-  x_c1[n] = di; x_c2[n] = dj;
+  const FgXVal v = x_val[n];
+  const FgSrcRec r = cen[x_src[n]];
+  double di = v.c1 / v.area, dj = v.c2 / v.area;
+  di -= r.cen_lon; dj -= r.cen_lat;
+  x_val[n] = FgXVal{v.area, di, dj};
+}
+__global__ __launch_bounds__(256) void k_xval_split(long nx, const FgXVal *x_val, double *area, double *c1, double *c2)
+{
+  long n = (long)blockIdx.x * blockDim.x + threadIdx.x;
+  if (n >= nx) return;
+  const FgXVal v = x_val[n];
+  if (area) area[n] = v.area;
+  if (c1) c1[n] = v.c1;
+  if (c2) c2[n] = v.c2;
+}
+__global__ __launch_bounds__(256) void k_xval_join(long nx, const double *area, const double *c1, const double *c2, FgXVal *x_val)
+{
+  long n = (long)blockIdx.x * blockDim.x + threadIdx.x;
+  if (n >= nx) return;
+  x_val[n] = FgXVal{area[n], c1[n], c2[n]};
 }
 
 static inline int nblk(long n, int t) { return (int)((n + t - 1) / t); }
@@ -1885,13 +1900,21 @@
   if (nsrc > 0) k_centroids<<<nblk(nsrc, 256), 256, 0, st>>>(nsrc, S, sums, cen);
 }
 
-void fgd_distances(long nx, const int *x_src, const double *x_area, const FgSrcRec *cen, double *x_c1, double *x_c2, hipStream_t st)
-{
-  if (nx > 0) k_distances<<<nblk(nx, 256), 256, 0, st>>>(nx, x_src, x_area, cen, x_c1, x_c2);
-}
-
-__global__ __launch_bounds__(256) void k_accumulate_cell_sums(int n, const int *cells, int nsrc, const int *xoff, const double *xa,
-                                                               const double *c1, const double *c2, double *total)
+void fgd_distances(long nx, const int *x_src, const FgSrcRec *cen, FgXVal *x_val, hipStream_t st)
+{
+  if (nx > 0) k_distances<<<nblk(nx, 256), 256, 0, st>>>(nx, x_src, cen, x_val);
+}
+void fgd_xval_split(long nx, const FgXVal *x_val, double *area, double *c1, double *c2, hipStream_t st)
+{
+  if (nx > 0) k_xval_split<<<nblk(nx, 256), 256, 0, st>>>(nx, x_val, area, c1, c2);
+}
+void fgd_xval_join(long nx, const double *area, const double *c1, const double *c2, FgXVal *x_val, hipStream_t st)
+{
+  if (nx > 0) k_xval_join<<<nblk(nx, 256), 256, 0, st>>>(nx, area, c1, c2, x_val);
+}
+
+__global__ __launch_bounds__(256) void k_accumulate_cell_sums(int n, const int *cells, int nsrc, const int *xoff, const FgXVal *x_val,
+                                                               double *total)
 {
   const int i = blockIdx.x * blockDim.x + threadIdx.x;
   if (i >= n) return;
@@ -1900,11 +1923,10 @@
   const int b = xoff[s], e = xoff[s + 1];
   if (b >= e) return;
   double a0 = total[s], a1 = total[(size_t)nsrc + s], a2 = total[2 * (size_t)nsrc + s];
-  for (int q = b; q < e; q++) { a0 += xa[q]; a1 += c1[q]; a2 += c2[q]; }
+  for (int q = b; q < e; q++) { const FgXVal v = x_val[q]; a0 += v.area; a1 += v.c1; a2 += v.c2; }
   total[s] = a0; total[(size_t)nsrc + s] = a1; total[2 * (size_t)nsrc + s] = a2;
 }
-void fgd_accumulate_cell_sums(int n, const int *cells, int nsrc, const int *xoff, const double *xa, const double *c1, const double *c2,
-                              double *total, hipStream_t st)
-{
-  if (n > 0) k_accumulate_cell_sums<<<(n + 255) / 256, 256, 0, st>>>(n, cells, nsrc, xoff, xa, c1, c2, total);
-}
+void fgd_accumulate_cell_sums(int n, const int *cells, int nsrc, const int *xoff, const FgXVal *x_val, double *total, hipStream_t st)
+{
+  if (n > 0) k_accumulate_cell_sums<<<(n + 255) / 256, 256, 0, st>>>(n, cells, nsrc, xoff, x_val, total);
+}
```

Result: faster. 5.384 billion exchange-cells/s, median of 6 (+1.3%).
